# ZhehuiWu/MP-HSIR

Measured on AMD Instinct MI355X. Metric: hsi_patches_per_sec_fwd_bwd, higher is better.
Workload: dtype bf16; 1 GPU; natural-scene MP_HSIR_Net(31,31,64,T=6) training step fwd+bwd+allreduce+AdamW, 64x64x31 patches, batch 32/GPU, dp1; global_batch=32, patch=64x64x31, parallelism=dp1, launch=hipGraph replay

## Files before the change

include/mphsir.h:

```cpp
#ifndef MPHSIR_H
#define MPHSIR_H
#include <stddef.h>
#include <stdint.h>

#ifdef __cplusplus
extern "C" {
#endif

#define MPHSIR_OK 0
#define MPHSIR_EINVAL (-1)
#define MPHSIR_ELAUNCH (-2)

#define MPHSIR_F32 0
#define MPHSIR_BF16 1
#define MPHSIR_F16 2

const char* mphsir_version(void);
const char* mphsir_last_error(void);
int mphsir_device_arch(char* buf, int n);

typedef struct mphsir_gemm_args {
    uint32_t struct_size;
    const void* X; int64_t ldx;
    const void* W; int64_t w_batch_stride; int64_t rows_per_batch;
    const float* bias;
    const float* ln_w; const float* ln_b;
    void* Y; int64_t ldy;
    int64_t M, N, K;
    int epi;
    const void* R; int64_t ldr;
    const void* SA; int64_t ldsa;
    const float* gate;
    const float* keep;
    int32_t H, Wimg, shift;
    int32_t form;
} mphsir_gemm_args;
int mphsir_gemm_tok(const mphsir_gemm_args* a, int dtype, void* stream);

typedef struct mphsir_win_attn_args {
    uint32_t struct_size;
    const void* X;
    const float* ln_w; const float* ln_b;
    const void* Wqkv; const float* bqkv;
    const float* rpb;
    const void* Wproj; const float* bproj;
    void* SA;
    float* mu;
    void* Oattn;
    int32_t B, H, W, C, heads, shift;
} mphsir_win_attn_args;
typedef struct mphsir_pg_fwd_args {
    uint32_t struct_size;
    const float* mu;
    const float* Wprompt; const float* prompt_param; const float* Wq; const float* Wkv; const float* Wdown;
    const float* Wpproj; const float* bpproj; const float* Wup;
    float* gate;
    int32_t nW, C, r;
} mphsir_pg_fwd_args;
int mphsir_pg_gate_fwd(const mphsir_pg_fwd_args* a, void* stream);
int mphsir_win_attn_fwd(const mphsir_win_attn_args* a, int dtype, void* stream);
int mphsir_win_attn_hdp(int head_dim, int dtype);

typedef struct mphsir_gram_args {
    uint32_t struct_size;
    const void* Tq; int64_t ldq; const void* Tk; int64_t ldk; const void* Tv; int64_t ldv;
    const float* wq; const float* wk; const float* wv; int64_t ldw;
    void* V; int64_t ldvo;
    float* Gpart; float* Spart;
    int32_t B, H, W, C, heads, nsplit;
    void* QK; int64_t ldqk;
} mphsir_gram_args;
int mphsir_dwconv_gram(const mphsir_gram_args* a, int dtype, void* stream);
int mphsir_dwconv_gram_keeps_qk(int32_t C, int32_t W, int dtype);

typedef struct mphsir_fused_gram_args {
    uint32_t struct_size;
    const void* X; int64_t ldx;
    const float* ln_w; const float* ln_b;
    const void* Wqkv;
    const float* w9; int64_t ldw;
    void* V; int64_t ldvo;
    float* Gpart; float* Spart;
    int32_t B, H, W, C, heads, nsplit;
    int32_t head_groups;
    void* T; int64_t ldt;
    void* QK; int64_t ldqk;
    int32_t row_segments;
} mphsir_fused_gram_args;
int mphsir_qkv_dwconv_gram(const mphsir_fused_gram_args* a, int dtype, void* stream);
int mphsir_qkv_dwconv_gram_fits(int32_t C, int32_t heads, int32_t H, int32_t W, int dtype);
int mphsir_qkv_dwconv_gram_rows_fits(int32_t C, int32_t heads, int32_t H, int32_t W, int dtype, int32_t with_ln);
enum { MPHSIR_DEBUG_PG_GATE = 0, MPHSIR_DEBUG_WIN_ATTN = 1, MPHSIR_DEBUG_FUSED_PASS_A = 2 };
int mphsir_debug(int kind, void* stamps);
typedef struct mphsir_fold_args {
    uint32_t struct_size;
    const float* Gpart; const float* Spart;
    const float* temperature;
    const float* Wo;
    void* M;
    void* MT;
    int32_t B, C, heads, nsplit;
    float* Gsum; float* Ssum;
} mphsir_fold_args;
int mphsir_spectral_fold(const mphsir_fold_args* a, int dtype, void* stream);

typedef struct mphsir_gate_args {
    uint32_t struct_size;
    const void* T; int64_t ldt;
    const float* w9; int64_t ldw;
    void* U; int64_t ldu;
    int32_t B, H, W, HP;
} mphsir_gate_args;
int mphsir_dwconv_gate(const mphsir_gate_args* a, int dtype, void* stream);

typedef struct mphsir_gdfn_args {
    uint32_t struct_size;
    const void* X; int64_t ldx;
    const float* ln_w; const float* ln_b;
    const void* Win; const float* w9; int64_t ldw;
    const void* Wout;
    void* Y; int64_t ldy;
    int32_t B, H, W, D, HP, nsplit;
    void* T; int64_t ldt;
} mphsir_gdfn_args;
int mphsir_gdfn_fused(const mphsir_gdfn_args* a, int dtype, void* stream);
int mphsir_gdfn_fused_fits(int32_t D, int32_t HP, int32_t H, int32_t W, int dtype);
int mphsir_gdfn_fused_tile_width(int32_t D);

typedef struct mphsir_mlp_args {
    uint32_t struct_size;
    const void* X; int64_t ldx;
    const float* ln_w; const float* ln_b;
    const void* W1; const float* b1;
    const void* W2; const float* b2;
    const float* keep; int64_t rows_per_batch;
    void* Y; int64_t ldy;
    int64_t M; int32_t C, HP;
    int32_t tiles_per_wave;
    int32_t hsplit;
    float* ypart;
    const void* R; int64_t ldr;
    const void* PV; int64_t ldpv; const void* PM; int64_t pm_batch_stride;
    const void* PSA; int64_t ldpsa; const float* pgate; const float* pkeep;
    void* Yb; int64_t ldyb;
    int32_t H, Wimg, shift;
} mphsir_mlp_args;
int mphsir_gated_mlp_fwd(const mphsir_mlp_args* a, int dtype, void* stream);
int mphsir_gated_mlp_fwd_fuses(int32_t C, int64_t M, int dtype);

typedef struct mphsir_mlp_bwd_args {
    uint32_t struct_size;
    const void* X; const void* dY; const void* DM;
    const float* ln_w; const float* ln_b;
    const void* W1; const float* b1; const void* W1T; const void* W2T;
    void* dX; void* XN; void* H; void* DPRE; float* part;
    int64_t M; int32_t C, HP;
    int32_t variant;
    const float* keep;
    int64_t rows_per_batch;
    int32_t hsplit;
    float* dxn_part;
} mphsir_mlp_bwd_args;
int mphsir_gated_mlp_bwd(const mphsir_mlp_bwd_args* a, int dtype, void* stream);

typedef struct mphsir_mlp_wgrad_args {
    uint32_t struct_size;
    const void* XN; const void* DM;
    const void* W1; const float* b1; const void* W2T;
    float* dW1p; float* dW2p; float* db1p; float* db2p;
    int64_t M; int32_t C, HP;
    int32_t ranges;
    int32_t chunks_per_wg;
} mphsir_mlp_wgrad_args;
int mphsir_gated_mlp_wgrad(const mphsir_mlp_wgrad_args* a, int dtype, void* stream);
int mphsir_gated_mlp_wgrad_fits(int32_t C, int32_t chunks_per_wg, int dtype);

int mphsir_gdfn_dw_bwd(const void* T, const float* w9, int64_t ldw, const void* dU, void* U, void* dT, float* partial, int32_t nblk,
                       int32_t B, int32_t H, int32_t W, int32_t HP, int32_t round_mid, int dtype, void* stream);
int mphsir_gdfn_dw_bwd_fits(int32_t H, int32_t W, int32_t HP, int dtype);

int mphsir_combine_bwd(const void* dY, const void* SA, const float* gate, const float* keep, void* dOut, void* dSA,
                       float* dgate, int32_t B, int32_t H, int32_t W, int32_t C, int32_t shift, int dtype, void* stream);
typedef struct mphsir_win_attn_bwd_args {
    uint32_t struct_size;
    const void* X; const void* dSA; const float* dmu;
    const float* ln_w; const float* ln_b;
    const void* Wqkv; const float* bqkv; const float* rpb; const void* WprojT;
    void* dQKV; void* XNw; void* dSAt; float* drpb;
    int32_t B, H, W, C, heads, shift;
    int32_t head_split;
} mphsir_win_attn_bwd_args;
int mphsir_win_attn_bwd(const mphsir_win_attn_bwd_args* a, int dtype, void* stream);
int mphsir_win_attn_bwd_fits(int32_t C, int32_t heads, int dtype);
int mphsir_ln_bwd_win(const void* X, const void* dXNw, const void* dRes, const float* ln_w, void* dX, float* part,
                      int32_t B, int32_t H, int32_t W, int32_t C, int32_t shift, const float* ln_b, void* XN, int32_t linear,
                      int dtype, void* stream);

int mphsir_ln_bwd_win_dxn(const void* X, const void* dQKV, const void* WqkvT, const void* dRes, const void* dRes2, const float* ln_w, void* dX,
                          float* part, int32_t B, int32_t H, int32_t W, int32_t C, int32_t shift, int dtype, void* stream);
int mphsir_ln_bwd_win_dxn_fits(int32_t C, int dtype);
int mphsir_ln_bwd_tok_dxn(const void* X, const void* dY, const void* WT, const void* dRes, const float* ln_w, const float* ln_b, void* dX,
                          void* XN, float* part, int64_t M, int32_t C, int32_t K, int32_t x_f32, int dtype, void* stream);

int mphsir_layernorm_tok(const void* X, int x_dtype, const float* ln_w, const float* ln_b, void* Y, void* Xcopy, int y_dtype,
                         int64_t M, int32_t C, void* stream);

typedef struct mphsir_fold_bwd_args {
    uint32_t struct_size;
    const float* Gpart; const float* Spart; const float* temperature; const float* Wo; const float* dM;
    void* W2; float* dWo; float* dtemp;
    int32_t B, C, heads, nsplit;
    int32_t dM_nsplit;
    const void* DO; int64_t lddo; const void* V; int64_t ldv; int32_t N;
    const float* dm_scale;
    int32_t w2_blocks;
} mphsir_fold_bwd_args;
int mphsir_spectral_fold_bwd(const mphsir_fold_bwd_args* a, int dtype, void* stream);
typedef struct mphsir_pg_bwd_args {
    uint32_t struct_size;
    const float* mu; const float* dgate;
    const float* Wprompt; const float* prompt_param; const float* Wq; const float* Wkv; const float* Wdown;
    const float* Wpproj; const float* bpproj; const float* Wup;
    float* dmu; void* L; void* R;
    int32_t nW, C, r, KL, KR;
    int32_t lr_bf16;
} mphsir_pg_bwd_args;
int mphsir_pg_gate_bwd(const mphsir_pg_bwd_args* a, void* stream);

typedef struct mphsir_spectral_bwd_args {
    uint32_t struct_size;
    const void* QK; int64_t ldqk;
    const void* DO; int64_t lddo;
    const void* T; int64_t ldt;
    const void* W2; const void* MbT;
    const float* w9; int64_t ldw;
    void* dT; int64_t lddt;
    float* part;
    int32_t B, H, W, C, heads, nblk, round_dall;
    const float* vscale;
} mphsir_spectral_bwd_args;
int mphsir_spectral_dqkv_bwd(const mphsir_spectral_bwd_args* a, int dtype, void* stream);
int mphsir_spectral_dqkv_bwd_fits(int32_t C, int32_t heads, int32_t H, int32_t W, int dtype);
int mphsir_spectral_dqkv_bwd_slabs(int32_t C, int32_t heads);

int mphsir_conv3x3_tok(const void* X, int64_t ldx, const void* W, void* Y, int64_t ldy, int32_t B, int32_t H, int32_t Wd,
                       int32_t Cin, int32_t N, int dtype, void* stream);
int mphsir_im2col3x3(const void* X, int64_t ldx, void* Col, int32_t B, int32_t H, int32_t Wd, int32_t Cin, int dtype, void* stream);
int mphsir_conv3x3_wgrad(const void* dY, int64_t lddy, const void* X, int64_t ldx, float* Cpart, int32_t B, int32_t H, int32_t W,
                         int32_t Cout, int32_t Cin, int32_t nsplit, int32_t form ,
                         int dtype, void* stream);

int mphsir_gemm_tn(const void* A, int64_t lda, int64_t a_batch_stride, const void* B, int64_t ldb, int64_t b_batch_stride,
                   float* Cpart, float* colsum_part, int64_t M, int32_t N1, int32_t N2, int32_t nsplit, int32_t batch,
                   int32_t tile128, int dtype, void* stream);
#define MPHSIR_TN_GROUP_MAX 8
typedef struct mphsir_gemm_tn_problem {
    const void* A; int64_t lda; const void* B; int64_t ldb;
    float* Cpart; float* colsum_part;
    int64_t M; int32_t N1, N2, nsplit, pad_;
} mphsir_gemm_tn_problem;
int mphsir_gemm_tn_group(const mphsir_gemm_tn_problem* probs, int32_t n, int32_t form , int dtype, void* stream);

int mphsir_dwconv3x3(const void* X, int64_t ldx, const float* w9, int64_t ldw, void* Y, int64_t ldy,
                     int32_t B, int32_t H, int32_t W, int32_t C, int32_t flip, int dtype, void* stream);
int mphsir_dwconv3x3_wgrad(const void* X, int64_t ldx, const void* dY, int64_t lddy, float* partial, int32_t nblk,
                           int32_t B, int32_t H, int32_t W, int32_t C, int dtype, void* stream);
int mphsir_dwconv3x3_wgrad_tiled(int32_t H, int32_t W, int32_t C, int dtype);
int mphsir_dwconv3x3_bwd(const void* X, int64_t ldx, const void* dY, int64_t lddy, const float* w9, int64_t ldw, void* dX, int64_t lddx,
                         float* partial, int32_t nblk, int32_t B, int32_t H, int32_t W, int32_t C, int dtype, void* stream);

int mphsir_gdfn_gate_bwd(const void* T, const void* dU, void* U, void* dT, int64_t M, int32_t HP, int dtype, void* stream);
int mphsir_dwconv_gate_bwd(const void* T, const float* w9, int64_t ldw, const void* dU, void* U, void* dT, int32_t B, int32_t H, int32_t W,
                           int32_t HP, int dtype, void* stream);
int mphsir_dwconv_gate_bwd_fits(int32_t H, int32_t W, int32_t HP, int dtype);

int64_t mphsir_gemm_tn_workspace_bytes(int32_t N1, int32_t N2, int32_t nsplit, int32_t batch, int32_t with_colsum);
int64_t mphsir_dwconv_gram_workspace_bytes(int32_t B, int32_t nsplit, int32_t C, int32_t heads);
int64_t mphsir_pg_gate_bwd_workspace_bytes(int32_t nW, int32_t C, int32_t r, int dtype, int32_t* KL, int32_t* KR);
int64_t mphsir_win_attn_bwd_workspace_bytes(int32_t B, int32_t H, int32_t W, int32_t C, int32_t heads, int dtype);

int mphsir_tvsp_text_map(const float* L, const float* clip, float* text, int32_t B, int32_t ps, int32_t D, void* stream);
int mphsir_tvsp_text_map_bwd(const float* dtext, const float* clip, float* part, int32_t B, int32_t ps, int32_t D, void* stream);
int mphsir_resize_bilinear(const void* X, void* Y, int32_t B, int32_t h, int32_t w, int32_t H, int32_t W, int32_t C, int32_t backward,
                           int dtype, void* stream);

int mphsir_nchw_to_cl(const float* X, void* Y, int32_t B, int32_t C, int64_t HW, int32_t Cp, int dtype, void* stream);
int mphsir_cl_to_nchw_add(const void* Y, int64_t ldy, const float* R, float* O, int32_t B, int32_t C, int64_t HW, int dtype, void* stream);
int mphsir_task_weights(const int64_t* ids, float* w, int32_t B, int32_t n, int32_t T, void* stream);
int mphsir_mix_rows(const float* A, const float* Bm, float* O, int32_t I, int32_t J, int32_t D, float scale, int32_t transA, void* stream);

typedef struct mphsir_scene_gather_args {
    uint32_t struct_size;
    const float* scene;
    const int32_t* origins;
    float* tiles;
    int32_t n, C, H, W, th, tw;
} mphsir_scene_gather_args;
int mphsir_scene_gather(const mphsir_scene_gather_args* a, void* stream);
typedef struct mphsir_scene_blend_args {
    uint32_t struct_size;
    const float* tiles;
    const int32_t* oy;
    const int32_t* ox;
    float* scene;
    int32_t ny, nx, C, H, W, th, tw, ov, clamp01;
} mphsir_scene_blend_args;
int mphsir_scene_blend(const mphsir_scene_blend_args* a, void* stream);

typedef struct mphsir_scene_gather_d4_args {
    uint32_t struct_size;
    const float* scene;
    const int32_t* origins;
    float* tiles;
    int32_t j0, count, n_tiles, G, modes_packed, C, H, W, th, tw;
} mphsir_scene_gather_d4_args;
int mphsir_scene_gather_d4(const mphsir_scene_gather_d4_args* a, void* stream);
typedef struct mphsir_scene_fold_d4_args {
    uint32_t struct_size;
    const float* y;
    float* store;
    int32_t j0, count, n_tiles, G, modes_packed, C, th, tw;
} mphsir_scene_fold_d4_args;
int mphsir_scene_fold_d4(const mphsir_scene_fold_d4_args* a, void* stream);

typedef struct mphsir_quality_args {
    uint32_t struct_size;
    const float* restored;
    const float* clean;
    double* psnr;
    double* ssim;
    double* sam_deg;
    int64_t* sam_pixels;
    void* workspace;
    int64_t workspace_bytes;
    int32_t B, C, H, W;
} mphsir_quality_args;
int64_t mphsir_quality_workspace_bytes(int32_t B, int32_t C, int32_t H, int32_t W);
int mphsir_quality(const mphsir_quality_args* a, void* stream);

#define MPHSIR_DEG_NONE 0
#define MPHSIR_DEG_GAUSSIAN 1
#define MPHSIR_DEG_COMPLEX 2
#define MPHSIR_DEG_BLUR 3
#define MPHSIR_DEG_SR 4
#define MPHSIR_DEG_INPAINT 5
#define MPHSIR_DEG_BANDMISS 6
#define MPHSIR_DEG_HAZE 7
#define MPHSIR_DEG_MAX_TASKS 16
#define MPHSIR_DEG_MAX_STENCILS 16
#define MPHSIR_DEG_MAX_FACTORS 8
#define MPHSIR_DEG_STENCIL_SIDE 21
typedef struct mphsir_degrade_args {
    uint32_t struct_size;
    const float* clean;
    float* degraded;
    float* clean_aug;
    const int32_t* menu;
    const int32_t* ksize;
    const int32_t* sr_factor;
    const int32_t* task;
    const int32_t* aug;
    const float* param;
    const int32_t* sub;
    const float* band_sigma;
    const uint8_t* band_flag;
    const uint8_t* col_dead;
    const float* col_off;
    const float* stencils;
    const float* cirrus;
    const float* atm;
    const float* haze_ratio;
    const float* z;
    const float* u0;
    const float* u1;
    const int64_t* ordinal_dev;
    int64_t seed, ordinal;
    int32_t B, C, H, W, T, K, F;
} mphsir_degrade_args;
int mphsir_degrade_batch(const mphsir_degrade_args* a, void* stream);

int mphsir_flat_adamw(float* p, const float* g, float* m, float* v, int64_t n, float lr, float beta1, float beta2,
                      float eps, float weight_decay, int32_t step, float grad_scale, const float* hyper, void* stream);

int mphsir_grad_check(const float* g, int64_t n, float* scaler, void* stream);
int mphsir_flat_adamw_scaled(float* p, const float* g, float* m, float* v, int64_t n, float lr, float beta1, float beta2, float eps,
                             float weight_decay, float grad_scale, const float* hyper, const float* scaler, void* stream);
int mphsir_scaler_update(float* scaler, float growth_factor, float backoff_factor, int32_t growth_interval, void* stream);

#define MPHSIR_REDUCE_MAX_SEGS 32
typedef struct mphsir_reduce_seg {
    const float* src; float* dst;
    int64_t n, stride, src_batch_stride, dst_batch_stride;
    int32_t nsplit, nbatch;
    int32_t rows, dst_col_stride;
    int64_t src_ld, dst_ld;
} mphsir_reduce_seg;
int mphsir_reduce_parts(const mphsir_reduce_seg* segs, int32_t nseg, void* stream);

int mphsir_pack_gather(const float* arena, const int32_t* index, void* dst, int64_t n, int dtype, void* stream);

int mphsir_multi_copy(const int64_t* table_dev, int32_t nseg, int64_t total_blocks, void* stream);

int mphsir_l1_clamp_loss(const float* y, const float* clean, float* grad, float* part, int64_t n, int32_t nblocks, void* stream);

#define MPHSIR_K_GEMM_TOK 0
#define MPHSIR_K_WIN_ATTN 1
#define MPHSIR_K_DWCONV_GRAM 2
#define MPHSIR_K_SPECTRAL_FOLD 3
#define MPHSIR_K_GATED_MLP 4
#define MPHSIR_K_DWCONV_GATE 5
#define MPHSIR_K_FLAT_ADAMW 6
#define MPHSIR_K_DWCONV 7
#define MPHSIR_K_DWCONV_WGRAD 8
#define MPHSIR_K_GATED_MLP_BWD 9
#define MPHSIR_K_COMBINE_BWD 10
#define MPHSIR_K_WIN_ATTN_BWD 11
#define MPHSIR_K_LN_BWD_WIN 12
#define MPHSIR_K_GEMM_TN 13
#define MPHSIR_K_GDFN_GATE_BWD 14
#define MPHSIR_K_FOLD_BWD 15
#define MPHSIR_K_PG_GATE_BWD 16
#define MPHSIR_K_CONV3X3 17
#define MPHSIR_K_IM2COL 18
#define MPHSIR_K_REDUCE_PARTS 19
#define MPHSIR_K_PACK_GATHER 20
#define MPHSIR_K_LAYERNORM 21
#define MPHSIR_K_PG_GATE 22
#define MPHSIR_K_RESAMPLE 23
#define MPHSIR_K_QKV_DWCONV_GRAM 24
#define MPHSIR_K_GDFN_FUSED 25
#define MPHSIR_K_DWCONV_BWD 26
#define MPHSIR_K_MULTI_COPY 27
#define MPHSIR_K_L1_LOSS 28
#define MPHSIR_K_GATED_MLP_WGRAD 29
#define MPHSIR_K_SPECTRAL_DQKV_BWD 30
#define MPHSIR_K_LAYOUT 31
#define MPHSIR_K_SCENE 32
#define MPHSIR_K_QUALITY 33
#define MPHSIR_K_DEGRADE 34
#define MPHSIR_K_COUNT 35
int mphsir_prof_enable(int kid);
int mphsir_prof_read(int* launches, float* total_ms);
const char* mphsir_kernel_name(int kid);

#ifdef __cplusplus
}
#endif
#endif
```

mp-hsir_amd/_lib.py:

```python
import ctypes
import os

import torch

_HERE = os.path.dirname(os.path.abspath(__file__))
_PATH = os.path.join(_HERE, os.environ.get("MPHSIR_LIB_AB", "libmphsir.so"))
_lib = None
_is_emu = False

c_void_p, c_int64, c_int32, c_int, c_float_p = (ctypes.c_void_p, ctypes.c_int64, ctypes.c_int32, ctypes.c_int,
                                                ctypes.POINTER(ctypes.c_float))


class _Args(ctypes.Structure):

    def __init__(self, *args, **kw):
        super().__init__(*args, **kw)
        self.struct_size = ctypes.sizeof(self)


_SZ = [("struct_size", ctypes.c_uint32)]


class GemmArgs(_Args):
    _fields_ = _SZ + [("X", c_void_p), ("ldx", c_int64), ("W", c_void_p), ("w_batch_stride", c_int64),
                ("rows_per_batch", c_int64), ("bias", c_void_p), ("ln_w", c_void_p), ("ln_b", c_void_p),
                ("Y", c_void_p), ("ldy", c_int64), ("M", c_int64), ("N", c_int64), ("K", c_int64),
                ("epi", c_int), ("R", c_void_p), ("ldr", c_int64), ("SA", c_void_p), ("ldsa", c_int64),
                ("gate", c_void_p), ("keep", c_void_p), ("H", c_int32), ("Wimg", c_int32), ("shift", c_int32), ("form", c_int32)]


class MlpArgs(_Args):
    _fields_ = _SZ + [("X", c_void_p), ("ldx", c_int64), ("ln_w", c_void_p), ("ln_b", c_void_p), ("W1", c_void_p),
                ("b1", c_void_p), ("W2", c_void_p), ("b2", c_void_p), ("keep", c_void_p), ("rows_per_batch", c_int64),
                ("Y", c_void_p), ("ldy", c_int64), ("M", c_int64), ("C", c_int32), ("HP", c_int32), ("tiles_per_wave", c_int32),
                ("hsplit", c_int32), ("ypart", c_void_p), ("R", c_void_p), ("ldr", c_int64),
                ("PV", c_void_p), ("ldpv", c_int64), ("PM", c_void_p), ("pm_batch_stride", c_int64), ("PSA", c_void_p), ("ldpsa", c_int64),
                ("pgate", c_void_p), ("pkeep", c_void_p), ("Yb", c_void_p), ("ldyb", c_int64), ("H", c_int32), ("Wimg", c_int32), ("shift", c_int32)]


class WinAttnArgs(_Args):
    _fields_ = _SZ + [(n, c_void_p) for n in ("X", "ln_w", "ln_b", "Wqkv", "bqkv", "rpb", "Wproj", "bproj", "SA", "mu", "Oattn")] + \
               [(n, c_int32) for n in ("B", "H", "W", "C", "heads", "shift")]


class PgFwdArgs(_Args):
    _fields_ = _SZ + [(n, c_void_p) for n in ("mu", "Wprompt", "prompt_param", "Wq", "Wkv", "Wdown", "Wpproj", "bpproj", "Wup", "gate")] + \
               [(n, c_int32) for n in ("nW", "C", "r")]


class GramArgs(_Args):
    _fields_ = _SZ + [("Tq", c_void_p), ("ldq", c_int64), ("Tk", c_void_p), ("ldk", c_int64), ("Tv", c_void_p), ("ldv", c_int64),
                ("wq", c_void_p), ("wk", c_void_p), ("wv", c_void_p), ("ldw", c_int64), ("V", c_void_p), ("ldvo", c_int64),
                ("Gpart", c_void_p), ("Spart", c_void_p)] + [(n, c_int32) for n in ("B", "H", "W", "C", "heads", "nsplit")] + \
               [("QK", c_void_p), ("ldqk", c_int64)]


class FusedGramArgs(_Args):
    _fields_ = _SZ + [("X", c_void_p), ("ldx", c_int64), ("ln_w", c_void_p), ("ln_b", c_void_p), ("Wqkv", c_void_p), ("w9", c_void_p),
                ("ldw", c_int64), ("V", c_void_p), ("ldvo", c_int64), ("Gpart", c_void_p), ("Spart", c_void_p)] + \
               [(n, c_int32) for n in ("B", "H", "W", "C", "heads", "nsplit", "head_groups")] + \
               [("T", c_void_p), ("ldt", c_int64), ("QK", c_void_p), ("ldqk", c_int64), ("row_segments", c_int32)]


class FoldArgs(_Args):
    _fields_ = _SZ + [("Gpart", c_void_p), ("Spart", c_void_p), ("temperature", c_void_p), ("Wo", c_void_p), ("M", c_void_p),
                ("MT", c_void_p)] + \
               [(n, c_int32) for n in ("B", "C", "heads", "nsplit")] + [("Gsum", c_void_p), ("Ssum", c_void_p)]


class GateArgs(_Args):
    _fields_ = _SZ + [("T", c_void_p), ("ldt", c_int64), ("w9", c_void_p), ("ldw", c_int64), ("U", c_void_p), ("ldu", c_int64)] + \
               [(n, c_int32) for n in ("B", "H", "W", "HP")]


class GdfnArgs(_Args):
    _fields_ = _SZ + [("X", c_void_p), ("ldx", c_int64), ("ln_w", c_void_p), ("ln_b", c_void_p), ("Win", c_void_p), ("w9", c_void_p),
                ("ldw", c_int64), ("Wout", c_void_p), ("Y", c_void_p), ("ldy", c_int64)] + \
               [(n, c_int32) for n in ("B", "H", "W", "D", "HP", "nsplit")] + [("T", c_void_p), ("ldt", c_int64)]


class MlpBwdArgs(_Args):
    _fields_ = _SZ + [(n, c_void_p) for n in ("X", "dY", "DM", "ln_w", "ln_b", "W1", "b1", "W1T", "W2T", "dX", "XN", "H", "DPRE", "part")] + \
               [("M", c_int64), ("C", c_int32), ("HP", c_int32), ("variant", c_int32), ("keep", c_void_p), ("rows_per_batch", c_int64),
                ("hsplit", c_int32), ("dxn_part", c_void_p)]


class MlpWgradArgs(_Args):
    _fields_ = _SZ + [(n, c_void_p) for n in ("XN", "DM", "W1", "b1", "W2T", "dW1p", "dW2p", "db1p", "db2p")] + \
               [("M", c_int64), ("C", c_int32), ("HP", c_int32), ("ranges", c_int32), ("chunks_per_wg", c_int32)]


class WinAttnBwdArgs(_Args):
    _fields_ = _SZ + [(n, c_void_p) for n in ("X", "dSA", "dmu", "ln_w", "ln_b", "Wqkv", "bqkv", "rpb", "WprojT", "dQKV", "XNw",
                                         "dSAt", "drpb")] + [(n, c_int32) for n in ("B", "H", "W", "C", "heads", "shift", "head_split")]


class FoldBwdArgs(_Args):
    _fields_ = _SZ + [(n, c_void_p) for n in ("Gpart", "Spart", "temperature", "Wo", "dM", "W2", "dWo", "dtemp")] + \
               [(n, c_int32) for n in ("B", "C", "heads", "nsplit", "dM_nsplit")] + \
               [("DO", c_void_p), ("lddo", c_int64), ("V", c_void_p), ("ldv", c_int64), ("N", c_int32), ("dm_scale", c_void_p),
                ("w2_blocks", c_int32)]


class PgBwdArgs(_Args):
    _fields_ = _SZ + [(n, c_void_p) for n in ("mu", "dgate", "Wprompt", "prompt_param", "Wq", "Wkv", "Wdown", "Wpproj", "bpproj", "Wup",
                                         "dmu", "L", "R")] + [(n, c_int32) for n in ("nW", "C", "r", "KL", "KR", "lr_bf16")]


class SpectralBwdArgs(_Args):
    _fields_ = _SZ + [("QK", c_void_p), ("ldqk", c_int64), ("DO", c_void_p), ("lddo", c_int64), ("T", c_void_p), ("ldt", c_int64),
                      ("W2", c_void_p), ("MbT", c_void_p), ("w9", c_void_p), ("ldw", c_int64), ("dT", c_void_p), ("lddt", c_int64),
                      ("part", c_void_p)] + [(n, c_int32) for n in ("B", "H", "W", "C", "heads", "nblk", "round_dall")] + [("vscale", c_void_p)]


class SceneGatherArgs(_Args):
    _fields_ = _SZ + [("scene", c_void_p), ("origins", c_void_p), ("tiles", c_void_p)] + [(n, c_int32) for n in ("n", "C", "H", "W", "th", "tw")]


class SceneBlendArgs(_Args):
    _fields_ = _SZ + [("tiles", c_void_p), ("oy", c_void_p), ("ox", c_void_p), ("scene", c_void_p)] + \
               [(n, c_int32) for n in ("ny", "nx", "C", "H", "W", "th", "tw", "ov", "clamp01")]


class SceneGatherD4Args(_Args):
    _fields_ = _SZ + [("scene", c_void_p), ("origins", c_void_p), ("tiles", c_void_p)] + \
               [(n, c_int32) for n in ("j0", "count", "n_tiles", "G", "modes_packed", "C", "H", "W", "th", "tw")]


class SceneFoldD4Args(_Args):
    _fields_ = _SZ + [("y", c_void_p), ("store", c_void_p)] + [(n, c_int32) for n in ("j0", "count", "n_tiles", "G", "modes_packed", "C", "th", "tw")]


class QualityArgs(_Args):
    _fields_ = _SZ + [(n, c_void_p) for n in ("restored", "clean", "psnr", "ssim", "sam_deg", "sam_pixels", "workspace")] + \
               [("workspace_bytes", c_int64)] + [(n, c_int32) for n in ("B", "C", "H", "W")]


class DegradeArgs(_Args):
    _fields_ = _SZ + [(n, c_void_p) for n in ("clean", "degraded", "clean_aug", "menu", "ksize", "sr_factor", "task", "aug", "param", "sub", "band_sigma",
                                         "band_flag", "col_dead", "col_off", "stencils", "cirrus", "atm", "haze_ratio", "z", "u0", "u1",
                                         "ordinal_dev")] + [("seed", c_int64), ("ordinal", c_int64)] + \
               [(n, c_int32) for n in ("B", "C", "H", "W", "T", "K", "F")]


class TnProblem(ctypes.Structure):
    _fields_ = [("A", c_void_p), ("lda", c_int64), ("B", c_void_p), ("ldb", c_int64), ("Cpart", c_void_p), ("colsum_part", c_void_p),
                ("M", c_int64), ("N1", c_int32), ("N2", c_int32), ("nsplit", c_int32), ("pad_", c_int32)]


TN_GROUP_MAX = 8


class ReduceSeg(ctypes.Structure):
    _fields_ = [("src", c_void_p), ("dst", c_void_p), ("n", c_int64), ("stride", c_int64), ("src_batch_stride", c_int64),
                ("dst_batch_stride", c_int64), ("nsplit", c_int32), ("nbatch", c_int32), ("rows", c_int32),
                ("dst_col_stride", c_int32), ("src_ld", c_int64), ("dst_ld", c_int64)]


REDUCE_MAX_SEGS = 32


_SYMBOLS = {
    "mphsir_version": (ctypes.c_char_p, []),
    "mphsir_last_error": (ctypes.c_char_p, []),
    "mphsir_device_arch": (c_int, [ctypes.c_char_p, c_int]),
    "mphsir_kernel_name": (ctypes.c_char_p, [c_int]),
    "mphsir_gemm_tn_workspace_bytes": (c_int64, [c_int32, c_int32, c_int32, c_int32, c_int32]),
    "mphsir_dwconv_gram_workspace_bytes": (c_int64, [c_int32, c_int32, c_int32, c_int32]),
    "mphsir_pg_gate_bwd_workspace_bytes": (c_int64, [c_int32, c_int32, c_int32, c_int, ctypes.POINTER(c_int32), ctypes.POINTER(c_int32)]),
    "mphsir_win_attn_bwd_workspace_bytes": (c_int64, [c_int32, c_int32, c_int32, c_int32, c_int32, c_int]),
    "mphsir_prof_enable": (c_int, [c_int]),
    "mphsir_prof_read": (c_int, [ctypes.POINTER(c_int), c_float_p]),
    "mphsir_gemm_tok": (c_int, [ctypes.POINTER(GemmArgs), c_int, c_void_p]),
    "mphsir_tvsp_text_map": (c_int, [c_void_p, c_void_p, c_void_p, c_int32, c_int32, c_int32, c_void_p]),
    "mphsir_tvsp_text_map_bwd": (c_int, [c_void_p, c_void_p, c_void_p, c_int32, c_int32, c_int32, c_void_p]),
    "mphsir_resize_bilinear": (c_int, [c_void_p, c_void_p, c_int32, c_int32, c_int32, c_int32, c_int32, c_int32, c_int32, c_int, c_void_p]),
    "mphsir_layernorm_tok": (c_int, [c_void_p, c_int, c_void_p, c_void_p, c_void_p, c_void_p, c_int, c_int64, c_int32, c_void_p]),
    "mphsir_win_attn_fwd": (c_int, [ctypes.POINTER(WinAttnArgs), c_int, c_void_p]),
    "mphsir_win_attn_hdp": (c_int, [c_int, c_int]),
    "mphsir_pg_gate_fwd": (c_int, [ctypes.POINTER(PgFwdArgs), c_void_p]),
    "mphsir_dwconv_gram": (c_int, [ctypes.POINTER(GramArgs), c_int, c_void_p]),
    "mphsir_dwconv_gram_keeps_qk": (c_int, [c_int32, c_int32, c_int]),
    "mphsir_qkv_dwconv_gram": (c_int, [ctypes.POINTER(FusedGramArgs), c_int, c_void_p]),
    "mphsir_qkv_dwconv_gram_fits": (c_int, [c_int32, c_int32, c_int32, c_int32, c_int]),
    "mphsir_qkv_dwconv_gram_rows_fits": (c_int, [c_int32, c_int32, c_int32, c_int32, c_int, c_int32]),
    "mphsir_debug": (c_int, [c_int, c_void_p]),
    "mphsir_dwconv3x3_wgrad_tiled": (c_int, [c_int32, c_int32, c_int32, c_int]),
    "mphsir_spectral_fold": (c_int, [ctypes.POINTER(FoldArgs), c_int, c_void_p]),
    "mphsir_dwconv_gate": (c_int, [ctypes.POINTER(GateArgs), c_int, c_void_p]),
    "mphsir_dwconv_gate_bwd": (c_int, [c_void_p, c_void_p, c_int64, c_void_p, c_void_p, c_void_p, c_int32, c_int32, c_int32, c_int32, c_int, c_void_p]),
    "mphsir_dwconv_gate_bwd_fits": (c_int, [c_int32, c_int32, c_int32, c_int]),
    "mphsir_gdfn_dw_bwd": (c_int, [c_void_p, c_void_p, c_int64, c_void_p, c_void_p, c_void_p, c_void_p, c_int32, c_int32, c_int32, c_int32, c_int32, c_int32, c_int, c_void_p]),
    "mphsir_gdfn_dw_bwd_fits": (c_int, [c_int32, c_int32, c_int32, c_int]),
    "mphsir_gdfn_fused": (c_int, [ctypes.POINTER(GdfnArgs), c_int, c_void_p]),
    "mphsir_gdfn_fused_fits": (c_int, [c_int32, c_int32, c_int32, c_int32, c_int]),
    "mphsir_gdfn_fused_tile_width": (c_int, [c_int32]),
    "mphsir_dwconv3x3": (c_int, [c_void_p, c_int64, c_void_p, c_int64, c_void_p, c_int64, c_int32, c_int32, c_int32, c_int32,
                                 c_int32, c_int, c_void_p]),
    "mphsir_dwconv3x3_bwd": (c_int, [c_void_p, c_int64, c_void_p, c_int64, c_void_p, c_int64, c_void_p, c_int64, c_void_p, c_int32, c_int32, c_int32,
                                     c_int32, c_int32, c_int, c_void_p]),
    "mphsir_dwconv3x3_wgrad": (c_int, [c_void_p, c_int64, c_void_p, c_int64, c_void_p, c_int32, c_int32, c_int32, c_int32,
                                       c_int32, c_int, c_void_p]),
    "mphsir_flat_adamw": (c_int, [c_void_p, c_void_p, c_void_p, c_void_p, c_int64, ctypes.c_float, ctypes.c_float,
                                  ctypes.c_float, ctypes.c_float, ctypes.c_float, c_int32, ctypes.c_float, c_void_p, c_void_p]),
    "mphsir_grad_check": (c_int, [c_void_p, c_int64, c_void_p, c_void_p]),
    "mphsir_flat_adamw_scaled": (c_int, [c_void_p, c_void_p, c_void_p, c_void_p, c_int64, ctypes.c_float, ctypes.c_float, ctypes.c_float,
                                         ctypes.c_float, ctypes.c_float, ctypes.c_float, c_void_p, c_void_p, c_void_p]),
    "mphsir_scaler_update": (c_int, [c_void_p, ctypes.c_float, ctypes.c_float, c_int32, c_void_p]),
    "mphsir_combine_bwd": (c_int, [c_void_p] * 7 + [c_int32] * 5 + [c_int, c_void_p]),
    "mphsir_win_attn_bwd": (c_int, [ctypes.POINTER(WinAttnBwdArgs), c_int, c_void_p]),
    "mphsir_win_attn_bwd_fits": (c_int, [c_int32, c_int32, c_int]),
    "mphsir_ln_bwd_win": (c_int, [c_void_p] * 6 + [c_int32] * 5 + [c_void_p, c_void_p, c_int32, c_int, c_void_p]),
    "mphsir_ln_bwd_win_dxn": (c_int, [c_void_p] * 8 + [c_int32] * 5 + [c_int, c_void_p]),
    "mphsir_ln_bwd_win_dxn_fits": (c_int, [c_int32, c_int]),
    "mphsir_ln_bwd_tok_dxn": (c_int, [c_void_p] * 9 + [c_int64, c_int32, c_int32, c_int32, c_int, c_void_p]),
    "mphsir_gemm_tn": (c_int, [c_void_p, c_int64, c_int64, c_void_p, c_int64, c_int64, c_void_p, c_void_p, c_int64, c_int32, c_int32,
                               c_int32, c_int32, c_int32, c_int, c_void_p]),
    "mphsir_spectral_fold_bwd": (c_int, [ctypes.POINTER(FoldBwdArgs), c_int, c_void_p]),
    "mphsir_pg_gate_bwd": (c_int, [ctypes.POINTER(PgBwdArgs), c_void_p]),
    "mphsir_spectral_dqkv_bwd": (c_int, [ctypes.POINTER(SpectralBwdArgs), c_int, c_void_p]),
    "mphsir_spectral_dqkv_bwd_fits": (c_int, [c_int32, c_int32, c_int32, c_int32, c_int]),
    "mphsir_spectral_dqkv_bwd_slabs": (c_int, [c_int32, c_int32]),
    "mphsir_conv3x3_tok": (c_int, [c_void_p, c_int64, c_void_p, c_void_p, c_int64, c_int32, c_int32, c_int32, c_int32, c_int32,
                                   c_int, c_void_p]),
    "mphsir_conv3x3_wgrad": (c_int, [c_void_p, c_int64, c_void_p, c_int64, c_void_p, c_int32, c_int32, c_int32, c_int32, c_int32, c_int32, c_int32, c_int, c_void_p]),
    "mphsir_im2col3x3": (c_int, [c_void_p, c_int64, c_void_p, c_int32, c_int32, c_int32, c_int32, c_int, c_void_p]),
    "mphsir_gdfn_gate_bwd": (c_int, [c_void_p, c_void_p, c_void_p, c_void_p, c_int64, c_int32, c_int, c_void_p]),
    "mphsir_gated_mlp_bwd": (c_int, [ctypes.POINTER(MlpBwdArgs), c_int, c_void_p]),
    "mphsir_gated_mlp_wgrad": (c_int, [ctypes.POINTER(MlpWgradArgs), c_int, c_void_p]),
    "mphsir_gated_mlp_wgrad_fits": (c_int, [c_int32, c_int32, c_int]),
    "mphsir_gated_mlp_fwd": (c_int, [ctypes.POINTER(MlpArgs), c_int, c_void_p]),
    "mphsir_gated_mlp_fwd_fuses": (c_int, [c_int32, c_int64, c_int]),
    "mphsir_reduce_parts": (c_int, [ctypes.POINTER(ReduceSeg), c_int32, c_void_p]),
    "mphsir_gemm_tn_group": (c_int, [ctypes.POINTER(TnProblem), c_int32, c_int32, c_int, c_void_p]),
    "mphsir_pack_gather": (c_int, [c_void_p, c_void_p, c_void_p, c_int64, c_int, c_void_p]),
    "mphsir_multi_copy": (c_int, [c_void_p, c_int32, c_int64, c_void_p]),
    "mphsir_nchw_to_cl": (c_int, [c_void_p, c_void_p, c_int32, c_int32, c_int64, c_int32, c_int, c_void_p]),
    "mphsir_cl_to_nchw_add": (c_int, [c_void_p, c_int64, c_void_p, c_void_p, c_int32, c_int32, c_int64, c_int, c_void_p]),
    "mphsir_task_weights": (c_int, [c_void_p, c_void_p, c_int32, c_int32, c_int32, c_void_p]),
    "mphsir_mix_rows": (c_int, [c_void_p, c_void_p, c_void_p, c_int32, c_int32, c_int32, ctypes.c_float, c_int32, c_void_p]),
    "mphsir_scene_gather": (c_int, [ctypes.POINTER(SceneGatherArgs), c_void_p]),
    "mphsir_scene_blend": (c_int, [ctypes.POINTER(SceneBlendArgs), c_void_p]),
    "mphsir_scene_gather_d4": (c_int, [ctypes.POINTER(SceneGatherD4Args), c_void_p]),
    "mphsir_scene_fold_d4": (c_int, [ctypes.POINTER(SceneFoldD4Args), c_void_p]),
    "mphsir_quality_workspace_bytes": (c_int64, [c_int32, c_int32, c_int32, c_int32]),
    "mphsir_quality": (c_int, [ctypes.POINTER(QualityArgs), c_void_p]),
    "mphsir_degrade_batch": (c_int, [ctypes.POINTER(DegradeArgs), c_void_p]),
    "mphsir_l1_clamp_loss": (c_int, [c_void_p, c_void_p, c_void_p, c_void_p, c_int64, c_int32, c_void_p]),
}


def symbols():
    return sorted(_SYMBOLS)


def _bind(lib):
    for name, (res, args) in _SYMBOLS.items():
        fn = getattr(lib, name)
        fn.restype = res
        fn.argtypes = args
    return lib


def load(path=None):
    global _lib, _is_emu
    if _lib is not None and path is None:
        return _lib
    p = path or _PATH
    if not os.path.exists(p):
        raise RuntimeError("mp-hsir_amd: HIP library %s not found -- run `python mp-hsir_amd/build.py` "
                           "(there is no CPU fallback)" % p)
    try:
        lib = _bind(ctypes.CDLL(p))
    except (OSError, AttributeError) as e:
        raise RuntimeError("mp-hsir_amd: cannot load %s: %s" % (p, e))
    _lib = lib
    _is_emu = path is not None and "hipemu" in os.path.abspath(path)
    return _lib


def use_library_for_tests(path):
    return load(path)


def is_emulated():
    return _is_emu


def check(rc, what):
    if rc != 0:
        raise RuntimeError("mp-hsir_amd: %s failed (%d): %s" % (what, rc, load().mphsir_last_error().decode()))
```

mp-hsir_amd/autograd_ops.py:

```python
import torch
import torch.nn.functional as F

from . import ops


class SkipGrad:

    def __init__(self):
        self.dz = None

    def take(self):
        dz, self.dz = self.dz, None
        return dz


def _skip_put(skip, dz, needed):
    if not needed:
        return None
    if skip is not None and skip[2]:
        skip[0].dz = dz
        return None
    return dz


def _skip_take(skip):
    return skip[0].take() if (skip is not None and skip[1]) else None


class _GatedMlp(torch.autograd.Function):

    @staticmethod
    def forward(ctx, blk, k2, y, ln_w, ln_b, fc1_w, fc1_b, fc2_w, fc2_b, res=None, skip=None):
        B, H, W, Cc = y.shape
        pk = blk.packed(y.dtype)
        ctx.blk, ctx.k2, ctx.skip = blk, k2, skip
        ctx.save_for_backward(y)
        z = ops.gated_mlp_fwd(y.reshape(-1, Cc), pk["ln2"][0], pk["ln2"][1], pk["W1"], pk["b1"], pk["W2"], pk["b2"],
                              keep=k2, rows_per_batch=H * W, res=None if res is None else res.reshape(-1, Cc))
        return z.reshape(B, H, W, Cc)

    @staticmethod
    def backward(ctx, dz):
        (y,) = ctx.saved_tensors
        return (None, None) + _gated_mlp_backward(ctx.blk, ctx.k2, y, dz) + (_skip_put(ctx.skip, dz, ctx.needs_input_grad[9]), None)


def _gated_mlp_backward(blk, k2, y, dz):
    B, H, W, Cc = y.shape
    dt = y.dtype
    pk = blk.packed(dt)
    dz2 = dz.reshape(-1, Cc).contiguous()
    hid = blk.mlp.fc2.weight.shape[1]
    HP = pk["W2T"].shape[0]
    fused = ops.gated_mlp_wgrad_fits(dz2.shape[0], Cc, HP, dt)
    if k2 is None:
        dm = dz2
        dx, xn, h, dpre, part = ops.gated_mlp_bwd(y.reshape(-1, Cc), dz2, dm, pk["ln2"][0], pk["ln2"][1], pk["W1"], pk["b1"],
                                                  pk["W1T"], pk["W2T"], operands=not fused)
    else:
        dx, xn, h, dpre, part, dm = ops.gated_mlp_bwd(y.reshape(-1, Cc), dz2, None, pk["ln2"][0], pk["ln2"][1], pk["W1"], pk["b1"],
                                                      pk["W1T"], pk["W2T"], keep=k2, rows_per_batch=H * W, operands=not fused)
    with ops.reduce_scope(leaf=True):
        if fused:
            dW1, db1, dW2, db2 = ops.gated_mlp_wgrad(xn, dm, pk["W1"], pk["b1"], pk["W2T"], hid)
        else:
            dW2, db2 = ops.gemm_tn_blocks(dm, h, [(0, Cc)], ncols=hid, colsum=True)
            dW1, db1 = ops.gemm_tn_blocks(dpre, xn, [(0, hid), (HP, hid)], colsum=True)
        dln = ops.reduce_parts(part)
    return (dx.reshape(B, H, W, Cc), dln[0], dln[1], dW1, db1, dW2, db2)


def channel_attention_bwd(d_out, t_q, t_k, t_v, w9q, w9k, w9v, v, gp, sp, Mb, MbT, temperature, wo, heads, B, H, W, qk=None, keep=None):
    C = v.shape[1]
    N = H * W
    M = B * N
    dt = v.dtype
    temp32, wo32 = temperature.detach().reshape(heads).float().contiguous(), wo.detach().reshape(C, C).float().contiguous()
    joint = (t_q.data_ptr() + C * t_q.element_size() == t_k.data_ptr() and t_k.data_ptr() + C * t_k.element_size() == t_v.data_ptr()
             and t_q.stride() == t_k.stride() == t_v.stride() and w9q.data_ptr() + 4 * C == w9k.data_ptr()
             and w9k.data_ptr() + 4 * C == w9v.data_ptr())
    fused = joint and t_q.stride(2) == 3 * C and w9q.stride(0) == 3 * C and ops.spectral_dqkv_bwd_fits(C, heads, H, W, dt)
    if ops.fold_bwd_forms_dm(N, C, heads, dt):
        W2, dwo_p, dtemp_p = ops.spectral_fold_bwd(gp, sp, temp32, wo32, None, dt, reduce=False, d_out=d_out.reshape(M, C), v=v.reshape(M, C), dm_scale=keep,
                                                   w2_blocks=fused)
    else:
        dM = ops.gemm_tn(d_out.reshape(B, N, C), v.reshape(B, N, C), reduce=False)
        W2, dwo_p, dtemp_p = ops.spectral_fold_bwd(gp, sp, temp32, wo32, dM, dt, reduce=False, dm_scale=keep, w2_blocks=fused)
    if qk is not None:
        pass
    elif joint:
        qk = ops.dwconv3x3(torch.as_strided(t_q, (B, H, W, 2 * C), t_q.stride()), torch.as_strided(w9q, (9, 2 * C), w9q.stride()))
    else:
        qk = torch.empty((B, H, W, 2 * C), dtype=dt, device=v.device)
        ops.dwconv3x3(t_q, w9q, out=qk[..., :C])
        ops.dwconv3x3(t_k, w9k, out=qk[..., C:])
    if fused:
        dwo, dtemp = ops.reduce_parts(dwo_p), ops.reduce_parts(dtemp_p)
        t_all = torch.as_strided(t_q, (M, 3 * C), (3 * C, 1))
        w9_all = torch.as_strided(w9q, (9, 3 * C), w9q.stride())
        dt_all, dw_all = ops.spectral_dqkv_bwd(qk.reshape(M, 2 * C), d_out, t_all, W2, MbT, w9_all, B, H, W, C, heads, vscale=keep)
        dt_all = dt_all.reshape(B, H, W, 3 * C)
        return (dt_all[..., :C], dt_all[..., C:2 * C], dt_all[..., 2 * C:], dw_all[:C], dw_all[C:2 * C], dw_all[2 * C:], dtemp, dwo)
    assert keep is None, "the unscaled d_out form needs the fused launch (ops.spectral_dqkv_bwd_fits)"
    dall = torch.empty((M, 3 * C), dtype=dt, device=v.device)
    ops.gemm_tok(d_out, MbT, out=dall[:, 2 * C:])
    dwo, dtemp = ops.reduce_parts(dwo_p), ops.reduce_parts(dtemp_p)
    ops.gemm_tok(qk.reshape(M, 2 * C), W2, out=dall[:, :2 * C])
    dall4 = dall.reshape(B, H, W, 3 * C)
    if joint:
        t_all = torch.as_strided(t_q, (B, H, W, 3 * C), t_q.stride())
        w9_all = torch.as_strided(w9q, (9, 3 * C), w9q.stride())
        dt_all, dw_all = ops.dwconv3x3_bwd(t_all, dall4, w9_all, col_ranges=[(0, 3 * C)])
        return (dt_all[..., :C], dt_all[..., C:2 * C], dt_all[..., 2 * C:], dw_all[:C], dw_all[C:2 * C], dw_all[2 * C:],
                dtemp, dwo)
    dq4, dk4, dv4 = dall4[..., :C], dall4[..., C:2 * C], dall4[..., 2 * C:]
    dw3 = torch.empty((3 * C, 9), dtype=torch.float32, device=v.device)
    dkv = torch.empty((B, H, W, 2 * C), dtype=dt, device=v.device)
    return (ops.dwconv3x3(dq4, w9q, flip=True), ops.dwconv3x3(dk4, w9k, flip=True, out=dkv[..., :C]), ops.dwconv3x3(dv4, w9v, flip=True, out=dkv[..., C:]),
            ops.dwconv3x3_wgrad(t_q, dq4, col_ranges=[(0, C)], out=dw3[:C]), ops.dwconv3x3_wgrad(t_k, dk4, col_ranges=[(0, C)], out=dw3[C:2 * C]),
            ops.dwconv3x3_wgrad(t_v, dv4, col_ranges=[(0, C)], out=dw3[2 * C:]), dtemp, dwo)


import os
COMBINE_SIDE = os.environ.get("MPHSIR_COMBINE_SIDE", "0") == "1"


_PG_KEYS = ("linear_down.weight", "linear_up.weight", "linear_prompt.weight", "prompt_param", "q.weight", "kv.weight",
            "proj.weight", "proj.bias")


def _pass_a_infer(x2, wqkv, w9, B, H, W, C, heads, ln=None):
    if ops.qkv_dwconv_gram_fits(C, heads, H, W, x2.dtype):
        v, gp, sp, _ = ops.qkv_dwconv_gram(x2, wqkv, w9, B, H, W, C, heads, ln=ln)
    else:
        t = ops.gemm_tok(x2, wqkv, ln=ln)
        v, gp, sp, _ = ops.dwconv_gram(t[:, :C], t[:, C:2 * C], t[:, 2 * C:], w9[:, :C], w9[:, C:2 * C], w9[:, 2 * C:], 3 * C, B, H, W, C, heads)
    return v, gp, sp


def _pgsstb_attn_infer(blk, k1, x, fuse=False):
    B, H, W, Cc = x.shape
    dt = x.dtype
    pk = blk.packed(dt)
    sp = blk.gobal_spectral_attn.packed(dt)
    heads, shift = blk.num_heads, blk.shift_size
    sa, mu, _ = ops.win_attn_fwd(x, pk["ln1"][0], pk["ln1"][1], pk["wqkv"], pk["bqkv"], pk["rpb"], pk["wproj"], pk["bproj"],
                                 pk["pg"], heads, shift, gate=False)
    sa2 = sa.reshape(-1, Cc)
    v, gp, spart = _pass_a_infer(sa2, sp["wqkv"], sp["w9"], B, H, W, Cc, heads)
    with ops.side_stream(sa, ops.SIDE_BRANCH) as br:
        gate = ops.pg_gate_fwd(mu, pk["pg"])
    Mb = ops.spectral_fold(gp, spart, sp["temp"], sp["wo"], dt)
    br.join()
    if fuse:
        return dict(v=v, Mb=Mb, sa=sa2, gate=gate, keep=k1, geom=(H, W, shift))
    y = ops.gemm_tok(v, Mb, epi=2, res=x.reshape(-1, Cc), sa=sa2, gate=gate, keep=k1, geom=(H, W, shift))
    return y.reshape(B, H, W, Cc)


def _self_channel_attn_infer(attn, ln, geom, t2):
    B, H, W = geom
    pa = attn.packed(t2.dtype)
    v, gp, sp = _pass_a_infer(t2, pa["wqkv"], pa["w9"], B, H, W, t2.shape[1], attn.num_heads, ln=ln.pair())
    return ops.gemm_tok(v, ops.spectral_fold(gp, sp, pa["temp"], pa["wo"], t2.dtype), epi=1, res=t2)


def _pgsstb_attn_forward(blk, k1, x, fuse=False):
    B, H, W, Cc = x.shape
    dt = x.dtype
    pk = blk.packed(dt)
    sp = blk.gobal_spectral_attn.packed(dt)
    heads, shift = blk.num_heads, blk.shift_size
    w9 = sp["w9"]
    sa, mu, oattn = ops.win_attn_fwd(x, pk["ln1"][0], pk["ln1"][1], pk["wqkv"], pk["bqkv"], pk["rpb"], pk["wproj"],
                                     pk["bproj"], pk["pg"], heads, shift, save=True, gate=False)
    with ops.side_stream(sa, ops.SIDE_BRANCH) as br:
        gate = ops.pg_gate_fwd(mu, pk["pg"])
    sa2 = sa.reshape(-1, Cc)
    if ops.FUSED_TRAIN and ops.qkv_dwconv_gram_fits(Cc, heads, H, W, dt):
        v, gp, spart, _, t, qk = ops.qkv_dwconv_gram(sa2, sp["wqkv"], w9, B, H, W, Cc, heads, keep=True)
    else:
        t = ops.gemm_tok(sa2, sp["wqkv"])
        v, gp, spart, _, qk = ops.dwconv_gram(t[:, :Cc], t[:, Cc:2 * Cc], t[:, 2 * Cc:], w9[:, :Cc], w9[:, Cc:2 * Cc], w9[:, 2 * Cc:],
                                              3 * Cc, B, H, W, Cc, heads, keep_qk=True)
    Mb, MbT, gp, spart = ops.spectral_fold(gp, spart, sp["temp"], sp["wo"], dt, transposed=True)
    br.join()
    saved = (x, sa, gate, mu, oattn, t, v, gp, spart, Mb, MbT) + ((qk,) if qk is not None else ())
    if fuse:
        return None, saved
    y = ops.gemm_tok(v, Mb, epi=2, res=x.reshape(-1, Cc), sa=sa2, gate=gate, keep=k1, geom=(H, W, shift))
    return y.reshape(B, H, W, Cc), saved


def _pgsstb_attn_backward(blk, k1, saved, dy, extra=None):
    x, sa, gate, mu, oattn, t, v, gp, spart, Mb, MbT = saved[:11]
    qk = saved[11] if len(saved) > 11 else None
    B, H, W, Cc = x.shape
    dt = x.dtype
    M = B * H * W
    heads, shift = blk.num_heads, blk.shift_size
    pk = blk.packed(dt)
    sp = blk.gobal_spectral_attn.packed(dt)
    dy = dy.contiguous()
    with ops.reduce_scope(leaf=True):
        f32_factors = dt == torch.float16 or mu.shape[0] <= 512
        lean = COMBINE_SIDE and ops.spectral_dqkv_bwd_fits(Cc, heads, H, W, dt) and sp["w9"].stride(0) == 3 * Cc and t.is_contiguous()
        if lean:
            with ops.side_stream(dy, ops.SIDE_BRANCH) as br:
                _, d_sa, dgate = ops.combine_bwd(dy, sa, gate, k1, shift, want_dout=False)
                dmu, gpg = ops.pg_gate_bwd(mu, dgate, pk["pg"], factor_dtype=torch.float32 if f32_factors else dt)
            d_out, keep_s = dy, k1
        else:
            d_out, d_sa, dgate = ops.combine_bwd(dy, sa, gate, k1, shift)
            keep_s = None
            with ops.side_stream(dy, ops.SIDE_BRANCH) as br:
                dmu, gpg = ops.pg_gate_bwd(mu, dgate, pk["pg"], factor_dtype=torch.float32 if f32_factors else dt)
        t4 = t.reshape(B, H, W, 3 * Cc)
        w9 = sp["w9"]
        tq, tk, tv = t4[..., :Cc], t4[..., Cc:2 * Cc], t4[..., 2 * Cc:]
        dtq, dtk, dtv, dwq, dwk, dwv, dtemp, dwo = channel_attention_bwd(
            d_out.reshape(M, Cc), tq, tk, tv, w9[:, :Cc], w9[:, Cc:2 * Cc], w9[:, 2 * Cc:], v, gp, spart, Mb, MbT,
            blk.gobal_spectral_attn.temperature, blk.gobal_spectral_attn.project_out.weight, heads, B, H, W, qk=qk, keep=keep_s)
        if dtq.data_ptr() + Cc * dtq.element_size() == dtk.data_ptr() and dtq.stride(2) == 3 * Cc:
            dt3 = torch.as_strided(dtq, (M, 3 * Cc), (3 * Cc, 1))
        else:
            dt3 = torch.cat([dtq, dtk, dtv], dim=-1).reshape(M, 3 * Cc)
        if lean:
            br.join()
        d_sa = ops.gemm_tok(dt3, sp["wqkvT"], epi=1, res=d_sa.reshape(M, Cc))
        d_sqkv = ops.gemm_tn(dt3, sa.reshape(M, Cc)).reshape(3 * Cc, Cc, 1, 1)
        dpg = tuple(gpg[k].reshape(getattr_path(blk.local_spectral_attn, k).shape) for k in _PG_KEYS)
        if not lean:
            br.join()
        dqkv, xnw, dsat, drpb = ops.win_attn_bwd(x, d_sa.reshape(B, H, W, Cc), dmu, pk["ln1"][0], pk["ln1"][1], pk["wqkv"], pk["bqkv"],
                                                 pk["rpb"], pk["wprojT"], heads, shift)
        d_qkv_w, d_qkv_b = ops.gemm_tn(dqkv, xnw, colsum=True)
        dsat2 = dsat.reshape(M, Cc)
        d_proj_w, d_proj_b = ops.gemm_tn(dsat2, oattn.reshape(M, Cc), colsum=True)
        if ops.ln_bwd_win_dxn_fits(M, Cc, dt):
            dx, part = ops.ln_bwd_win_dxn(x, dqkv, pk["wqkvT"], dy, pk["ln1"][0], shift, dres2=None if extra is None else extra.contiguous())
        else:
            dx, part = ops.ln_bwd_win(x, ops.gemm_tok(dqkv, pk["wqkvT"]), dy, pk["ln1"][0], shift)
            if extra is not None:
                dx = dx + extra
        dln = ops.reduce_parts(part)
        drpb = ops.reduce_parts(drpb)
    d_sdw = _join_taps(dwq, dwk, dwv).reshape(3 * Cc, 1, 3, 3)
    return (dx, dln[0], dln[1], d_qkv_w, d_qkv_b, d_proj_w, d_proj_b, drpb,
            dtemp.reshape(heads, 1, 1), d_sqkv, d_sdw, dwo.reshape(Cc, Cc, 1, 1)) + tuple(dpg)




class _PgsstbAttn(torch.autograd.Function):

    @staticmethod
    def forward(ctx, blk, k1, skip, x, n1w, n1b, qkv_w, qkv_b, proj_w, proj_b, rpb, s_temp, s_qkv, s_dw, s_out, *pg):
        y, saved = _pgsstb_attn_forward(blk, k1, x)
        ctx.blk, ctx.k1, ctx.skip = blk, k1, skip
        ctx.save_for_backward(*saved)
        return y

    @staticmethod
    def backward(ctx, dy):
        return (None, None, None) + _pgsstb_attn_backward(ctx.blk, ctx.k1, ctx.saved_tensors, dy, extra=_skip_take(ctx.skip))


_N_ATTN_PARAMS = 11 + len(_PG_KEYS)


class _Pgsstb(torch.autograd.Function):

    @staticmethod
    def forward(ctx, blk, k1, k2, res, skip, x, *params):
        B, H, W, Cc = x.shape
        _, saved = _pgsstb_attn_forward(blk, k1, x, fuse=True)
        pk = blk.packed(x.dtype)
        z, y = ops.gated_mlp_fwd(x.reshape(-1, Cc), pk["ln2"][0], pk["ln2"][1], pk["W1"], pk["b1"], pk["W2"], pk["b2"], keep=k2, rows_per_batch=H * W,
                                 res=None if res is None else res.reshape(-1, Cc),
                                 branch=dict(v=saved[6], Mb=saved[9], sa=saved[1].reshape(-1, Cc), gate=saved[2], keep=k1,
                                             geom=(H, W, blk.shift_size), want_y=True))
        ctx.blk, ctx.k1, ctx.k2, ctx.skip = blk, k1, k2, skip
        ctx.save_for_backward(y.reshape(B, H, W, Cc), *saved)
        return z.reshape(B, H, W, Cc)

    @staticmethod
    def backward(ctx, dz):
        y, saved = ctx.saved_tensors[0], ctx.saved_tensors[1:]
        d_res = _skip_put(ctx.skip, dz, ctx.needs_input_grad[3])
        gm = _gated_mlp_backward(ctx.blk, ctx.k2, y, dz)
        ga = _pgsstb_attn_backward(ctx.blk, ctx.k1, saved, gm[0], extra=_skip_take(ctx.skip))
        return (None, None, None, d_res, None) + ga + gm[1:]


def _join_taps(*dw):
    w0 = dw[0]
    ok, off = True, w0.data_ptr()
    for w in dw:
        ok = (ok and w.data_ptr() == off and w.is_contiguous()
              and w.untyped_storage().data_ptr() == w0.untyped_storage().data_ptr())
        off += w.numel() * w.element_size()
    if ok:
        return torch.as_strided(w0, (sum(w.shape[0] for w in dw), 9), (9, 1))
    ops.flush_deferred()
    return torch.cat(dw, dim=0)


def getattr_path(mod, dotted):
    for part in dotted.split("."):
        mod = getattr(mod, part)
    return mod


def pgsstb(blk, x, k1, k2, res=None, skip=None):
    a, sp, pgm = blk.attn, blk.gobal_spectral_attn, blk.local_spectral_attn
    m = blk.mlp
    B, H, W, Cc = x.shape
    fuse = ops.gated_mlp_fuses(B * H * W, Cc, H * W, x.dtype)
    if not torch.is_grad_enabled():
        if fuse:
            pk = blk.packed(x.dtype)
            z, _ = ops.gated_mlp_fwd(x.reshape(-1, Cc), pk["ln2"][0], pk["ln2"][1], pk["W1"], pk["b1"], pk["W2"], pk["b2"], keep=k2, rows_per_batch=H * W,
                                     res=None if res is None else res.reshape(-1, Cc), branch=_pgsstb_attn_infer(blk, k1, x, fuse=True))
            return z.reshape(B, H, W, Cc)
        y = _pgsstb_attn_infer(blk, k1, x)
    else:
        attn_params = (blk.norm1.weight, blk.norm1.bias, a.qkv.weight, a.qkv.bias, a.proj.weight, a.proj.bias,
                       a.relative_position_bias_table, sp.temperature, sp.qkv.weight, sp.qkv_dwconv.weight,
                       sp.project_out.weight, *[getattr_path(pgm, k) for k in _PG_KEYS])
        if fuse:
            return _Pgsstb.apply(blk, k1, k2, res, skip, x, *attn_params, blk.norm2.weight, blk.norm2.bias, m.fc1.weight, m.fc1.bias, m.fc2.weight, m.fc2.bias)
        y = _PgsstbAttn.apply(blk, k1, skip, x, *attn_params)
    return _GatedMlp.apply(blk, k2, y, blk.norm2.weight, blk.norm2.bias, m.fc1.weight, m.fc1.bias, m.fc2.weight, m.fc2.bias, res, skip)


class _GdfnRes(torch.autograd.Function):

    @staticmethod
    def forward(ctx, ffn, ln, geom, a2, ln_w, ln_b, w_in, w_dw, w_out):
        B, H, W = geom
        pf = ffn.packed(a2.dtype)
        D, HP = a2.shape[1], pf["w_out"].shape[1]
        if B * H * W >= ops.GDFN_FUSED_MIN_PIXELS and ops.gdfn_fused_fits(D, HP, H, W, a2.dtype):
            y, t = ops.gdfn_fused(a2, ln.pair(), pf["w_in"], pf["w9"], pf["w_out"], B, H, W, keep=True)
        else:
            t = ops.gemm_tok(a2, pf["w_in"], ln=ln.pair())
            u = ops.dwconv_gate(t, pf["w9"], B, H, W)
            y = ops.gemm_tok(u, pf["w_out"], epi=1, res=a2)
        ctx.ffn, ctx.ln, ctx.geom = ffn, ln, geom
        ctx.save_for_backward(a2, t)
        return y

    @staticmethod
    def backward(ctx, dy):
        a2, t = ctx.saved_tensors
        ffn, ln, (B, H, W) = ctx.ffn, ctx.ln, ctx.geom
        pf = ffn.packed(a2.dtype)
        HP = pf["w_out"].shape[1]
        hid = ffn.project_out.weight.shape[1]
        D = a2.shape[1]
        dy = dy.contiguous()
        t4 = t.reshape(B, H, W, 2 * HP)
        with ops.reduce_scope(leaf=True):
            du = ops.gemm_tok(dy, pf["w_outT"])
            if ops.gdfn_dw_bwd_fits(H, W, HP, a2.dtype):
                u, dt_, dwp = ops.gdfn_dw_bwd(t, pf["w9"], du, B, H, W)
                d_out_w = ops.gemm_tn_blocks(dy, u, [(0, D)], ncols=hid).reshape(D, hid, 1, 1)
                d_dw = torch.empty((2 * hid, 9), dtype=torch.float32, device=t.device)
                ops.reduce_block(dwp, 0, 9, 0, hid, d_dw[:hid], transpose=True)
# ... 405 lines not shown
```

mp-hsir_amd/csrc/arena.hip:

```cpp
#include <stdlib.h>

#include "mphsir_dev.h"
#include "mphsir_host.h"

namespace mphsir {

struct RedSegDev {
    const float* src; float* dst;
    long n, stride, sbs, dbs, t0, nitems;
    long src_ld, dst_ld;
    int nsplit, vec, lg, rows, dcs;
};
struct RedDev {
    RedSegDev s[MPHSIR_REDUCE_MAX_SEGS];
    int nseg; long threads;
};

__global__ __launch_bounds__(256) void reduce_parts_kernel(RedDev a) {
    const long t = (long)blockIdx.x * 256 + threadIdx.x;
    if (t >= a.threads) return;
    RedSegDev s = a.s[0];
#pragma unroll
    for (int k = 1; k < MPHSIR_REDUCE_MAX_SEGS; ++k)
        if (k < a.nseg && t >= a.s[k].t0) s = a.s[k];
    const int G = 1 << s.lg;
    const long local = t - s.t0, item = local >> s.lg, ipr = (s.n + 3) / 4, ipb = ipr * s.rows;
    const int g = (int)(local & (G - 1));
    const bool live = item < s.nitems;
    const long b = live ? item / ipb : 0, rem = live ? item % ipb : 0, r = rem / ipr, i4 = (rem % ipr) * 4;
    const float* src = s.src + b * s.sbs + r * s.src_ld + i4;
    const int ne = (s.n - i4) < 4 ? (int)(s.n - i4) : 4;
    f32x4 acc = f32x4{0.f, 0.f, 0.f, 0.f};
    if (live) {
        int sp = g;
        if (s.vec & 1) {
            for (; sp + 7 * G < s.nsplit; sp += 8 * G) {
                f32x4 v[8];
#pragma unroll
                for (int u = 0; u < 8; ++u) v[u] = *reinterpret_cast<const f32x4*>(src + (long)(sp + u * G) * s.stride);
#pragma unroll
                for (int u = 0; u < 8; ++u) acc += v[u];
            }
            for (; sp < s.nsplit; sp += G) acc += *reinterpret_cast<const f32x4*>(src + (long)sp * s.stride);
        } else {
            for (; sp + 7 * G < s.nsplit; sp += 8 * G) {
                f32x4 v[8];
#pragma unroll
                for (int u = 0; u < 8; ++u)
                    for (int e = 0; e < 4; ++e) v[u][e] = e < ne ? src[(long)(sp + u * G) * s.stride + e] : 0.f;
#pragma unroll
                for (int u = 0; u < 8; ++u) acc += v[u];
            }
            for (; sp < s.nsplit; sp += G)
                for (int e = 0; e < ne; ++e) acc[e] += src[(long)sp * s.stride + e];
        }
    }
    for (int m = 1; m < G; m <<= 1)
        for (int e = 0; e < 4; ++e) acc[e] += __shfl_xor(acc[e], m);
    if (live && g == 0) {
        float* dst = s.dst + b * s.dbs + r * s.dst_ld + i4 * s.dcs;
        if (s.vec & 2) *reinterpret_cast<f32x4*>(dst) = acc;
        else
            for (int e = 0; e < ne; ++e) dst[(long)e * s.dcs] = acc[e];
    }
}

template <class T>
__global__ __launch_bounds__(256) void pack_gather_kernel(const float* arena, const int* idx, T* dst, long n) {
    const long i = (long)blockIdx.x * 256 + threadIdx.x;
    if (i >= n / 4) return;
    const int* ip = idx + i * 4;
    const int i0 = ip[0], i1 = ip[1], i2 = ip[2], i3 = ip[3];
    f32x4 v;
    v[0] = i0 >= 0 ? arena[i0] : 0.f;
    v[1] = i1 >= 0 ? arena[i1] : 0.f;
    v[2] = i2 >= 0 ? arena[i2] : 0.f;
    v[3] = i3 >= 0 ? arena[i3] : 0.f;
    store4<T>(dst + i * 4, v);
}

constexpr int MC_BLOCK = 4096;
__global__ __launch_bounds__(256) void multi_copy_kernel(const long* __restrict__ table, int nseg) {
    const long b = blockIdx.x;
    int lo = 0, hi = nseg - 1;
    while (lo < hi) {
        const int mid = (lo + hi + 1) >> 1;
        if (table[4 * mid + 3] <= b) lo = mid; else hi = mid - 1;
    }
    const float* src = reinterpret_cast<const float*>(table[4 * lo]);
    float* dst = reinterpret_cast<float*>(table[4 * lo + 1]);
    const long n = table[4 * lo + 2], e0 = (b - table[4 * lo + 3]) * MC_BLOCK;
    const long e1 = e0 + MC_BLOCK < n ? e0 + MC_BLOCK : n;
    if ((((unsigned long)src | (unsigned long)dst) & 15) == 0) {
        for (long e = e0 + 4 * threadIdx.x; e + 4 <= e1; e += 1024) *reinterpret_cast<f32x4*>(dst + e) = *reinterpret_cast<const f32x4*>(src + e);
        for (long e = e0 + ((e1 - e0) & ~3L) + threadIdx.x; e < e1; e += 256) dst[e] = src[e];
    } else {
        for (long e = e0 + threadIdx.x; e < e1; e += 256) dst[e] = src[e];
    }
}

__device__ __forceinline__ float clamp01_nan(float y) { return y < 0.f ? 0.f : (y > 1.f ? 1.f : y); }
__global__ __launch_bounds__(256) void l1_clamp_loss_kernel(const float* __restrict__ y, const float* __restrict__ c, float* __restrict__ g,
                                                            float* __restrict__ part, long n, float inv_n) {
    __shared__ float red[4];
    float acc = 0.f;
    const long stride = (long)gridDim.x * 1024;
    for (long e = (long)blockIdx.x * 1024 + 4 * threadIdx.x; e < n; e += stride) {
        if (e + 4 <= n) {
            const f32x4 yv = *reinterpret_cast<const f32x4*>(y + e), cv = *reinterpret_cast<const f32x4*>(c + e);
            f32x4 gv;
            for (int i = 0; i < 4; ++i) {
                const float d = clamp01_nan(yv[i]) - cv[i];
                acc += fabsf(d);
                gv[i] = (yv[i] >= 0.f && yv[i] <= 1.f) ? (d > 0.f ? inv_n : (d < 0.f ? -inv_n : 0.f)) : 0.f;
            }
            if (g) *reinterpret_cast<f32x4*>(g + e) = gv;
        } else {
            for (long k = e; k < n; ++k) {
                const float d = clamp01_nan(y[k]) - c[k];
                acc += fabsf(d);
                if (g) g[k] = (y[k] >= 0.f && y[k] <= 1.f) ? (d > 0.f ? inv_n : (d < 0.f ? -inv_n : 0.f)) : 0.f;
            }
        }
    }
    acc = wave_sum(acc);
    if (lane_id() == 0) red[wave_id()] = acc;
    __syncthreads();
    if (threadIdx.x == 0) part[blockIdx.x] = ((red[0] + red[1]) + (red[2] + red[3])) * inv_n;
}

}

extern "C" int mphsir_multi_copy(const int64_t* table_dev, int32_t nseg, int64_t total_blocks, void* stream) {
    using namespace mphsir;
    clear_error();
    MPHSIR_REQUIRE(table_dev && nseg > 0 && total_blocks > 0 && total_blocks < (1LL << 31), "multi_copy: bad arguments");
    static_assert(sizeof(long) == sizeof(int64_t), "table rows are 64-bit");
    MPHSIR_LAUNCH(MPHSIR_K_MULTI_COPY, multi_copy_kernel, dim3((unsigned)total_blocks), dim3(256), 0, reinterpret_cast<hipStream_t>(stream),
                  reinterpret_cast<const long*>(table_dev), (int)nseg);
    return MPHSIR_OK;
}

extern "C" int mphsir_l1_clamp_loss(const float* y, const float* clean, float* grad, float* part, int64_t n, int32_t nblocks, void* stream) {
    using namespace mphsir;
    clear_error();
    MPHSIR_REQUIRE(y && clean && part && n > 0 && nblocks > 0 && nblocks <= 65535, "l1_clamp_loss: bad arguments");
    MPHSIR_REQUIRE(aligned16(y) && aligned16(clean) && (grad == nullptr || aligned16(grad)), "l1_clamp_loss: 16-byte alignment required");
    MPHSIR_LAUNCH(MPHSIR_K_L1_LOSS, l1_clamp_loss_kernel, dim3((unsigned)nblocks), dim3(256), 0, reinterpret_cast<hipStream_t>(stream),
                  y, clean, grad, part, (long)n, 1.0f / (float)n);
    return MPHSIR_OK;
}

extern "C" int mphsir_reduce_parts(const mphsir_reduce_seg* segs, int32_t nseg, void* stream) {
    using namespace mphsir;
    clear_error();
    MPHSIR_REQUIRE(segs && nseg > 0 && nseg <= MPHSIR_REDUCE_MAX_SEGS, "reduce_parts: 1..%d segments per call", MPHSIR_REDUCE_MAX_SEGS);
    RedDev d;
    d.nseg = nseg;
    long threads = 0;
    for (int k = 0; k < nseg; ++k) {
        const mphsir_reduce_seg& g = segs[k];
        MPHSIR_REQUIRE(g.src && g.dst && g.n > 0 && g.nsplit > 0 && g.nbatch > 0, "reduce_parts: bad segment %d", k);
        const int rows = g.rows > 1 ? g.rows : 1, dcs = g.dst_col_stride > 0 ? g.dst_col_stride : 1;
        const long src_ld = rows > 1 ? (long)g.src_ld : 0, dst_ld = rows > 1 ? (long)g.dst_ld : 0;
        const bool vload = aligned16(g.src) && g.n % 4 == 0 && g.stride % 4 == 0 && g.src_batch_stride % 4 == 0 && src_ld % 4 == 0;
        const bool vstore = vload && aligned16(g.dst) && dcs == 1 && g.dst_batch_stride % 4 == 0 && dst_ld % 4 == 0;
        const long nitems = (long)g.nbatch * rows * ((g.n + 3) / 4);
        int lg = 0;
        while (lg < 6 && (g.nsplit >> lg) > 32) ++lg;
        while (lg < 6 && (nitems << lg) < 8192 && (g.nsplit >> lg) > 4) ++lg;
        d.s[k] = RedSegDev{g.src, g.dst, (long)g.n, (long)g.stride, (long)g.src_batch_stride, (long)g.dst_batch_stride, threads, nitems,
                           src_ld, dst_ld, g.nsplit, (vload ? 1 : 0) | (vstore ? 2 : 0), lg, rows, dcs};
        threads += ((nitems << lg) + 63) / 64 * 64;
    }
    d.threads = threads;
    MPHSIR_LAUNCH(MPHSIR_K_REDUCE_PARTS, reduce_parts_kernel, dim3((unsigned)((threads + 255) / 256)), dim3(256), 0,
                  reinterpret_cast<hipStream_t>(stream), d);
    return MPHSIR_OK;
}

extern "C" int mphsir_pack_gather(const float* arena, const int32_t* index, void* dst, int64_t n, int dtype, void* stream) {
    using namespace mphsir;
    clear_error();
    MPHSIR_REQUIRE(arena && index && dst, "pack_gather: null pointer");
    MPHSIR_REQUIRE(MPHSIR_DTYPE_OK(dtype), "pack_gather: dtype %d unsupported", dtype);
    const int vec = dtype == MPHSIR_F32 ? 4 : 8;
    MPHSIR_REQUIRE(n > 0 && n % vec == 0 && aligned16(index) && aligned16(dst), "pack_gather: n must be a multiple of %d, 16-byte alignment", vec);
    const dim3 grid((unsigned)((n / 4 + 255) / 256));
    hipStream_t s = reinterpret_cast<hipStream_t>(stream);
    if (dtype == MPHSIR_F32) {
        MPHSIR_LAUNCH(MPHSIR_K_PACK_GATHER, pack_gather_kernel<float>, grid, dim3(256), 0, s, arena, index, reinterpret_cast<float*>(dst), (long)n);
    } else if (dtype == MPHSIR_BF16) {
        MPHSIR_LAUNCH(MPHSIR_K_PACK_GATHER, pack_gather_kernel<bf16_t>, grid, dim3(256), 0, s, arena, index, reinterpret_cast<bf16_t*>(dst), (long)n);
    } else {
        MPHSIR_LAUNCH(MPHSIR_K_PACK_GATHER, pack_gather_kernel<f16_t>, grid, dim3(256), 0, s, arena, index, reinterpret_cast<f16_t*>(dst), (long)n);
    }
    return MPHSIR_OK;
}
```

mp-hsir_amd/csrc/pg_gate.hip:

```cpp
#include "mphsir_dev.h"
#include "mphsir_host.h"

namespace mphsir {

constexpr int PG_NWIN = 16;
constexpr int PG_RMAX = 32;

struct PgDev {
    const float* mu; const float* dgate;
    const float* Wprompt; const float* Pp; const float* Wq; const float* Wkv; const float* Wdown;
    const float* Wpproj; const float* bpproj; const float* Wup;
    float* gate;
    float* dmu;
    void* L; void* R;
    int nW, C, r, KL, KR, lr_bf16;
    int stage_wdn;
    int wpg;
    unsigned long long* dbg;
};
static unsigned long long* g_pg_dbg = nullptr;
#define PG_MARK(k) do { if (a.dbg && blockIdx.x == 0 && threadIdx.x == 0) a.dbg[k] = __builtin_amdgcn_s_memtime(); } while (0)

__device__ __forceinline__ f32x4 pg_frag_rows(const float* W, int ld, int nrows, int row0, int k0) {
    const int l = lane_id();
    int row = row0 + (l & 15);
    row = row < nrows ? row : nrows - 1;
    return *reinterpret_cast<const f32x4*>(W + (long)row * ld + k0 + 4 * (l >> 4));
}
__device__ __forceinline__ f32x4 pg_frag_cols(const float* W, int ld, int ncols, int nk, int col0, int k0) {
    const int l = lane_id();
    int col = col0 + (l & 15);
    col = col < ncols ? col : ncols - 1;
    const int kb = k0 + 4 * (l >> 4);
    f32x4 v;
#pragma unroll
    for (int j = 0; j < 4; ++j) {
        const int k = kb + j < nk ? kb + j : nk - 1;
        v[j] = kb + j < nk ? W[(long)k * ld + col] : 0.f;
        (void)k;
    }
    return v;
}

struct FastDiv {
    unsigned d, m;
    __device__ __forceinline__ explicit FastDiv(int dd) : d((unsigned)dd), m(0xFFFFFFFFu / (unsigned)dd + 1u) {}
    __device__ __forceinline__ int div(int i) const { return (int)(((unsigned long long)(unsigned)i * m) >> 32); }
};

struct PgLds {
    float* mu;
    float* dg;
    float* w;
    float* dl;
    float* P;
    float* Wq;
    float* Wkv;
    float* Wpp;
    float* bpp;
    float* Wup;
    float* Wdn;
    float* sm;
    float* At;
    int LDC, LDW, LDA, RP;
};
#define PG_S (0 * pgw)
#define PG_D (1 * pgw)
#define PG_KV (2 * pgw)
#define PG_Q (4 * pgw)
#define PG_O (5 * pgw)
#define PG_O2 (6 * pgw)
#define PG_DO2 (7 * pgw)
#define PG_DO (8 * pgw)
#define PG_DQ (9 * pgw)
#define PG_DKV (10 * pgw)
#define PG_DD (12 * pgw)
#define PG_DS (13 * pgw)
#define PG_RS (14 * pgw)
#define PG_SMW (15 * pgw + 4)

__device__ __forceinline__ PgLds pg_lds(float* base, int C, int r, bool bwd, bool wdn = false) {
    PgLds s;
    const int pgw = r;
    s.LDC = C + 8;
    s.LDW = 128 + 8;
    s.RP = r + 1;
    s.LDA = r * (r + 1) + 4;
    s.mu = base;
    s.dg = s.mu + PG_NWIN * s.LDC;
    s.w = s.dg + (bwd ? PG_NWIN * s.LDC : 0);
    s.dl = s.w + PG_NWIN * s.LDW;
    s.P = s.dl + (bwd ? PG_NWIN * s.LDW : 0);
    s.Wq = s.P + 128 * (r + 1);
    s.Wkv = s.Wq + r * (r + 1);
    s.Wpp = s.Wkv + 2 * r * (r + 1);
    s.bpp = s.Wpp + r * (r + 1) + (4 - (132 * (r + 1)) % 4) % 4;
    s.Wup = s.bpp + ((r + 3) & ~3);
    s.Wdn = s.Wup + C * (r + 1) + 32 + (4 - (C * (r + 1)) % 4) % 4;
    s.sm = s.Wdn + (bwd && wdn ? r * C : 0);
    s.At = s.sm + PG_NWIN * PG_SMW;
    return s;
}
static size_t pg_lds_bytes(int C, int r, bool bwd, bool wdn = false) {
    const size_t rp = r + 1;
    const int pgw = r;
    size_t n = (size_t)PG_NWIN * (C + 8) * (bwd ? 2 : 1) + (size_t)PG_NWIN * 136 * (bwd ? 2 : 1) + 132 * rp + 3 + 4 * (size_t)r * rp +
               ((r + 3) & ~3) + (size_t)C * rp + 32 + 3 + (size_t)PG_NWIN * PG_SMW;
    if (bwd) n += (size_t)PG_NWIN * (r * rp + 4) + (wdn ? (size_t)r * C : 0);
    return n * sizeof(float);
}

template <int NT, bool COLS>
__device__ __forceinline__ void pg_load_chunk(f32x4 (&wf)[8][NT], const float* W, int ld, int nrows, int nk, const int (&row0)[NT], int k0, int K) {
#pragma unroll
    for (int i = 0; i < 8; ++i)
#pragma unroll
        for (int t = 0; t < NT; ++t)
            if (k0 + 16 * i < K)
                wf[i][t] = COLS ? pg_frag_cols(W, ld, nrows, nk, row0[t], k0 + 16 * i) : pg_frag_rows(W, ld, nrows, row0[t], k0 + 16 * i);
}
template <int NT>
__device__ __forceinline__ void pg_mma_chunk(f32x4 (&acc)[NT], const f32x4 (&wf)[8][NT], const float* B, int ldb, int k0, int K) {
#pragma unroll
    for (int i = 0; i < 8; ++i)
        if (k0 + 16 * i < K) {
            const f32x4 b = load_frag<float>(B, ldb, 0, k0 + 16 * i);
#pragma unroll
            for (int t = 0; t < NT; ++t) mma(acc[t], wf[i][t], b);
        }
}
template <int NT, bool COLS>
__device__ __forceinline__ void pg_mfma_rows(f32x4 (&acc)[NT], f32x4 (&wf)[8][NT], const float* W, int ld, int nrows, int nk,
                                             const int (&row0)[NT], const float* B, int ldb, int K) {
    pg_mma_chunk<NT>(acc, wf, B, ldb, 0, K);
    for (int k0 = 128; k0 < K; k0 += 128) {
        pg_load_chunk<NT, COLS>(wf, W, ld, nrows, nk, row0, k0, K);
        pg_mma_chunk<NT>(acc, wf, B, ldb, k0, K);
    }
}

template <bool KEEP_AT, int R>
__device__ __forceinline__ void pg_forward_chain(const PgDev& a, const PgLds& s, int win0) {
    const int C = a.C, r = R > 0 ? R : a.r, pgw = r, tid = threadIdx.x, lane = tid & 63, wv = wave_id_uniform(), nwl = a.wpg;
    const int rows[2] = {wv * 32, wv * 32 + 16}, rowd[1] = {wv * 16};
    const bool has_d = wv * 16 < r;
    PG_MARK(0);
    f32x4 wfp[8][2], wfd[8][1];
    pg_load_chunk<2, false>(wfp, a.Wprompt, C, 128, 0, rows, 0, C);
    if (has_d) pg_load_chunk<1, false>(wfd, a.Wdown, C, r, 0, rowd, 0, C);
    const FastDiv byC(C), byR(r);
#pragma unroll 4
    for (int i = tid; i < nwl * C; i += 256) {
        const int w = byC.div(i), c = i - w * C;
        s.mu[w * s.LDC + c] = win0 + w < a.nW ? a.mu[(long)(win0 + w) * C + c] : 0.f;
    }
    const int RP = s.RP;
#pragma unroll 4
    for (int i = tid; i < 128 * r; i += 256) { const int q = byR.div(i); s.P[q * RP + i - q * r] = a.Pp[i]; }
    for (int i = tid; i < r * r; i += 256) {
        const int q = byR.div(i), o = q * RP + i - q * r;
        s.Wq[o] = a.Wq[i]; s.Wpp[o] = a.Wpproj[i]; s.Wkv[o] = a.Wkv[i]; s.Wkv[r * RP + o] = a.Wkv[r * r + i];
    }
    if (tid < r) s.bpp[tid] = a.bpproj[tid];
#pragma unroll 4
    for (int i = tid; i < C * r; i += 256) { const int q = byR.div(i); s.Wup[q * RP + i - q * r] = a.Wup[i]; }
    if (tid < 32) s.Wup[C * RP + tid] = 0.f;
    if (KEEP_AT && a.stage_wdn)
        for (int i = tid; i < r * C; i += 256) s.Wdn[i] = a.Wdown[i];
    __syncthreads();
    PG_MARK(1);
    {
        f32x4 acc[2] = {{0, 0, 0, 0}, {0, 0, 0, 0}};
        pg_mfma_rows<2, false>(acc, wfp, a.Wprompt, C, 128, 0, rows, s.mu, s.LDC, C);
        const int w = lane & 15, rr = (lane >> 4) * 4;
        for (int j = 0; j < 4; ++j) {
            s.w[w * s.LDW + wv * 32 + rr + j] = acc[0][j];
            s.w[w * s.LDW + wv * 32 + 16 + rr + j] = acc[1][j];
        }
        if (has_d) {
            f32x4 accd[1] = {{0, 0, 0, 0}};
            pg_mfma_rows<1, false>(accd, wfd, a.Wdown, C, r, 0, rowd, s.mu, s.LDC, C);
            for (int j = 0; j < 4; ++j)
                if (wv * 16 + rr + j < r) s.sm[w * PG_SMW + PG_D + wv * 16 + rr + j] = accd[0][j];
        }
    }
    __syncthreads();
    PG_MARK(2);
    for (int ww = 0; ww < 4; ++ww) {
        if (wv * 4 + ww >= nwl) break;
        float* lw = s.w + (wv * 4 + ww) * s.LDW;
        const float l0 = lw[lane], l1 = lw[lane + 64];
        float m = fmaxf(l0, l1);
        for (int k = 32; k >= 1; k >>= 1) m = fmaxf(m, __shfl_xor(m, k));
        const float e0 = expf(l0 - m), e1 = expf(l1 - m);
        const float tot = wave_sum(e0 + e1);
        lw[lane] = e0 / tot;
        lw[lane + 64] = e1 / tot;
    }
    const FastDiv by2R(2 * r);
    for (int i = tid; i < nwl * 2 * r; i += 256) {
        const int w = by2R.div(i), m = i - w * 2 * r;
        const float* d = s.sm + w * PG_SMW + PG_D;
        float acc = 0.f;
        for (int j = 0; j < r; ++j) acc += s.Wkv[m * RP + j] * d[j];
        s.sm[w * PG_SMW + PG_KV + m] = acc;
    }
    __syncthreads();
    PG_MARK(3);
    for (int i = tid; i < nwl * r; i += 256) {
        const int w = byR.div(i), j = i - w * r;
        const float* lw = s.w + w * s.LDW;
        float acc = 0.f;
        for (int p = 0; p < 128; ++p) acc += lw[p] * s.P[p * RP + j];
        s.sm[w * PG_SMW + PG_S + j] = acc;
    }
    __syncthreads();
    PG_MARK(4);
    for (int i = tid; i < nwl * r; i += 256) {
        const int w = byR.div(i), m = i - w * r;
        const float* sv = s.sm + w * PG_SMW + PG_S;
        float acc = 0.f;
        for (int j = 0; j < r; ++j) acc += s.Wq[m * RP + j] * sv[j];
        s.sm[w * PG_SMW + PG_Q + m] = acc;
    }
    __syncthreads();
    PG_MARK(5);
    const float sc = rsqrtf((float)r);
    for (int i = tid; i < nwl * r; i += 256) {
        const int w = byR.div(i), m = i - w * r;
        const float* kv = s.sm + w * PG_SMW + PG_KV;
        const float qs = s.sm[w * PG_SMW + PG_Q + m] * sc;
        float mx = -3.0e38f;
        for (int j = 0; j < r; ++j) mx = fmaxf(mx, qs * kv[j]);
        float den = 0.f, num = 0.f;
        for (int j = 0; j < r; ++j) {
            const float e = expf(qs * kv[j] - mx);
            if (KEEP_AT) s.At[w * s.LDA + m * RP + j] = e;
            den += e;
            num += e * kv[r + j];
        }
        if (KEEP_AT)
            for (int j = 0; j < r; ++j) s.At[w * s.LDA + m * RP + j] /= den;
        s.sm[w * PG_SMW + PG_O + m] = num / den;
    }
    __syncthreads();
    PG_MARK(6);
    for (int i = tid; i < nwl * r; i += 256) {
        const int w = byR.div(i), m = i - w * r;
        const float* o = s.sm + w * PG_SMW + PG_O;
        float acc = s.bpp[m];
        for (int j = 0; j < r; ++j) acc += s.Wpp[m * RP + j] * o[j];
        s.sm[w * PG_SMW + PG_O2 + m] = acc;
    }
    __syncthreads();
}

template <int R>
__global__ __launch_bounds__(256) void pg_gate_fwd_kernel(PgDev a) {
    HIP_DYNAMIC_SHARED(f32x4, smem_v)
    const int C = a.C, r = R > 0 ? R : a.r, pgw = r, tid = threadIdx.x, nwl = a.wpg, win0 = blockIdx.x * nwl;
    const PgLds s = pg_lds(reinterpret_cast<float*>(smem_v), C, r, false);
    pg_forward_chain<false, R>(a, s, win0);
    PG_MARK(7);
    const FastDiv byC(C);
    if (R > 0 && R % 4 == 0 && 256 % C == 0) {
        constexpr int RR = R > 0 ? R : 4;
        const int c = tid % C;
        float wrow[RR];
#pragma unroll
        for (int j = 0; j < RR; ++j) wrow[j] = s.Wup[c * s.RP + j];
        for (int i = tid; i < nwl * C; i += 256) {
            const int w = byC.div(i);
            if (win0 + w >= a.nW) continue;
            const float* o2 = s.sm + w * PG_SMW + PG_O2;
            float acc = 0.f;
#pragma unroll
            for (int j4 = 0; j4 < RR / 4; ++j4) {
                const f32x4 ov = *reinterpret_cast<const f32x4*>(o2 + 4 * j4);
                for (int e = 0; e < 4; ++e) acc += wrow[4 * j4 + e] * ov[e];
            }
            a.gate[(long)(win0 + w) * C + c] = acc;
        }
    } else {
        for (int i = tid; i < nwl * C; i += 256) {
            const int w = byC.div(i), c = i - w * C;
            if (win0 + w >= a.nW) continue;
            const float* o2 = s.sm + w * PG_SMW + PG_O2;
            float acc = 0.f;
            for (int j = 0; j < r; ++j) acc += s.Wup[c * s.RP + j] * o2[j];
            a.gate[(long)(win0 + w) * C + c] = acc;
        }
    }
    PG_MARK(8);
}

template <int R>
__global__ __launch_bounds__(256) void pg_gate_bwd_kernel(PgDev a) {
    HIP_DYNAMIC_SHARED(f32x4, smem_v)
    const int C = a.C, r = R > 0 ? R : a.r, pgw = r, tid = threadIdx.x, lane = tid & 63, wv = wave_id_uniform(), nwl = a.wpg, win0 = blockIdx.x * nwl;
    const PgLds s = pg_lds(reinterpret_cast<float*>(smem_v), C, r, true, a.stage_wdn != 0);
    const int nct = C / 16;
    const int colA[1] = {wv * 16}, colB[1] = {(wv + 4) * 16};
    f32x4 wfa[8][1], wfb[8][1];
    if (wv < nct) pg_load_chunk<1, true>(wfa, a.Wprompt, C, C, 128, colA, 0, 128);
    if (wv + 4 < nct) pg_load_chunk<1, true>(wfb, a.Wprompt, C, C, 128, colB, 0, 128);
    const FastDiv byC(C), byR(r);
#pragma unroll 4
    for (int i = tid; i < nwl * C; i += 256) {
        const int w = byC.div(i), c = i - w * C;
        s.dg[w * s.LDC + c] = win0 + w < a.nW ? a.dgate[(long)(win0 + w) * C + c] : 0.f;
    }
    pg_forward_chain<true, R>(a, s, win0);
    PG_MARK(7);
    const float sc = rsqrtf((float)r);
    if (wv * 16 < r) {
        f32x4 acc = {0, 0, 0, 0};
        for (int kc = 0; kc < C; kc += 16)
            mma(acc, load_frag_tr<float>(s.Wup, s.RP, wv * 16, kc), load_frag<float>(s.dg, s.LDC, 0, kc));
        const int w = lane & 15, rr = wv * 16 + (lane >> 4) * 4;
        for (int j = 0; j < 4; ++j)
            if (rr + j < r) s.sm[w * PG_SMW + PG_DO2 + rr + j] = acc[j];
    }
    __syncthreads();
    PG_MARK(8);
    for (int i = tid; i < nwl * r; i += 256) {
        const int w = byR.div(i), m = i - w * r;
        const float* do2 = s.sm + w * PG_SMW + PG_DO2;
        float acc = 0.f;
        for (int j = 0; j < r; ++j) acc += s.Wpp[j * s.RP + m] * do2[j];
        s.sm[w * PG_SMW + PG_DO + m] = acc;
    }
    __syncthreads();
    PG_MARK(9);
    for (int i = tid; i < nwl * r; i += 256) {
        const int w = byR.div(i), m = i - w * r;
        const float* A = s.At + w * s.LDA + m * s.RP;
        const float* kv = s.sm + w * PG_SMW + PG_KV;
        const float dov = s.sm[w * PG_SMW + PG_DO + m];
        float rs = 0.f;
        for (int j = 0; j < r; ++j) rs += A[j] * dov * kv[r + j];
        float acc = 0.f;
        for (int j = 0; j < r; ++j) acc += A[j] * (dov * kv[r + j] - rs) * kv[j];
        s.sm[w * PG_SMW + PG_DQ + m] = acc * sc;
        s.sm[w * PG_SMW + PG_RS + m] = rs;
    }
    __syncthreads();
    PG_MARK(10);
    for (int i = tid; i < nwl * r; i += 256) {
        const int w = byR.div(i), j = i - w * r;
        const float* sm = s.sm + w * PG_SMW;
        const float vj = sm[PG_KV + r + j];
        float dk = 0.f, dv = 0.f;
        for (int m = 0; m < r; ++m) {
            const float A = s.At[w * s.LDA + m * s.RP + j], dov = sm[PG_DO + m];
            dk += A * (dov * vj - sm[PG_RS + m]) * sm[PG_Q + m];
            dv += A * dov;
        }
        s.sm[w * PG_SMW + PG_DKV + j] = dk * sc;
        s.sm[w * PG_SMW + PG_DKV + r + j] = dv;
    }
    __syncthreads();
    PG_MARK(11);
    for (int i = tid; i < nwl * r; i += 256) {
        const int w = byR.div(i), j = i - w * r;
        const float* dkv = s.sm + w * PG_SMW + PG_DKV;
        const float* dq = s.sm + w * PG_SMW + PG_DQ;
        float acc = 0.f, acc2 = 0.f;
        for (int m = 0; m < 2 * r; ++m) acc += s.Wkv[m * s.RP + j] * dkv[m];
        for (int m = 0; m < r; ++m) acc2 += s.Wq[m * s.RP + j] * dq[m];
        s.sm[w * PG_SMW + PG_DD + j] = acc;
        s.sm[w * PG_SMW + PG_DS + j] = acc2;
    }
    __syncthreads();
    PG_MARK(12);
    for (int i = tid; i < nwl * 128; i += 256) {
        const int w = i >> 7, p = i & 127;
        const float* ds = s.sm + w * PG_SMW + PG_DS;
        float acc = 0.f;
        for (int j = 0; j < r; ++j) acc += s.P[p * s.RP + j] * ds[j];
        s.dl[w * s.LDW + p] = acc;
    }
    __syncthreads();
    PG_MARK(13);
    for (int ww = 0; ww < 4; ++ww) {
        const int w = wv * 4 + ww;
        if (w >= nwl) break;
        const float w0 = s.w[w * s.LDW + lane], w1 = s.w[w * s.LDW + lane + 64];
        const float d0 = s.dl[w * s.LDW + lane], d1 = s.dl[w * s.LDW + lane + 64];
        const float tot = wave_sum(w0 * d0 + w1 * d1);
        s.dl[w * s.LDW + lane] = w0 * (d0 - tot);
        s.dl[w * s.LDW + lane + 64] = w1 * (d1 - tot);
    }
    __syncthreads();
    PG_MARK(14);
    for (int ct = wv; ct < nct; ct += 4) {
        f32x4 acc[1] = {{0, 0, 0, 0}};
        const int col0[1] = {ct * 16};
        if (ct == wv) pg_mma_chunk<1>(acc, wfa, s.dl, s.LDW, 0, 128);
        else if (ct == wv + 4) pg_mma_chunk<1>(acc, wfb, s.dl, s.LDW, 0, 128);
        else {
            f32x4 wf[8][1];
            pg_load_chunk<1, true>(wf, a.Wprompt, C, C, 128, col0, 0, 128);
            pg_mma_chunk<1>(acc, wf, s.dl, s.LDW, 0, 128);
        }
        const int w = lane & 15, c0 = ct * 16 + (lane >> 4) * 4;
        const float* dd = s.sm + w * PG_SMW + PG_DD;
        const float* wdn = a.stage_wdn ? s.Wdn : a.Wdown;
        for (int m = 0; m < r; ++m) {
            const f32x4 wd = *reinterpret_cast<const f32x4*>(wdn + (long)m * C + c0);
            for (int j = 0; j < 4; ++j) acc[0][j] += wd[j] * dd[m];
        }
        if (w < nwl && win0 + w < a.nW) *reinterpret_cast<f32x4*>(a.dmu + (long)(win0 + w) * C + c0) = acc[0];
    }
    PG_MARK(15);
    auto put = [&](void* base, long idx, float v) __attribute__((always_inline)) {
        if (a.lr_bf16 == MPHSIR_BF16) reinterpret_cast<bf16_t*>(base)[idx] = (bf16_t)v;
        else if (a.lr_bf16 == MPHSIR_F16) reinterpret_cast<f16_t*>(base)[idx] = (f16_t)v;
        else reinterpret_cast<float*>(base)[idx] = v;
    };
    for (int w = wv; w < nwl && win0 + w < a.nW; w += 4) {
        const float* sm = s.sm + w * PG_SMW;
        const long L0 = (long)(win0 + w) * a.KL, R0 = (long)(win0 + w) * a.KR;
        for (int c = lane; c < C; c += 64) { put(a.L, L0 + c, s.dg[w * s.LDC + c]); put(a.R, R0 + 5 * r + 1 + c, s.mu[w * s.LDC + c]); }
        for (int c = lane; c < 128; c += 64) { put(a.L, L0 + C + 4 * r + c, s.w[w * s.LDW + c]); put(a.L, L0 + C + 4 * r + 128 + c, s.dl[w * s.LDW + c]); }
        if (lane < r) {
            put(a.L, L0 + C + lane, sm[PG_DO2 + lane]);
            put(a.L, L0 + C + 3 * r + lane, sm[PG_DQ + lane]);
            put(a.L, L0 + C + 4 * r + 256 + lane, sm[PG_DD + lane]);
            put(a.R, R0 + lane, sm[PG_O2 + lane]);
            put(a.R, R0 + r + lane, sm[PG_O + lane]);
            put(a.R, R0 + 2 * r + 1 + lane, sm[PG_D + lane]);
            put(a.R, R0 + 3 * r + 1 + lane, sm[PG_S + lane]);
            put(a.R, R0 + 4 * r + 1 + lane, sm[PG_DS + lane]);
        }
        if (lane < 2 * r) put(a.L, L0 + C + r + lane, sm[PG_DKV + lane]);
        if (lane == 0) put(a.R, R0 + 2 * r, 1.f);
        for (int c = C + 5 * r + 256 + lane; c < a.KL; c += 64) put(a.L, L0 + c, 0.f);
        for (int c = 5 * r + 1 + C + lane; c < a.KR; c += 64) put(a.R, R0 + c, 0.f);
    }
    PG_MARK(16);
}

}

namespace mphsir {
static int pg_windows_per_wg(int nW) {
    int w = PG_NWIN;
    while (w > 2 && (nW + w / 2 - 1) / (w / 2) <= 256) w /= 2;
    return w;
}
void pg_debug_buffer(unsigned long long* p) { g_pg_dbg = p; }
}

extern "C" int mphsir_pg_gate_fwd(const mphsir_pg_fwd_args* a, void* stream) {
    using namespace mphsir;
    clear_error();
    MPHSIR_CHECK_ARGS(a, "pg_gate_fwd");
    MPHSIR_REQUIRE(a && a->mu && a->Wprompt && a->prompt_param && a->Wq && a->Wkv && a->Wdown && a->Wpproj && a->bpproj && a->Wup && a->gate,
                   "pg_gate_fwd: null pointer");
    MPHSIR_REQUIRE(a->nW > 0 && a->C > 0 && a->C % 16 == 0 && a->r > 0 && a->r <= PG_RMAX, "pg_gate_fwd: need C %% 16 == 0 and 0 < r <= 32");
    PgDev d{a->mu, nullptr, a->Wprompt, a->prompt_param, a->Wq, a->Wkv, a->Wdown, a->Wpproj, a->bpproj, a->Wup, a->gate, nullptr, nullptr,
            nullptr, a->nW, a->C, a->r, 0, 0, 0, 0, pg_windows_per_wg(a->nW), g_pg_dbg};
    const size_t shmem = pg_lds_bytes(a->C, a->r, false);
    MPHSIR_REQUIRE(shmem <= 160 * 1024, "pg_gate_fwd: (C=%d, r=%d) needs %d bytes of LDS", a->C, a->r, (int)shmem);
    const dim3 grid((a->nW + d.wpg - 1) / d.wpg);
    hipStream_t s = reinterpret_cast<hipStream_t>(stream);
#define MPHSIR_PG_FWD(R_)                                                                        \
    do {                                                                                         \
        allow_big_lds(pg_gate_fwd_kernel<R_>, shmem);                                            \
        MPHSIR_LAUNCH(MPHSIR_K_PG_GATE, pg_gate_fwd_kernel<R_>, grid, dim3(256), shmem, s, d);    \
        return MPHSIR_OK;                                                                        \
    } while (0)
    if (a->r == 8) MPHSIR_PG_FWD(8);
    if (a->r == 12) MPHSIR_PG_FWD(12);
    if (a->r == 16) MPHSIR_PG_FWD(16);
    if (a->r == 24) MPHSIR_PG_FWD(24);
    MPHSIR_PG_FWD(0);
#undef MPHSIR_PG_FWD
}

extern "C" int mphsir_pg_gate_bwd(const mphsir_pg_bwd_args* a, void* stream) {
    using namespace mphsir;
    clear_error();
    MPHSIR_CHECK_ARGS(a, "pg_gate_bwd");
    MPHSIR_REQUIRE(a && a->mu && a->dgate && a->Wprompt && a->prompt_param && a->Wq && a->Wkv && a->Wdown && a->Wpproj && a->bpproj &&
                       a->Wup && a->dmu && a->L && a->R, "pg_gate_bwd: null pointer");
    MPHSIR_REQUIRE(a->nW > 0 && a->C > 0 && a->C % 16 == 0 && a->r > 0 && a->r <= PG_RMAX, "pg_gate_bwd: need C %% 16 == 0 and 0 < r <= 32");
    MPHSIR_REQUIRE(a->KL >= a->C + 5 * a->r + 256 && a->KR >= 5 * a->r + 1 + a->C, "pg_gate_bwd: factor widths too small");
    MPHSIR_REQUIRE(!a->lr_bf16 || (a->KL % 8 == 0 && a->KR % 8 == 0), "pg_gate_bwd: bf16 factor rows need KL, KR multiples of 8");
    PgDev d{a->mu, a->dgate, a->Wprompt, a->prompt_param, a->Wq, a->Wkv, a->Wdown, a->Wpproj, a->bpproj, a->Wup, nullptr, a->dmu, a->L, a->R,
            a->nW, a->C, a->r, a->KL, a->KR, a->lr_bf16, 0, pg_windows_per_wg(a->nW), g_pg_dbg};
    d.stage_wdn = pg_lds_bytes(a->C, a->r, true, true) <= 160 * 1024 ? 1 : 0;
    const size_t shmem = pg_lds_bytes(a->C, a->r, true, d.stage_wdn != 0);
    MPHSIR_REQUIRE(shmem <= 160 * 1024, "pg_gate_bwd: (C=%d, r=%d) needs %d bytes of LDS", a->C, a->r, (int)shmem);
    const dim3 grid((a->nW + d.wpg - 1) / d.wpg);
    hipStream_t s = reinterpret_cast<hipStream_t>(stream);
#define MPHSIR_PG_BWD(R_)                                                                            \
    do {                                                                                             \
        allow_big_lds(pg_gate_bwd_kernel<R_>, shmem);                                                \
        MPHSIR_LAUNCH(MPHSIR_K_PG_GATE_BWD, pg_gate_bwd_kernel<R_>, grid, dim3(256), shmem, s, d);    \
        return MPHSIR_OK;                                                                            \
    } while (0)
    if (a->r == 8) MPHSIR_PG_BWD(8);
    if (a->r == 12) MPHSIR_PG_BWD(12);
    if (a->r == 16) MPHSIR_PG_BWD(16);
    if (a->r == 24) MPHSIR_PG_BWD(24);
    MPHSIR_PG_BWD(0);
#undef MPHSIR_PG_BWD
}
```

mp-hsir_amd/ops.py:

```python
import ctypes
import os
import weakref

import torch

from . import _lib

_DT = {torch.float32: 0, torch.bfloat16: 1, torch.float16: 2}
_HALF = (torch.bfloat16, torch.float16)

ACCOUNT = None


def _acct(name, flops, nbytes):
    if ACCOUNT is not None:
        a = ACCOUNT.setdefault(name, [0, 0.0, 0.0])
        a[0] += 1
        a[1] += flops
        a[2] += nbytes


def _p(t):
    return None if t is None else ctypes.c_void_p(t.data_ptr())


def _stream(t):
    if t.is_cuda:
        return ctypes.c_void_p(torch.cuda.current_stream(t.device).cuda_stream)
    return None


def _check(*tensors):
    emu = _lib.is_emulated()
    for t in tensors:
        if t is None:
            continue
        if emu and t.is_cuda:
            raise RuntimeError("mp-hsir_amd: emulated test library bound but got a GPU tensor")
        if not emu and not t.is_cuda:
            raise RuntimeError("mp-hsir_amd: ops run on the GPU only (got a CPU tensor; there is no CPU fallback)")


_SIDE = {}
SIDE_BRANCH = os.environ.get("MPHSIR_SIDE_BRANCH", "1") == "1"
PROMPT_SIDE = os.environ.get("MPHSIR_PROMPT_SIDE", "1") == "1"
_SIDE_USED = set()


class side_stream:

    def __init__(self, like, enabled=True, name="gate", track=True):
        self.on = enabled and like.is_cuda
        self.ctx = None
        self.track = track
        if self.on:
            dev = like.device
            self.main = torch.cuda.current_stream(dev)
            self.side = _SIDE.get((dev, name))
            if self.side is None:
                self.side = _SIDE[(dev, name)] = torch.cuda.Stream(dev)

    def __enter__(self):
        if self.on:
            self.side.wait_stream(self.main)
            if self.track:
                _SIDE_USED.add((self.main.device, self.side))
            self.ctx = torch.cuda.stream(self.side)
            self.ctx.__enter__()
        return self

    def __exit__(self, *exc):
        if self.on:
            self.ctx.__exit__(*exc)
        return False

    def join(self, *tensors):
        if self.on:
            self.main.wait_stream(self.side)
            for t in tensors:
                if t is not None:
                    t.record_stream(self.main)


_SCOPE = None


_DEFERRED = None


class reduce_scope:

    def __init__(self, leaf=False):
        self.leaf = leaf

    def __enter__(self):
        global _SCOPE
        self.prev, self.segs, self.gemms, self.calls = _SCOPE, [], [], []
        _SCOPE = self
        return self

    def __exit__(self, *exc):
        global _SCOPE
        _SCOPE = self.prev
        if exc[0] is None:
            if self.leaf and _DEFERRED is not None and DW_SIDE and _dw_side(self):
                pass
            elif self.leaf and _DEFERRED is not None:
                _flush_calls(self.calls)
                _flush_gemms(self.gemms)
                for g in self.segs:
                    g["keep"] = (g["keep"][0], g["keep"][1].detach())
                _poison(self.segs)
                _DEFERRED.extend(self.segs)
            else:
                _flush_calls(self.calls)
                _flush_gemms(self.gemms)
                _flush(self.segs)
        self.segs, self.gemms, self.calls = [], [], []
        return False


DW_SIDE = int(os.environ.get("MPHSIR_DW_SIDE", "2"))
_DW_STREAM = {}
_DW_KEEP = []


DEBUG_DEFERRED = os.environ.get("MPHSIR_DEBUG_DEFERRED", "0") == "1"


def _poison(segs):
    if DEBUG_DEFERRED:
        for g in segs:
            g["keep"][1].fill_(float("nan"))


def _dw_side(scope):
    like = None
    for g in scope.gemms + scope.segs:
        like = g["keep"][0]
        break
    if like is None or not like.is_cuda:
        return False
    dev = like.device
    st = _DW_STREAM.get(dev)
    if st is None:
        st = _DW_STREAM[dev] = torch.cuda.Stream(dev)
    main = torch.cuda.current_stream(dev)
    for g in scope.segs:
        g["keep"] = (g["keep"][0], g["keep"][1].detach())
    _poison(scope.segs)
    if DW_SIDE >= 2:
        nbytes = sum(g["M"] * (g["N1"] + g["N2"]) * 2 for g in scope.gemms)
        rows = max([g["M"] for g in scope.gemms] + [c["keep"][0].shape[0] for c in scope.calls if c["keep"][0].dim() == 2] + [0])
        if DW_DEFER and rows >= DW_DEFER_ROWS:
            _DW_HELD.setdefault(dev, []).append((scope.gemms, scope.calls, scope.segs))
            return True
        if DW_DEFER and rows > 0:
            _dw_release_held(dev)
        pend = _DW_PENDING.setdefault(dev, [[], [], [], 0])
        pend[0] += scope.gemms
        pend[1] += scope.calls
        pend[2] += scope.segs
        pend[3] += nbytes
        if scope.calls or pend[3] >= DW_BATCH_BYTES or len(pend[0]) + 3 > _lib.TN_GROUP_MAX or len(pend[2]) + 17 > _lib.REDUCE_MAX_SEGS:
            _dw_flush_pending(dev)
        return True
    else:
        _flush_calls(scope.calls)
        _flush_gemms(scope.gemms)
        st.wait_stream(main)
        for d2, s2 in list(_SIDE_USED):
            if d2 == dev and s2 != st:
                st.wait_stream(s2)
        with torch.cuda.stream(st):
            _flush(scope.segs)
    _DW_KEEP.append((dev, [g["keep"] for g in scope.gemms] + [c["keep"] for c in scope.calls], [g["keep"] for g in scope.segs]))
    return True


DW_BATCH_BYTES = int(float(os.environ.get("MPHSIR_DW_BATCH_MB", "256")) * (1 << 20))
_DW_PENDING = {}
DW_DEFER = os.environ.get("MPHSIR_DW_DEFER", "0") == "1"
DW_DEFER_ROWS = int(os.environ.get("MPHSIR_DW_DEFER_ROWS", "65536"))
_DW_HELD = {}
DW_SUMS_LATE = os.environ.get("MPHSIR_DW_SUMS_LATE", "0") == "1"
_DW_SUMS = {}


def _dw_release_held(dev):
    held = _DW_HELD.get(dev)
    if not held:
        return
    _dw_flush_pending(dev)
    _DW_HELD[dev] = []
    for gemms, calls, segs in held:
        _DW_PENDING[dev] = [list(gemms), list(calls), list(segs), 0]
        _dw_flush_pending(dev)


def _dw_flush_pending(dev):
    pend = _DW_PENDING.get(dev)
    if not pend or not (pend[0] or pend[1] or pend[2]):
        return
    gemms, calls, segs = pend[0], pend[1], pend[2]
    _DW_PENDING[dev] = [[], [], [], 0]
    st = _DW_STREAM[dev]
    st.wait_stream(torch.cuda.current_stream(dev))
    for d2, s2 in list(_SIDE_USED):
        if d2 == dev and s2 != st:
            st.wait_stream(s2)
    with torch.cuda.stream(st):
        _flush_calls(calls)
        _flush_gemms(gemms)
        if DW_SUMS_LATE:
            _DW_SUMS.setdefault(dev, []).extend(segs)
        else:
            _flush(segs)
    _DW_KEEP.append((dev, [g["keep"] for g in gemms] + [c["keep"] for c in calls], [g["keep"] for g in segs]))


def _dw_join(final=True):
    for dev in list(_DW_HELD):
        _dw_release_held(dev)
    for dev in list(_DW_PENDING):
        _dw_flush_pending(dev)
    for dev, segs in list(_DW_SUMS.items()):
        if segs:
            _DW_SUMS[dev] = []
            with torch.cuda.stream(_DW_STREAM[dev]):
                _flush(segs)
    if _DW_KEEP:
        for dev in {k[0] for k in _DW_KEEP}:
            torch.cuda.current_stream(dev).wait_stream(_DW_STREAM[dev])
        if final:
            del _DW_KEEP[:]
    for dev, st in list(_SIDE_USED):
        torch.cuda.current_stream(dev).wait_stream(st)
    if final:
        _SIDE_USED.clear()


class deferred_reductions:

    def __enter__(self):
        global _DEFERRED
        self.prev = _DEFERRED
        _DEFERRED = []
        if self.prev is None:
            _SIDE_USED.clear()
        return self

    def __exit__(self, *exc):
        global _DEFERRED
        segs, _DEFERRED = _DEFERRED, self.prev
        if exc[0] is None:
            _flush(segs)
        _dw_join()
        return False


def flush_deferred():
    if _DEFERRED:
        segs = _DEFERRED[:]
        del _DEFERRED[:]
        _flush(segs)
    _dw_join(final=False)


LOG_SEGS = os.environ.get("MPHSIR_LOG_SEGS", "0") == "1"


def _flush_calls(calls):
    for c in calls:
        c["run"]()


def _flush_gemms(gemms):
    lib = _lib.load()
    for i in range(0, len(gemms), _lib.TN_GROUP_MAX):
        chunk = gemms[i:i + _lib.TN_GROUP_MAX]
        k0 = chunk[0]["keep"][0]
        assert all(g["keep"][0].dtype == k0.dtype and g["keep"][0].device == k0.device for g in chunk), "grouped token-reduction GEMMs of mixed dtype / device"
        arr = (_lib.TnProblem * len(chunk))()
        for k, g in enumerate(chunk):
            q = arr[k]
            q.A, q.lda, q.B, q.ldb, q.Cpart, q.colsum_part = g["A"], g["lda"], g["B"], g["ldb"], g["Cpart"], g["cs"]
            q.M, q.N1, q.N2, q.nsplit = g["M"], g["N1"], g["N2"], g["nsplit"]
        form = TN_FORM or (2 if all(g["form"] == 2 for g in chunk) else 1)
        if LOG_SEGS:
            print("gemm_tn_group form %d:" % form, [(g["M"], g["N1"], g["N2"], g["nsplit"], g["cs"] is not None) for g in chunk], flush=True)
        _lib.check(lib.mphsir_gemm_tn_group(arr, len(chunk), form, _DT[chunk[0]["keep"][0].dtype], _stream(chunk[0]["keep"][0])), "gemm_tn_group")


def _flush(segs):
    lib = _lib.load()
    for i in range(0, len(segs), _lib.REDUCE_MAX_SEGS):
        chunk = segs[i:i + _lib.REDUCE_MAX_SEGS]
        arr = (_lib.ReduceSeg * len(chunk))()
        nbytes = 0.0
        for k, g in enumerate(chunk):
            a = arr[k]
            a.src, a.dst = g["src"], g["dst"]
            a.n, a.stride, a.src_batch_stride, a.dst_batch_stride = g["n"], g["stride"], g["sbs"], g["dbs"]
            a.nsplit, a.nbatch, a.rows, a.dst_col_stride = g["nsplit"], g["nbatch"], g["rows"], g["dcs"]
            a.src_ld, a.dst_ld = g["src_ld"], g["dst_ld"]
            nbytes += 4.0 * g["nbatch"] * max(1, g["rows"]) * g["n"] * (g["nsplit"] + 1)
        _lib.check(lib.mphsir_reduce_parts(arr, len(chunk), _stream(chunk[0]["keep"][0])), "reduce_parts")
        _acct("reduce_parts", nbytes / 4.0, nbytes)
        if LOG_SEGS:
            print("reduce_parts %.1f MB:" % (nbytes / 1e6), [(g["n"], g["rows"], g["nsplit"], g["nbatch"], g["dcs"], g["src"] % 16 == 0 and g["stride"] % 4 == 0) for g in chunk], flush=True)


def _submit(seg, immediate):
    if _SCOPE is None or immediate:
        _flush([seg])
    else:
        _SCOPE.segs.append(seg)


def reduce_parts(part, batched=False, immediate=False):
    _check(part)
    assert part.dtype == torch.float32
    if batched:
        Bt, nsplit, shape = part.shape[0], part.shape[1], tuple(part.shape[2:])
        sbs, sst = part.stride(0), part.stride(1)
    else:
        Bt, nsplit, shape = 1, part.shape[0], tuple(part.shape[1:])
        sbs, sst = 0, part.stride(0)
    n = 1
    for d in shape:
        n *= d
    assert part[0, 0].is_contiguous() if batched else part[0].is_contiguous()
    if nsplit == 1 and (not batched or Bt == 1 or sbs == n):
        return part[:, 0] if batched else part[0]
    out = torch.empty(((Bt,) + shape) if batched else shape, dtype=torch.float32, device=part.device)
    _submit(dict(src=part.data_ptr(), dst=out.data_ptr(), n=n, stride=sst, sbs=sbs, dbs=n, nsplit=nsplit, nbatch=Bt,
                 rows=1, dcs=1, src_ld=0, dst_ld=0, keep=(part, out)), immediate)
    return out


def reduce_block(part, r0, nr, c0, nc, out, transpose=False, immediate=False):
    _check(part, out)
    assert part.dtype == torch.float32 and part.dim() == 3 and part[0].is_contiguous() and out.dtype == torch.float32
    nsplit, R, Cc = part.shape
    assert 0 <= r0 and r0 + nr <= R and 0 <= c0 and c0 + nc <= Cc and out.dim() == 2
    if transpose:
        assert tuple(out.shape) == (nc, nr) and out.stride(1) == 1
        dst_ld, dcs = 1, out.stride(0)
    else:
        assert tuple(out.shape) == (nr, nc) and out.stride(1) == 1
        dst_ld, dcs = out.stride(0), 1
    _submit(dict(src=part.data_ptr() + 4 * (r0 * Cc + c0), dst=out.data_ptr(), n=nc, stride=part.stride(0), sbs=0, dbs=0, nsplit=nsplit,
                 nbatch=1, rows=max(nr, 1), dcs=dcs, src_ld=Cc, dst_ld=dst_ld, keep=(part, out)), immediate)
    if nr == 1:
        pass
    return out


def pack_gather(arena, index, dtype, out=None):
    lib = _lib.load()
    _check(arena, index, out)
    assert arena.dtype == torch.float32 and index.dtype == torch.int32 and arena.is_contiguous() and index.is_contiguous()
    n = index.numel()
    if out is None:
        out = torch.empty((n,), dtype=dtype, device=arena.device)
    assert out.numel() == n and out.dtype == dtype and out.is_contiguous()
    _lib.check(lib.mphsir_pack_gather(_p(arena), _p(index), _p(out), n, _DT[dtype], _stream(arena)), "pack_gather")
    _acct("pack_gather", 0.0, n * (8.0 + out.element_size()))
    return out


class MultiCopy:
    BLOCK = 4096

    def __init__(self, device, capacity, ring=4):
        self.device, self.capacity, self.ring = device, capacity, ring
        self.host = [torch.empty((capacity, 4), dtype=torch.int64).pin_memory() if device.type == "cuda" else torch.empty((capacity, 4), dtype=torch.int64)
                     for _ in range(ring)]
        self.dev = [torch.empty((capacity, 4), dtype=torch.int64, device=device) for _ in range(ring)]
        self.events = [None] * ring
        self.turn = 0
        pin = device.type == "cuda"
        self.for_capture = [(torch.empty((capacity, 4), dtype=torch.int64).pin_memory() if pin else torch.empty((capacity, 4), dtype=torch.int64),
                             torch.empty((capacity, 4), dtype=torch.int64, device=device)) for _ in range(24)]
        self.captured = []

    def __call__(self, dsts, srcs):
        n = len(dsts)
        if n == 0:
            return
        assert n <= self.capacity
        capturing = self.device.type == "cuda" and torch.cuda.is_current_stream_capturing()
        if capturing:
            if not self.for_capture:
                torch._foreach_copy_(list(dsts), list(srcs))
                return
            h, dv = self.for_capture.pop()
            self.captured.append((h, dv))
        else:
            k = self.turn
            self.turn = (k + 1) % self.ring
            if self.events[k] is not None:
                self.events[k].synchronize()
            h, dv = self.host[k], self.dev[k]
        rows, blk = [], 0
        for d, s_ in zip(dsts, srcs):
            ne = d.numel()
            rows.append((s_.data_ptr(), d.data_ptr(), ne, blk))
            blk += (ne + self.BLOCK - 1) // self.BLOCK
        h[:n] = torch.tensor(rows, dtype=torch.int64)
        dv[:n].copy_(h[:n], non_blocking=True)
        _lib.check(_lib.load().mphsir_multi_copy(_p(dv), n, blk, _stream(dv)), "multi_copy")
        if self.device.type == "cuda" and not capturing:
            self.events[k] = torch.cuda.Event()
            self.events[k].record()
        _acct("multi_copy", 0.0, 8.0 * sum(d.numel() for d in dsts))


class _L1ClampLoss(torch.autograd.Function):

    @staticmethod
    def forward(ctx, y, clean):
        lib = _lib.load()
        _check(y, clean)
        y, clean = y.contiguous(), clean.contiguous()
        assert y.dtype == torch.float32 and clean.dtype == torch.float32 and y.shape == clean.shape
        n = y.numel()
        nblk = max(1, min(1024, (n + 1023) // 1024))
        need = ctx.needs_input_grad[0]
        g = torch.empty_like(y) if need else None
        part = torch.empty((nblk, 1), dtype=torch.float32, device=y.device)
        _lib.check(lib.mphsir_l1_clamp_loss(_p(y), _p(clean), _p(g), _p(part), n, nblk, _stream(y)), "l1_clamp_loss")
        _acct("l1_clamp_loss", 4.0 * n, 4.0 * n * (3 if need else 2))
        ctx.g = g
        return reduce_parts(part, immediate=True).reshape(())

    @staticmethod
    def backward(ctx, dloss):
        g, ctx.g = ctx.g, None
        assert g is not None, "l1_clamp_loss: its gradient buffer is scaled in place and handed over: backward() runs once"
        return g.mul_(dloss), None


def l1_clamp_loss(y, clean):
    return _L1ClampLoss.apply(y, clean)


def l1_clamp_loss_grad(y, clean):
    lib = _lib.load()
    _check(y, clean)
    y, clean = y.contiguous(), clean.contiguous()
    assert y.dtype == torch.float32 and clean.dtype == torch.float32 and y.shape == clean.shape
    n = y.numel()
    nblk = max(1, min(1024, (n + 1023) // 1024))
    g = torch.empty_like(y)
    part = torch.empty((nblk, 1), dtype=torch.float32, device=y.device)
    _lib.check(lib.mphsir_l1_clamp_loss(_p(y), _p(clean), _p(g), _p(part), n, nblk, _stream(y)), "l1_clamp_loss")
    _acct("l1_clamp_loss", 4.0 * n, 12.0 * n)
    return reduce_parts(part, immediate=True).reshape(()), g


def _rows(t):
    assert t.dim() == 2 and t.stride(1) == 1, "expected a row-major 2-D view"
    return t.shape[0], t.stride(0)


TOK_FORM = int(os.environ.get("MPHSIR_TOK_FORM", "0"))


def gemm_tok(x, w, bias=None, ln=None, epi=0, res=None, sa=None, gate=None, keep=None, geom=None, out=None):
    lib = _lib.load()
    _check(x, w, bias, res, sa, gate, keep)
    M, ldx = _rows(x)
    K = x.shape[1]
    per_sample = w.dim() == 3
    N = w.shape[-2]
    assert w.shape[-1] == K and w.is_contiguous() and w.dtype == x.dtype, (w.shape, K, w.dtype, x.dtype)
    y = out if out is not None else torch.empty((M, N), dtype=x.dtype, device=x.device)
    a = _lib.GemmArgs()
    a.X, a.ldx = _p(x), ldx
    a.W = _p(w)
    a.w_batch_stride = N * K if per_sample else 0
    a.rows_per_batch = M // w.shape[0] if per_sample else 0
    a.bias = _p(bias)
    if ln is not None:
        a.ln_w, a.ln_b = _p(ln[0]), _p(ln[1])
    a.Y, a.ldy = _p(y), _rows(y)[1]
    a.M, a.N, a.K, a.epi = M, N, K, epi
    if res is not None:
        a.R, a.ldr = _p(res), _rows(res)[1]
    if sa is not None:
        a.SA, a.ldsa = _p(sa), _rows(sa)[1]
    a.gate, a.keep = _p(gate), _p(keep)
    if geom is not None:
        a.H, a.Wimg, a.shift = geom
    a.form = TOK_FORM
    _lib.check(lib.mphsir_gemm_tok(ctypes.byref(a), _DT[x.dtype], _stream(x)), "gemm_tok")
    es = x.element_size()
    _acct("gemm_tok", 2.0 * M * N * K, (M * K + M * N * (1 + (res is not None) + (sa is not None))) * es + w.numel() * es)
    return y





def layernorm_tok(x, ln_w, ln_b, out_dtype, want_cast=False):
    lib = _lib.load()
    _check(x, ln_w, ln_b)
# ... 210 lines not shown
    B, C, H, W = clean.shape
    want = {"b": (B,), "bc": (B, C), "bcn": (B, C, W), "k": (len(plan.ksize), 21, 21), "bnn": (B, H, W), "c": (C,)}
    for (name, dt, shp), t in zip(_DEG_TABLES, tabs):
        assert t is None or (t.dtype == dt and tuple(t.shape) == want[shp] and t.is_contiguous() and t.device == clean.device), \
            "degrade_batch: plan.%s must be a contiguous %s tensor of shape %s on %s" % (name, dt, want[shp], clean.device)
    for t in dr:
        assert t is None or (t.dtype == torch.float32 and t.shape == clean.shape and t.is_contiguous() and t.device == clean.device), \
            "degrade_batch: explicit draws are contiguous fp32 cubes of the batch's shape"
    if od is not None:
        assert od.dtype == torch.int64 and od.numel() == 1 and od.device == clean.device, "degrade_batch: a device ordinal is one int64"
    if out is None:
        out = (torch.empty_like(clean), torch.empty_like(clean))
    for t in out:
        assert t.shape == clean.shape and t.dtype == torch.float32 and t.is_contiguous() and t.device == clean.device
    assert out[0].data_ptr() != out[1].data_ptr() and clean.data_ptr() not in (out[0].data_ptr(), out[1].data_ptr()), "degrade_batch: distinct cubes"
    host = [(ctypes.c_int32 * max(len(v), 1))(*v) for v in (plan.menu, plan.ksize, plan.sr_factor)]
    a = _lib.DegradeArgs(clean=_p(clean), degraded=_p(out[0]), clean_aug=_p(out[1]), menu=ctypes.addressof(host[0]),
                         ksize=ctypes.addressof(host[1]) if plan.ksize else None, sr_factor=ctypes.addressof(host[2]) if plan.sr_factor else None,
                         z=_p(dr[0]), u0=_p(dr[1]), u1=_p(dr[2]), ordinal_dev=_p(od), seed=ctypes.c_int64(int(seed) & 0xFFFFFFFFFFFFFFFF).value,
                         ordinal=0 if od is not None else int(ordinal), B=B, C=C, H=H, W=W, T=len(plan.menu), K=len(plan.ksize),
                         F=len(plan.sr_factor), **{n: _p(t) for (n, _, _), t in zip(_DEG_TABLES, tabs)})
    _lib.check(lib.mphsir_degrade_batch(ctypes.byref(a), _stream(clean)), "degrade_batch")
    _acct("degrade", 0.0, 12.0 * clean.numel())
    return out


def round_up(n, m):
    return (n + m - 1) // m * m


def pack_gated_mlp(fc1_w, fc1_b, fc2_w, dtype):
    two_hid, C = fc1_w.shape
    hid = two_hid // 2
    HP = round_up(hid, 32)
    W1 = torch.zeros((2 * HP, C), dtype=cdt(dtype), device=fc1_w.device)
    W1[:hid] = fc1_w[:hid].to(cdt(dtype))
    W1[HP:HP + hid] = fc1_w[hid:].to(cdt(dtype))
    b1 = torch.zeros((2 * HP,), dtype=torch.float32, device=fc1_w.device)
    b1[:hid] = fc1_b[:hid]
    b1[HP:HP + hid] = fc1_b[hid:]
    W2 = torch.zeros((C, HP), dtype=cdt(dtype), device=fc1_w.device)
    W2[:, :hid] = fc2_w.to(cdt(dtype))
    return W1, b1, W2




BASE_SKIP_FUSED = os.environ.get("MPHSIR_BASE_SKIP_FUSED", "1") == "1"
BASE_SKIP_TRAIN = os.environ.get("MPHSIR_BASE_SKIP_TRAIN", "1") == "1"
BASE_SKIP_BWD = os.environ.get("MPHSIR_BASE_SKIP_BWD", "1") == "1"
MLP_HSPLIT = os.environ.get("MPHSIR_MLP_HSPLIT", "1") == "1"


def mlp_hsplit(M, C, HP):
    if not MLP_HSPLIT or C < 192 or M // 64 >= 256:
        return 1
    s, chunks = 1, HP // 32
    while (M // 64) * s * 2 <= 256 and chunks % (s * 2) == 0:
        s *= 2
    return s


MLP_FUSE_SUM = os.environ.get("MPHSIR_MLP_FUSE_SUM", "1") == "1"
MLP_FUSE_MIN_TILES = int(os.environ.get("MPHSIR_MLP_FUSE_MIN_TILES", "256"))


def gated_mlp_fuses(M, C, HW, dtype):
    return (MLP_FUSE_SUM and dtype in _HALF and HW % 128 == 0 and M // 128 >= MLP_FUSE_MIN_TILES
            and bool(_lib.load().mphsir_gated_mlp_fwd_fuses(C, M, _DT[dtype])))


def gated_mlp_fwd(x, ln_w, ln_b, W1, b1, W2, b2, keep=None, rows_per_batch=0, out=None, tiles_per_wave=0, hsplit=None, res=None, branch=None):
    lib = _lib.load()
    _check(x, W1, W2, b1, b2, ln_w, ln_b, keep, res)
    M, ldx = _rows(x)
    C = x.shape[1]
    HP = W2.shape[1]
    assert W1.shape == (2 * HP, C) and W1.dtype == x.dtype and W2.dtype == x.dtype
    y = out if out is not None else torch.empty((M, C), dtype=x.dtype, device=x.device)
    a = _lib.MlpArgs()
    a.X, a.ldx, a.ln_w, a.ln_b = _p(x), ldx, _p(ln_w), _p(ln_b)
    a.W1, a.b1, a.W2, a.b2 = _p(W1), _p(b1), _p(W2), _p(b2)
    a.keep, a.rows_per_batch = _p(keep), rows_per_batch
    if res is not None:
        assert res.shape == x.shape and res.dtype == x.dtype
        a.R, a.ldr = _p(res), _rows(res)[1]
    a.Y, a.ldy, a.M, a.C, a.HP, a.tiles_per_wave = _p(y), _rows(y)[1], M, C, HP, tiles_per_wave
    yb = None
    if branch is not None:
        v, Mb, sa, gate = branch["v"], branch["Mb"], branch["sa"], branch["gate"]
        H, W, shift = branch["geom"]
        _check(v, Mb, sa, gate, branch.get("keep"))
        assert x.dtype in _HALF and (H * W) % 128 == 0 and lib.mphsir_gated_mlp_fwd_fuses(C, M, _DT[x.dtype]) and Mb.dim() == 3 and Mb.shape[1:] == (C, C) and Mb.is_contiguous() and M == Mb.shape[0] * H * W
        assert v.dtype == x.dtype and sa.dtype == x.dtype and gate.dtype == torch.float32 and gate.is_contiguous() and hsplit in (None, 1)
        a.PV, a.ldpv, a.PM, a.pm_batch_stride = _p(v), _rows(v)[1], _p(Mb), C * C
        a.PSA, a.ldpsa, a.pgate, a.pkeep = _p(sa), _rows(sa)[1], _p(gate), _p(branch.get("keep"))
        a.H, a.Wimg, a.shift = H, W, shift
        if branch.get("want_y"):
            yb = torch.empty((M, C), dtype=x.dtype, device=x.device)
            a.Yb, a.ldyb = _p(yb), C
        hsplit = 1
    if hsplit is None:
        hsplit = mlp_hsplit(M, C, HP) if tiles_per_wave == 0 and (x.dtype in _HALF or C < 256) else 1
    if hsplit > 1:
        ypart = torch.empty((hsplit, M, C), dtype=torch.float32, device=x.device)
        a.hsplit, a.ypart, a.tiles_per_wave = hsplit, _p(ypart), 1
    _lib.check(lib.mphsir_gated_mlp_fwd(ctypes.byref(a), _DT[x.dtype], _stream(x)), "gated_mlp_fwd")
    es = x.element_size()
    if branch is not None:
        _acct("gated_mlp", 6.0 * M * C * HP + 2.0 * M * C * C, (4.0 + (1.0 if yb is not None else 0.0)) * M * C * es + 3.0 * C * HP * es)
        return y, yb
    _acct("gated_mlp", 6.0 * M * C * HP, 2.0 * M * C * es + 3.0 * C * HP * es)
    return y


def pack_win_proj(proj_w, heads, dtype):
    C = proj_w.shape[0]
    hd = C // heads
    hdp = _lib.load().mphsir_win_attn_hdp(hd, _DT[dtype])
    if hdp == hd:
        return proj_w.to(cdt(dtype)).contiguous()
    out = torch.zeros((C, heads, hdp), dtype=cdt(dtype), device=proj_w.device)
    out[:, :, :hd] = proj_w.reshape(C, heads, hd).to(cdt(dtype))
    return out.reshape(C, heads * hdp)


def win_attn_fwd(x, ln_w, ln_b, Wqkv, bqkv, rpb, Wproj, bproj, pg, heads, shift, save=False, gate=True):
    lib = _lib.load()
    _check(x, Wqkv, Wproj, *pg.values())
    B, H, W, C = x.shape
    assert x.is_contiguous() and Wqkv.shape == (3 * C, C) and Wqkv.dtype == x.dtype and Wproj.dtype == x.dtype
    sa = torch.empty_like(x)
    mu = torch.empty((B * (H // 8) * (W // 8), C), dtype=torch.float32, device=x.device)
    a = _lib.WinAttnArgs()
    a.X, a.ln_w, a.ln_b = _p(x), _p(ln_w), _p(ln_b)
    a.Wqkv, a.bqkv, a.rpb, a.Wproj, a.bproj = _p(Wqkv), _p(bqkv), _p(rpb), _p(Wproj), _p(bproj)
    a.SA, a.mu = _p(sa), _p(mu)
    oattn = None
    if save:
        oattn = torch.empty_like(x)
        a.Oattn = _p(oattn)
    a.B, a.H, a.W, a.C, a.heads, a.shift = B, H, W, C, heads, shift
    _lib.check(lib.mphsir_win_attn_fwd(ctypes.byref(a), _DT[x.dtype], _stream(x)), "win_attn_fwd")
    M = B * H * W
    _acct("win_attn", M * (8.0 * C * C + 4.0 * 64 * C), 2.0 * M * C * x.element_size() + mu.numel() * 4 + 4.0 * C * C * x.element_size())
    if not gate:
        return sa, mu, oattn
    gate = pg_gate_fwd(mu, pg)
    if save:
        return sa, gate, mu, oattn
    return sa, gate


def pg_gate_fwd(mu, pg):
    lib = _lib.load()
    _check(mu, *pg.values())
    nW, C = mu.shape
    r = pg["linear_down.weight"].shape[0]
    gate = torch.empty_like(mu)
    a = _lib.PgFwdArgs()
    a.mu, a.gate = _p(mu), _p(gate)
    a.Wprompt, a.prompt_param = _p(pg["linear_prompt.weight"]), _p(pg["prompt_param"])
    a.Wq, a.Wkv, a.Wdown = _p(pg["q.weight"]), _p(pg["kv.weight"]), _p(pg["linear_down.weight"])
    a.Wpproj, a.bpproj, a.Wup = _p(pg["proj.weight"]), _p(pg["proj.bias"]), _p(pg["linear_up.weight"])
    a.nW, a.C, a.r = nW, C, r
    _lib.check(lib.mphsir_pg_gate_fwd(ctypes.byref(a), _stream(mu)), "pg_gate_fwd")
    _acct("pg_gate", 2.0 * nW * C * (128 + 2 * r), 4.0 * nW * 2 * C)
    return gate


def pack_dw(w):
    return w.reshape(w.shape[0], 9).t().contiguous().float()


def choose_nsplit(B, H, W):
    tiles = H * W // 64
    n = tiles
    while n > 1 and B * n > 1024 and n % 2 == 0:
        n //= 2
    return n


def dwconv_gram(tq, tk, tv, wq, wk, wv, ldw, B, H, W, C, heads, nsplit=None, keep_qk=False):
    lib = _lib.load()
    _check(tq, tk, tv, wq, wk, wv)
    M = B * H * W
    nsplit = nsplit or choose_nsplit(B, H, W)
    hd = C // heads
    v = torch.empty((M, C), dtype=tq.dtype, device=tq.device)
    gp = torch.empty((B, nsplit, heads, hd, hd), dtype=torch.float32, device=tq.device)
    sp = torch.empty((B, nsplit, 2, C), dtype=torch.float32, device=tq.device)
    a = _lib.GramArgs()
    a.Tq, a.ldq, a.Tk, a.ldk, a.Tv, a.ldv = _p(tq), tq.stride(0), _p(tk), tk.stride(0), _p(tv), tv.stride(0)
    a.wq, a.wk, a.wv, a.ldw = _p(wq), _p(wk), _p(wv), ldw
    a.V, a.ldvo, a.Gpart, a.Spart = _p(v), C, _p(gp), _p(sp)
    a.B, a.H, a.W, a.C, a.heads, a.nsplit = B, H, W, C, heads, nsplit
    qk = None
    if keep_qk and lib.mphsir_dwconv_gram_keeps_qk(C, W, _DT[tq.dtype]):
        qk = torch.empty((M, 2 * C), dtype=tq.dtype, device=tq.device)
        a.QK, a.ldqk = _p(qk), 2 * C
    _lib.check(lib.mphsir_dwconv_gram(ctypes.byref(a), _DT[tq.dtype], _stream(tq)), "dwconv_gram")
    _acct("dwconv_gram", M * (54.0 * C + 2.0 * C * hd), (4.0 + (2.0 if qk is not None else 0.0)) * M * C * tq.element_size() + gp.numel() * 4 + sp.numel() * 4)
    _acct("dwconv_gram:qk", 2.0 * M * C * hd, 0.0)
    if keep_qk:
        return v, gp, sp, nsplit, qk
    return v, gp, sp, nsplit


FUSED_TRAIN = os.environ.get("MPHSIR_FUSED_TRAIN", "1") == "1"


def qkv_dwconv_gram_fits(C, heads, H, W, dtype):
    return bool(_lib.load().mphsir_qkv_dwconv_gram_fits(C, heads, H, W, _DT[dtype]))


FUSED_WGS = 512


def fused_wgs(C):
    return 256 if C >= 256 else FUSED_WGS


def choose_nsplit_fused(B, H, W, C=0):
    n = (H // 8) * (W // 16)
    while n > 1 and B * n > fused_wgs(C) and n % 2 == 0:
        n //= 2
    return n


def choose_head_groups(B, nsplit, heads, C=0):
    g = 1
    while g < heads and heads % (2 * g) == 0 and B * nsplit * 2 * g <= fused_wgs(C):
        g *= 2
    return g


def qkv_dwconv_gram_rows_fits(C, heads, H, W, dtype, ln=False):
    return bool(_lib.load().mphsir_qkv_dwconv_gram_rows_fits(C, heads, H, W, _DT[dtype], int(bool(ln))))


ROWS_FORM = os.environ.get("MPHSIR_ROWS_FORM", "1") == "1"


def choose_row_segments(B, H, W, C, heads):
    hgroups = max(1, heads // (2 if C // heads == 32 else 1))
    s = 1
    while B * (W // 32) * s * hgroups < 256 and H % (2 * s) == 0 and H // (2 * s) >= 4:
        s *= 2
    return s


def qkv_dwconv_gram(x, wqkv, w9, B, H, W, C, heads, ln=None, nsplit=None, head_groups=None, keep=False, row_segments=None):
    lib = _lib.load()
    _check(x, wqkv, w9)
    M, ldx = _rows(x)
    assert M == B * H * W and wqkv.shape == (3 * C, C) and wqkv.is_contiguous() and wqkv.dtype == x.dtype
    if row_segments is None:
        row_segments = 0
        if ROWS_FORM and nsplit is None and head_groups is None and qkv_dwconv_gram_rows_fits(C, heads, H, W, x.dtype, ln is not None):
            row_segments = choose_row_segments(B, H, W, C, heads)
    if row_segments:
        nsplit = (W // 32) * row_segments
    nsplit = nsplit or choose_nsplit_fused(B, H, W, C)
    hd = C // heads
    v = torch.empty((M, C), dtype=x.dtype, device=x.device)
    gp = torch.empty((B, nsplit, heads, hd, hd), dtype=torch.float32, device=x.device)
    sp = torch.empty((B, nsplit, 2, C), dtype=torch.float32, device=x.device)
    a = _lib.FusedGramArgs()
    a.X, a.ldx, a.Wqkv, a.w9, a.ldw = _p(x), ldx, _p(wqkv), _p(w9), w9.stride(0)
    if ln is not None:
        a.ln_w, a.ln_b = _p(ln[0]), _p(ln[1])
    a.V, a.ldvo, a.Gpart, a.Spart = _p(v), C, _p(gp), _p(sp)
    a.B, a.H, a.W, a.C, a.heads, a.nsplit = B, H, W, C, heads, nsplit
    a.head_groups = 1 if row_segments else (head_groups or choose_head_groups(B, nsplit, heads, C))
    a.row_segments = row_segments
    t = qk = None
    if keep:
        t = torch.empty((M, 3 * C), dtype=x.dtype, device=x.device)
        qk = torch.empty((M, 2 * C), dtype=x.dtype, device=x.device)
        a.T, a.ldt, a.QK, a.ldqk = _p(t), 3 * C, _p(qk), 2 * C
    _lib.check(lib.mphsir_qkv_dwconv_gram(ctypes.byref(a), _DT[x.dtype], _stream(x)), "qkv_dwconv_gram")
    _acct("qkv_dwconv_gram", M * (6.0 * C * C + 54.0 * C + 2.0 * C * hd), (7.0 if keep else 2.0) * M * C * x.element_size()
          + wqkv.numel() * x.element_size() + gp.numel() * 4 + sp.numel() * 4)
    _acct("qkv_dwconv_gram:qk", 2.0 * M * C * hd, 0.0)
    _acct("qkv_dwconv_gram:rows" if row_segments else "qkv_dwconv_gram:tile", 0.0, 0.0)
    if keep:
        return v, gp, sp, nsplit, t, qk
    return v, gp, sp, nsplit


def spectral_fold(gp, sp, temperature, Wo, dtype, transposed=False):
    lib = _lib.load()
    _check(gp, sp, temperature, Wo)
    B, nsplit, heads, hd, _ = gp.shape
    C = heads * hd
    assert Wo.dtype == torch.float32 and Wo.is_contiguous() and temperature.is_contiguous()
    if nsplit > 64:
        with reduce_scope():
            gp = reduce_parts(gp, batched=True)
            sp = reduce_parts(sp, batched=True)
        gp, sp = gp.unsqueeze(1), sp.unsqueeze(1)
        nsplit = 1
    Mo = torch.empty((B, C, C), dtype=dtype, device=gp.device)
    a = _lib.FoldArgs()
    a.Gpart, a.Spart, a.temperature, a.Wo, a.M = _p(gp), _p(sp), _p(temperature), _p(Wo), _p(Mo)
    MT = torch.empty_like(Mo) if transposed else None
    a.MT = _p(MT)
    gsum = ssum = None
    if transposed:
        gsum = torch.empty((B, 1, heads, hd, hd), dtype=torch.float32, device=gp.device)
        ssum = torch.empty((B, 1, 2, C), dtype=torch.float32, device=gp.device)
        a.Gsum, a.Ssum = _p(gsum), _p(ssum)
    a.B, a.C, a.heads, a.nsplit = B, C, heads, nsplit
    _lib.check(lib.mphsir_spectral_fold(ctypes.byref(a), _DT[dtype], _stream(gp)), "spectral_fold")
    _acct("spectral_fold", 2.0 * B * C * C * hd, gp.numel() * 4 + sp.numel() * 4 + C * C * 4 + Mo.numel() * Mo.element_size())
    return (Mo, MT, gsum, ssum) if transposed else Mo


def dwconv_gate(t, w9, B, H, W):
    lib = _lib.load()
    _check(t, w9)
# ... 451 lines not shown
                resident = 2 if (N1 > 64 and N2 > 64) else (4 if (N1 <= 64 and N2 <= 64) else 3)
                nsplit = max(1, min(M // 256, 128, max(1, int(256 * resident * TN_BIG_ROUNDS) // tiles)))
        else:
            ts = 128 if tile128 else 64
            tiles = ((N1 + ts - 1) // ts) * ((N2 + ts - 1) // ts) * Bt
            nsplit = max(1, min(M // 512, 64, max(1, 768 // tiles)))
        if TN_PART_CAP > 0:
            cap = int(TN_PART_CAP * M * (N1 + N2) * a.element_size() / (N1 * N2 * 4.0))
            nsplit = max(1, (M + 4095) // 4096, min(nsplit, cap))
    part = torch.empty((Bt, nsplit, N1, N2), dtype=torch.float32, device=a.device)
    cs = torch.empty((Bt, nsplit, N1), dtype=torch.float32, device=a.device) if colsum else None
    if _SCOPE is not None and TN_GROUPED and not immediate and not batched and tile128 and a.dtype in _HALF:
        _SCOPE.gemms.append(dict(A=a.data_ptr(), lda=a.stride(-2), B=b.data_ptr(), ldb=b.stride(-2), Cpart=part.data_ptr(),
                                 cs=cs.data_ptr() if colsum else None, M=M, N1=N1, N2=N2, nsplit=nsplit, form=form,
                                 keep=(a, b, part, cs)))
    else:
        _lib.check(lib.mphsir_gemm_tn(_p(a), a.stride(-2), a.stride(0) if batched else 0, _p(b), b.stride(-2),
                                      b.stride(0) if batched else 0, _p(part), _p(cs), M, N1, N2, nsplit, Bt,
                                      (form if a.dtype in _HALF else 1) if tile128 else 0,
                                      _DT[a.dtype], _stream(a)),
                   "gemm_tn")
    _acct("gemm_tn", 2.0 * Bt * M * N1 * N2, Bt * M * (N1 + N2) * a.element_size())
    _acct("gemm_tn:partials", 0.0, part.numel() * 4.0)
    if not reduce:
        return (part, cs) if colsum else part
    out = reduce_parts(part, batched=True, immediate=immediate)
    out = out if batched else out[0]
    if colsum:
        c = reduce_parts(cs, batched=True, immediate=immediate)
        return out, (c if batched else c[0])
    return out


def gemm_tn_blocks(a, b, row_ranges, ncols=None, colsum=False):
    N2 = b.shape[-1]
    ncols = N2 if ncols is None else ncols
    res = gemm_tn(a, b, colsum=colsum, reduce=False)
    part, cs = (res if colsum else (res, None))
    rows = sum(nr for _, nr in row_ranges)
    out = torch.empty((rows, ncols), dtype=torch.float32, device=a.device)
    outc = torch.empty((1, rows), dtype=torch.float32, device=a.device) if colsum else None
    o = 0
    for r0, nr in row_ranges:
        reduce_block(part[0], r0, nr, 0, ncols, out[o:o + nr])
        if colsum:
            reduce_block(cs[0].unsqueeze(1), 0, 1, r0, nr, outc[:, o:o + nr])
        o += nr
    return (out, outc[0]) if colsum else out


def gdfn_gate_bwd(t, du):
    lib = _lib.load()
    _check(t, du)
    M, HP = du.shape
    assert t.shape == (M, 2 * HP) and t.is_contiguous() and du.is_contiguous()
    u, dt_ = torch.empty_like(du), torch.empty_like(t)
    _lib.check(lib.mphsir_gdfn_gate_bwd(_p(t), _p(du), _p(u), _p(dt_), M, HP, _DT[t.dtype], _stream(t)), "gdfn_gate_bwd")
    _acct("gdfn_gate_bwd", 30.0 * M * HP, 7.0 * M * HP * t.element_size())
    return u, dt_


def dwconv_gate_bwd(t, w9, du, B, H, W):
    lib = _lib.load()
    _check(t, w9, du)
    M, HP = du.shape
    assert t.shape == (M, 2 * HP) and t.is_contiguous() and du.is_contiguous() and M == B * H * W
    if not lib.mphsir_dwconv_gate_bwd_fits(H, W, HP, _DT[t.dtype]):
        return gdfn_gate_bwd(dwconv3x3(t.reshape(B, H, W, 2 * HP), w9).reshape(M, 2 * HP), du)
    u, dt_ = torch.empty_like(du), torch.empty_like(t)
    _lib.check(lib.mphsir_dwconv_gate_bwd(_p(t), _p(w9), w9.stride(0), _p(du), _p(u), _p(dt_), B, H, W, HP, _DT[t.dtype], _stream(t)), "dwconv_gate_bwd")
    _acct("gdfn_gate_bwd", 66.0 * M * HP, 6.0 * M * HP * t.element_size())
    return u, dt_


FOLD_BWD_DM_MAX_TOKENS = int(os.environ.get("MPHSIR_FOLD_BWD_DM_TOKENS", "1024"))


def fold_bwd_forms_dm(N, C, heads, dtype):
    return dtype in _HALF and 0 < N <= FOLD_BWD_DM_MAX_TOKENS and N % 64 == 0 and (C // heads) in (32, 48, 64)


GDFN_DW_BWD = os.environ.get("MPHSIR_GDFN_DW_BWD", "0") == "1"
GDFN_DW_BWD_WGS = int(os.environ.get("MPHSIR_GDFN_DW_BWD_WGS", "2048"))


def gdfn_dw_bwd_fits(H, W, HP, dtype):
    return GDFN_DW_BWD and dtype in _HALF and bool(_lib.load().mphsir_gdfn_dw_bwd_fits(H, W, HP, _DT[dtype]))


def gdfn_dw_bwd(t, w9, du, B, H, W, nblk=None, round_mid=False):
    lib = _lib.load()
    _check(t, w9, du)
    M, HP = du.shape
    assert t.shape == (M, 2 * HP) and t.is_contiguous() and du.is_contiguous() and M == B * H * W and w9.shape == (9, 2 * HP) and w9.stride(1) == 1
    nslab = HP // 16
    tiles = B * (H // 8) * (W // 16)
    if nblk is None:
        nblk = max(1, min(tiles, GDFN_DW_BWD_WGS // nslab))
        if nblk >= 8:
            nblk = nblk // 8 * 8
    u = torch.empty((M, HP), dtype=t.dtype, device=t.device)
    dt = torch.empty((M, 2 * HP), dtype=t.dtype, device=t.device)
    part = torch.empty((nblk, 9, 2 * HP), dtype=torch.float32, device=t.device)
    _lib.check(lib.mphsir_gdfn_dw_bwd(_p(t), _p(w9), w9.stride(0), _p(du), _p(u), _p(dt), _p(part), nblk, B, H, W, HP, int(round_mid),
                                      _DT[t.dtype], _stream(t)), "gdfn_dw_bwd")
    _acct("gdfn_gate_bwd", M * HP * (40.0 + 72.0), (2.0 * 1.9 + 1.4 + 1.0 + 2.0) * M * HP * t.element_size())
    return u, dt, part


def spectral_fold_bwd(gp, sp, temperature, Wo, dM, dtype, reduce=True, d_out=None, v=None, dm_scale=None, w2_blocks=False):
    lib = _lib.load()
    B, nsplit, heads, hd, _ = gp.shape
    C = heads * hd
    if dM is None:
        _check(gp, sp, temperature, Wo, d_out, v)
        N = d_out.shape[0] // B
        assert d_out.shape == (B * N, C) and v.shape == (B * N, C) and d_out.dtype == dtype and v.dtype == dtype and d_out.stride(1) == 1 and v.stride(1) == 1
        assert fold_bwd_forms_dm(N, C, heads, dtype)
        W2 = torch.empty((B, 2 * C, 2 * C), dtype=dtype, device=gp.device)
        dWo = torch.empty((B, C, C), dtype=torch.float32, device=gp.device)
        dtemp = torch.empty((B, heads), dtype=torch.float32, device=gp.device)
        a = _lib.FoldBwdArgs()
        a.Gpart, a.Spart, a.temperature, a.Wo = _p(gp), _p(sp), _p(temperature), _p(Wo)
        a.W2, a.dWo, a.dtemp = _p(W2), _p(dWo), _p(dtemp)
        a.B, a.C, a.heads, a.nsplit, a.dM_nsplit = B, C, heads, nsplit, 0
        a.DO, a.lddo, a.V, a.ldv, a.N = _p(d_out), d_out.stride(0), _p(v), v.stride(0), N
        a.dm_scale = _p(dm_scale)
        a.w2_blocks = 1 if w2_blocks else 0
        _lib.check(lib.mphsir_spectral_fold_bwd(ctypes.byref(a), _DT[dtype], _stream(gp)), "spectral_fold_bwd")
        _acct("spectral_fold_bwd", 4.0 * B * C * C * hd + 2.0 * B * N * C * C, 3.0 * B * C * C * 4 + 2.0 * B * N * C * d_out.element_size())
        _acct("spectral_fold_bwd:dm", 0.0, 0.0)
        if not reduce:
            return W2, dWo, dtemp
        return W2, reduce_parts(dWo), reduce_parts(dtemp)
    _check(gp, sp, temperature, Wo, dM)
    dm_nsplit = dM.shape[1] if dM.dim() == 4 else 1
    assert dM.shape[0] == B and dM.shape[-2:] == (C, C) and dM.dtype == torch.float32 and dM.is_contiguous()
    W2 = torch.empty((B, 2 * C, 2 * C), dtype=dtype, device=gp.device)
    dWo = torch.empty((B, C, C), dtype=torch.float32, device=gp.device)
    dtemp = torch.empty((B, heads), dtype=torch.float32, device=gp.device)
    a = _lib.FoldBwdArgs()
    a.Gpart, a.Spart, a.temperature, a.Wo, a.dM = _p(gp), _p(sp), _p(temperature), _p(Wo), _p(dM)
    a.W2, a.dWo, a.dtemp = _p(W2), _p(dWo), _p(dtemp)
    a.B, a.C, a.heads, a.nsplit, a.dM_nsplit = B, C, heads, nsplit, dm_nsplit
    a.dm_scale = _p(dm_scale)
    a.w2_blocks = 1 if w2_blocks else 0
    _lib.check(lib.mphsir_spectral_fold_bwd(ctypes.byref(a), _DT[dtype], _stream(gp)), "spectral_fold_bwd")
    _acct("spectral_fold_bwd", 4.0 * B * C * C * hd, 3.0 * B * C * C * 4)
    if not reduce:
        return W2, dWo, dtemp
    return W2, reduce_parts(dWo), reduce_parts(dtemp)


def pg_gate_bwd(mu, dgate, pg, factor_dtype=torch.float32):
    lib = _lib.load()
    _check(mu, dgate, *pg.values())
    nW, C = mu.shape
    r = pg["linear_down.weight"].shape[0]
    KL, KR = round_up(C + 5 * r + 256, 8), round_up(5 * r + 1 + C, 8)
    dmu = torch.empty_like(mu)
    L = torch.empty((nW, KL), dtype=factor_dtype, device=mu.device)
    R = torch.empty((nW, KR), dtype=factor_dtype, device=mu.device)
    a = _lib.PgBwdArgs()
    a.mu, a.dgate = _p(mu), _p(dgate)
    a.Wprompt, a.prompt_param = _p(pg["linear_prompt.weight"]), _p(pg["prompt_param"])
    a.Wq, a.Wkv, a.Wdown = _p(pg["q.weight"]), _p(pg["kv.weight"]), _p(pg["linear_down.weight"])
    a.Wpproj, a.bpproj, a.Wup = _p(pg["proj.weight"]), _p(pg["proj.bias"]), _p(pg["linear_up.weight"])
    a.dmu, a.L, a.R = _p(dmu), _p(L), _p(R)
    a.nW, a.C, a.r, a.KL, a.KR, a.lr_bf16 = nW, C, r, KL, KR, _DT[factor_dtype]
    _lib.check(lib.mphsir_pg_gate_bwd(ctypes.byref(a), _stream(mu)), "pg_gate_bwd")
    _acct("pg_gate_bwd", 4.0 * nW * C * (128 + 2 * r), 4.0 * nW * (2 * C + KL + KR))
    part = gemm_tn(L, R, reduce=False)[0]
    blocks = {
        "linear_up.weight": (0, C, 0, r),
        "proj.weight": (C, r, r, r),
        "proj.bias": (C, r, 2 * r, 1),
        "kv.weight": (C + r, 2 * r, 2 * r + 1, r),
        "q.weight": (C + 3 * r, r, 3 * r + 1, r),
        "prompt_param": (C + 4 * r, 128, 4 * r + 1, r),
        "linear_prompt.weight": (C + 4 * r + 128, 128, 5 * r + 1, C),
        "linear_down.weight": (C + 4 * r + 256, r, 5 * r + 1, C),
    }
    g = {k: reduce_block(part, r0, nr, c0, nc, torch.empty((nr, nc), dtype=torch.float32, device=mu.device))
         for k, (r0, nr, c0, nc) in blocks.items()}
    g["proj.bias"] = g["proj.bias"].reshape(r)
    return dmu, g


def pack_conv3x3(w, dtype, flip_transpose=False):
    if flip_transpose:
        w = w.flip(2, 3).transpose(0, 1)
    Co, Ci = w.shape[0], w.shape[1]
    Np, Cp = round_up(Co, 16), round_up(Ci, 32)
    out = torch.zeros((Np, 9, Cp), dtype=cdt(dtype), device=w.device)
    out[:Co, :, :Ci] = w.permute(0, 2, 3, 1).reshape(Co, 9, Ci).to(cdt(dtype))
    return out.reshape(Np, 9 * Cp)


def pixel_pitch(t):
    B, H, W, C = t.shape
    ld = t.stride(2)
    ok = t.stride(3) == 1 and ld >= C and t.stride(1) == W * ld and t.stride(0) == H * W * ld and (ld * t.element_size()) % 16 == 0 and t.data_ptr() % 16 == 0
    return ld if ok else None


def conv3x3_tok(x, wp, out=None):
    lib = _lib.load()
    _check(x, wp, out)
    B, H, W, Cp = x.shape
    Np = wp.shape[0]
    ldx = pixel_pitch(x)
    assert ldx is not None and wp.shape[1] == 9 * Cp and wp.dtype == x.dtype
    y = out if out is not None else torch.empty((B, H, W, Np), dtype=x.dtype, device=x.device)
    ldy = pixel_pitch(y)
    assert ldy is not None and y.shape == (B, H, W, Np) and y.dtype == x.dtype
    _lib.check(lib.mphsir_conv3x3_tok(_p(x), ldx, _p(wp), _p(y), ldy, B, H, W, Cp, Np, _DT[x.dtype], _stream(x)), "conv3x3_tok")
    _acct("conv3x3_tok", 18.0 * B * H * W * Cp * Np, (B * H * W * (Cp + Np) + wp.numel()) * x.element_size())
    return y


def conv3x3_wgrad(dy2, x, nsplit=None, cout=None, cin=None):
    lib = _lib.load()
    _check(dy2, x)
    B, H, W, Cp = x.shape
    M, Np = dy2.shape
    assert x.is_contiguous() and dy2.stride(1) == 1 and M == B * H * W and x.dtype == dy2.dtype and x.dtype in _HALF
    if nsplit is None:
        tiles = ((Np + 127) // 128 if Np > 64 else 1) * ((9 * Cp + 127) // 128)
        nsplit = max(1, min(M // 256, 128, max(1, (TN_RING_WGS if TN_FORM == 2 else int(256 * 2 * TN_BIG_ROUNDS)) // tiles)))
    part = torch.empty((1, nsplit, Np, 9 * Cp), dtype=torch.float32, device=x.device)
    _lib.check(lib.mphsir_conv3x3_wgrad(_p(dy2), dy2.stride(0), _p(x), Cp, _p(part), B, H, W, Np, Cp, nsplit, TN_FORM or 1, _DT[x.dtype],
                                        _stream(x)), "conv3x3_wgrad")
    _acct("gemm_tn", 2.0 * M * Np * 9 * Cp, M * (Np + Cp) * x.element_size())
    _acct("gemm_tn:partials", 0.0, part.numel() * 4.0)
    if cout is None:
        return reduce_parts(part, batched=True, immediate=True)[0]
    assert cout <= Np and cin <= Cp
    out = torch.empty((cout, cin, 3, 3), dtype=torch.float32, device=x.device)
    _submit(dict(src=part.data_ptr(), dst=out.data_ptr(), n=cin, stride=part.stride(1), sbs=9 * Cp, dbs=cin * 9, nsplit=part.shape[1], nbatch=cout,
                 rows=9, dcs=9, src_ld=Cp, dst_ld=1, keep=(part, out)), False)
    return out


def im2col3x3(x):
    lib = _lib.load()
    _check(x)
    B, H, W, Cp = x.shape
    assert x.is_contiguous()
    col = torch.empty((B * H * W, 9 * Cp), dtype=x.dtype, device=x.device)
    _lib.check(lib.mphsir_im2col3x3(_p(x), Cp, _p(col), B, H, W, Cp, _DT[x.dtype], _stream(x)), "im2col3x3")
    _acct("im2col3x3", 0.0, 10.0 * x.numel() * x.element_size())
    return col
```

Before: 1725 patches/s.

## Save prompt-gate forward state for backward and reduce weight grads via direct products

```diff
diff --git a/include/mphsir.h b/include/mphsir.h
--- a/include/mphsir.h
+++ b/include/mphsir.h
@@ -56,8 +56,10 @@
     const float* Wpproj; const float* bpproj; const float* Wup;
     float* gate;
     int32_t nW, C, r;
+    float* state;
 } mphsir_pg_fwd_args;
 int mphsir_pg_gate_fwd(const mphsir_pg_fwd_args* a, void* stream);
+int32_t mphsir_pg_state_width(int32_t r);
 int mphsir_win_attn_fwd(const mphsir_win_attn_args* a, int dtype, void* stream);
 int mphsir_win_attn_hdp(int head_dim, int dtype);
 
@@ -224,6 +226,7 @@
     float* dmu; void* L; void* R;
     int32_t nW, C, r, KL, KR;
     int32_t lr_bf16;
+    const float* state;
 } mphsir_pg_bwd_args;
 int mphsir_pg_gate_bwd(const mphsir_pg_bwd_args* a, void* stream);
 
@@ -394,6 +397,8 @@
     int32_t nsplit, nbatch;
     int32_t rows, dst_col_stride;
     int64_t src_ld, dst_ld;
+    const float* mul;
+    int64_t mul_stride;
 } mphsir_reduce_seg;
 int mphsir_reduce_parts(const mphsir_reduce_seg* segs, int32_t nseg, void* stream);
 
diff --git a/mp-hsir_amd/_lib.py b/mp-hsir_amd/_lib.py
--- a/mp-hsir_amd/_lib.py
+++ b/mp-hsir_amd/_lib.py
@@ -46,7 +46,7 @@
 
 class PgFwdArgs(_Args):
     _fields_ = _SZ + [(n, c_void_p) for n in ("mu", "Wprompt", "prompt_param", "Wq", "Wkv", "Wdown", "Wpproj", "bpproj", "Wup", "gate")] + \
-               [(n, c_int32) for n in ("nW", "C", "r")]
+               [(n, c_int32) for n in ("nW", "C", "r")] + [("state", c_void_p)]
 
 
 class GramArgs(_Args):
@@ -105,7 +105,8 @@
 
 class PgBwdArgs(_Args):
     _fields_ = _SZ + [(n, c_void_p) for n in ("mu", "dgate", "Wprompt", "prompt_param", "Wq", "Wkv", "Wdown", "Wpproj", "bpproj", "Wup",
-                                         "dmu", "L", "R")] + [(n, c_int32) for n in ("nW", "C", "r", "KL", "KR", "lr_bf16")]
+                                         "dmu", "L", "R")] + [(n, c_int32) for n in ("nW", "C", "r", "KL", "KR", "lr_bf16")] + \
+               [("state", c_void_p)]
 
 
 class SpectralBwdArgs(_Args):
@@ -155,7 +156,7 @@
 class ReduceSeg(ctypes.Structure):
     _fields_ = [("src", c_void_p), ("dst", c_void_p), ("n", c_int64), ("stride", c_int64), ("src_batch_stride", c_int64),
                 ("dst_batch_stride", c_int64), ("nsplit", c_int32), ("nbatch", c_int32), ("rows", c_int32),
-                ("dst_col_stride", c_int32), ("src_ld", c_int64), ("dst_ld", c_int64)]
+                ("dst_col_stride", c_int32), ("src_ld", c_int64), ("dst_ld", c_int64), ("mul", c_void_p), ("mul_stride", c_int64)]
 
 
 REDUCE_MAX_SEGS = 32
@@ -180,6 +181,7 @@
     "mphsir_win_attn_fwd": (c_int, [ctypes.POINTER(WinAttnArgs), c_int, c_void_p]),
     "mphsir_win_attn_hdp": (c_int, [c_int, c_int]),
     "mphsir_pg_gate_fwd": (c_int, [ctypes.POINTER(PgFwdArgs), c_void_p]),
+    "mphsir_pg_state_width": (c_int32, [c_int32]),
     "mphsir_dwconv_gram": (c_int, [ctypes.POINTER(GramArgs), c_int, c_void_p]),
     "mphsir_dwconv_gram_keeps_qk": (c_int, [c_int32, c_int32, c_int]),
     "mphsir_qkv_dwconv_gram": (c_int, [ctypes.POINTER(FusedGramArgs), c_int, c_void_p]),
diff --git a/mp-hsir_amd/autograd_ops.py b/mp-hsir_amd/autograd_ops.py
--- a/mp-hsir_amd/autograd_ops.py
+++ b/mp-hsir_amd/autograd_ops.py
@@ -175,7 +175,7 @@
     sa, mu, oattn = ops.win_attn_fwd(x, pk["ln1"][0], pk["ln1"][1], pk["wqkv"], pk["bqkv"], pk["rpb"], pk["wproj"],
                                      pk["bproj"], pk["pg"], heads, shift, save=True, gate=False)
     with ops.side_stream(sa, ops.SIDE_BRANCH) as br:
-        gate = ops.pg_gate_fwd(mu, pk["pg"])
+        gate, pgst = ops.pg_gate_fwd(mu, pk["pg"], keep_state=True)
     sa2 = sa.reshape(-1, Cc)
     if ops.FUSED_TRAIN and ops.qkv_dwconv_gram_fits(Cc, heads, H, W, dt):
         v, gp, spart, _, t, qk = ops.qkv_dwconv_gram(sa2, sp["wqkv"], w9, B, H, W, Cc, heads, keep=True)
@@ -185,7 +185,7 @@
                                               3 * Cc, B, H, W, Cc, heads, keep_qk=True)
     Mb, MbT, gp, spart = ops.spectral_fold(gp, spart, sp["temp"], sp["wo"], dt, transposed=True)
     br.join()
-    saved = (x, sa, gate, mu, oattn, t, v, gp, spart, Mb, MbT) + ((qk,) if qk is not None else ())
+    saved = (x, sa, gate, mu, oattn, t, v, gp, spart, Mb, MbT, pgst) + ((qk,) if qk is not None else ())
     if fuse:
         return None, saved
     y = ops.gemm_tok(v, Mb, epi=2, res=x.reshape(-1, Cc), sa=sa2, gate=gate, keep=k1, geom=(H, W, shift))
@@ -193,8 +193,8 @@
 
 
 def _pgsstb_attn_backward(blk, k1, saved, dy, extra=None):
-    x, sa, gate, mu, oattn, t, v, gp, spart, Mb, MbT = saved[:11]
-    qk = saved[11] if len(saved) > 11 else None
+    x, sa, gate, mu, oattn, t, v, gp, spart, Mb, MbT, pgst = saved[:12]
+    qk = saved[12] if len(saved) > 12 else None
     B, H, W, Cc = x.shape
     dt = x.dtype
     M = B * H * W
@@ -208,13 +208,13 @@
         if lean:
             with ops.side_stream(dy, ops.SIDE_BRANCH) as br:
                 _, d_sa, dgate = ops.combine_bwd(dy, sa, gate, k1, shift, want_dout=False)
-                dmu, gpg = ops.pg_gate_bwd(mu, dgate, pk["pg"], factor_dtype=torch.float32 if f32_factors else dt)
+                dmu, gpg = ops.pg_gate_bwd(mu, dgate, pk["pg"], factor_dtype=torch.float32 if f32_factors else dt, state=pgst)
             d_out, keep_s = dy, k1
         else:
             d_out, d_sa, dgate = ops.combine_bwd(dy, sa, gate, k1, shift)
             keep_s = None
             with ops.side_stream(dy, ops.SIDE_BRANCH) as br:
-                dmu, gpg = ops.pg_gate_bwd(mu, dgate, pk["pg"], factor_dtype=torch.float32 if f32_factors else dt)
+                dmu, gpg = ops.pg_gate_bwd(mu, dgate, pk["pg"], factor_dtype=torch.float32 if f32_factors else dt, state=pgst)
         t4 = t.reshape(B, H, W, 3 * Cc)
         w9 = sp["w9"]
         tq, tk, tv = t4[..., :Cc], t4[..., Cc:2 * Cc], t4[..., 2 * Cc:]
diff --git a/mp-hsir_amd/csrc/arena.hip b/mp-hsir_amd/csrc/arena.hip
--- a/mp-hsir_amd/csrc/arena.hip
+++ b/mp-hsir_amd/csrc/arena.hip
@@ -10,11 +10,13 @@
     long n, stride, sbs, dbs, t0, nitems;
     long src_ld, dst_ld;
     int nsplit, vec, lg, rows, dcs;
+    const float* mul; long mul_stride;
 };
 struct RedDev {
     RedSegDev s[MPHSIR_REDUCE_MAX_SEGS];
     int nseg; long threads;
 };
+static_assert(sizeof(RedDev) <= 4096, "reduce_parts: the by-value argument block must fit the 4 KB kernel-argument segment");
 
 __global__ __launch_bounds__(256) void reduce_parts_kernel(RedDev a) {
     const long t = (long)blockIdx.x * 256 + threadIdx.x;
@@ -33,7 +35,39 @@
     f32x4 acc = f32x4{0.f, 0.f, 0.f, 0.f};
     if (live) {
         int sp = g;
-        if (s.vec & 1) {
+        if (s.mul != nullptr) {
+            const float* mul = s.mul + r;
+            if (s.vec & 1) {
+                for (; sp + 7 * G < s.nsplit; sp += 8 * G) {
+                    f32x4 v[8];
+                    float m[8];
+#pragma unroll
+                    for (int u = 0; u < 8; ++u) {
+                        v[u] = *reinterpret_cast<const f32x4*>(src + (long)(sp + u * G) * s.stride);
+                        m[u] = mul[(long)(sp + u * G) * s.mul_stride];
+                    }
+#pragma unroll
+                    for (int u = 0; u < 8; ++u) acc += m[u] * v[u];
+                }
+                for (; sp < s.nsplit; sp += G) acc += mul[(long)sp * s.mul_stride] * *reinterpret_cast<const f32x4*>(src + (long)sp * s.stride);
+            } else {
+                for (; sp + 7 * G < s.nsplit; sp += 8 * G) {
+                    f32x4 v[8];
+                    float m[8];
+#pragma unroll
+                    for (int u = 0; u < 8; ++u) {
+                        for (int e = 0; e < 4; ++e) v[u][e] = e < ne ? src[(long)(sp + u * G) * s.stride + e] : 0.f;
+                        m[u] = mul[(long)(sp + u * G) * s.mul_stride];
+                    }
+#pragma unroll
+                    for (int u = 0; u < 8; ++u) acc += m[u] * v[u];
+                }
+                for (; sp < s.nsplit; sp += G) {
+                    const float m = mul[(long)sp * s.mul_stride];
+                    for (int e = 0; e < ne; ++e) acc[e] += m * src[(long)sp * s.stride + e];
+                }
+            }
+        } else if (s.vec & 1) {
             for (; sp + 7 * G < s.nsplit; sp += 8 * G) {
                 f32x4 v[8];
 #pragma unroll
@@ -161,8 +195,9 @@
     for (int k = 0; k < nseg; ++k) {
         const mphsir_reduce_seg& g = segs[k];
         MPHSIR_REQUIRE(g.src && g.dst && g.n > 0 && g.nsplit > 0 && g.nbatch > 0, "reduce_parts: bad segment %d", k);
+        MPHSIR_REQUIRE(g.mul == nullptr || (g.nbatch == 1 && g.mul_stride > 0), "reduce_parts: product segment %d needs nbatch 1 and a row pitch of mul", k);
         const int rows = g.rows > 1 ? g.rows : 1, dcs = g.dst_col_stride > 0 ? g.dst_col_stride : 1;
-        const long src_ld = rows > 1 ? (long)g.src_ld : 0, dst_ld = rows > 1 ? (long)g.dst_ld : 0;
+        const long src_ld = rows > 1 && !g.mul ? (long)g.src_ld : 0, dst_ld = rows > 1 ? (long)g.dst_ld : 0;
         const bool vload = aligned16(g.src) && g.n % 4 == 0 && g.stride % 4 == 0 && g.src_batch_stride % 4 == 0 && src_ld % 4 == 0;
         const bool vstore = vload && aligned16(g.dst) && dcs == 1 && g.dst_batch_stride % 4 == 0 && dst_ld % 4 == 0;
         const long nitems = (long)g.nbatch * rows * ((g.n + 3) / 4);
@@ -170,7 +205,7 @@
         while (lg < 6 && (g.nsplit >> lg) > 32) ++lg;
         while (lg < 6 && (nitems << lg) < 8192 && (g.nsplit >> lg) > 4) ++lg;
         d.s[k] = RedSegDev{g.src, g.dst, (long)g.n, (long)g.stride, (long)g.src_batch_stride, (long)g.dst_batch_stride, threads, nitems,
-                           src_ld, dst_ld, g.nsplit, (vload ? 1 : 0) | (vstore ? 2 : 0), lg, rows, dcs};
+                           src_ld, dst_ld, g.nsplit, (vload ? 1 : 0) | (vstore ? 2 : 0), lg, rows, dcs, g.mul, (long)g.mul_stride};
         threads += ((nitems << lg) + 63) / 64 * 64;
     }
     d.threads = threads;
diff --git a/mp-hsir_amd/csrc/pg_gate.hip b/mp-hsir_amd/csrc/pg_gate.hip
--- a/mp-hsir_amd/csrc/pg_gate.hip
+++ b/mp-hsir_amd/csrc/pg_gate.hip
@@ -13,7 +13,8 @@
     float* gate;
     float* dmu;
     void* L; void* R;
-    int nW, C, r, KL, KR, lr_bf16;
+    float* state;
+    int nW, C, r, KL, KR, lr_bf16, SW;
     int stage_wdn;
     int wpg;
     unsigned long long* dbg;
@@ -101,12 +102,13 @@
     s.At = s.sm + PG_NWIN * PG_SMW;
     return s;
 }
-static size_t pg_lds_bytes(int C, int r, bool bwd, bool wdn = false) {
+static size_t pg_lds_bytes(int C, int r, bool bwd, bool wdn = false, bool at = false) {
     const size_t rp = r + 1;
     const int pgw = r;
     size_t n = (size_t)PG_NWIN * (C + 8) * (bwd ? 2 : 1) + (size_t)PG_NWIN * 136 * (bwd ? 2 : 1) + 132 * rp + 3 + 4 * (size_t)r * rp +
                ((r + 3) & ~3) + (size_t)C * rp + 32 + 3 + (size_t)PG_NWIN * PG_SMW;
-    if (bwd) n += (size_t)PG_NWIN * (r * rp + 4) + (wdn ? (size_t)r * C : 0);
+    if (bwd || at) n += (size_t)PG_NWIN * (r * rp + 4);
+    if (bwd && wdn) n += (size_t)r * C;
     return n * sizeof(float);
 }
 
@@ -137,6 +139,32 @@
         pg_load_chunk<NT, COLS>(wf, W, ld, nrows, nk, row0, k0, K);
         pg_mma_chunk<NT>(acc, wf, B, ldb, k0, K);
     }
+}
+
+static int pg_state_width(int r) { return (128 + 7 * r + r * r + 3) & ~3; }
+
+template <bool BWD, int R>
+__device__ __forceinline__ void pg_stage(const PgDev& a, const PgLds& s, int win0) {
+    const int C = a.C, r = R > 0 ? R : a.r, tid = threadIdx.x, nwl = a.wpg;
+    const FastDiv byC(C), byR(r);
+#pragma unroll 4
+    for (int i = tid; i < nwl * C; i += 256) {
+        const int w = byC.div(i), c = i - w * C;
+        s.mu[w * s.LDC + c] = win0 + w < a.nW ? a.mu[(long)(win0 + w) * C + c] : 0.f;
+    }
+    const int RP = s.RP;
+#pragma unroll 4
+    for (int i = tid; i < 128 * r; i += 256) { const int q = byR.div(i); s.P[q * RP + i - q * r] = a.Pp[i]; }
+    for (int i = tid; i < r * r; i += 256) {
+        const int q = byR.div(i), o = q * RP + i - q * r;
+        s.Wq[o] = a.Wq[i]; s.Wpp[o] = a.Wpproj[i]; s.Wkv[o] = a.Wkv[i]; s.Wkv[r * RP + o] = a.Wkv[r * r + i];
+    }
+    if (tid < r) s.bpp[tid] = a.bpproj[tid];
+#pragma unroll 4
+    for (int i = tid; i < C * r; i += 256) { const int q = byR.div(i); s.Wup[q * RP + i - q * r] = a.Wup[i]; }
+    if (tid < 32) s.Wup[C * RP + tid] = 0.f;
+    if (BWD && a.stage_wdn)
+        for (int i = tid; i < r * C; i += 256) s.Wdn[i] = a.Wdown[i];
 }
 
 template <bool KEEP_AT, int R>
@@ -148,25 +176,9 @@
     f32x4 wfp[8][2], wfd[8][1];
     pg_load_chunk<2, false>(wfp, a.Wprompt, C, 128, 0, rows, 0, C);
     if (has_d) pg_load_chunk<1, false>(wfd, a.Wdown, C, r, 0, rowd, 0, C);
-    const FastDiv byC(C), byR(r);
-#pragma unroll 4
-    for (int i = tid; i < nwl * C; i += 256) {
-        const int w = byC.div(i), c = i - w * C;
-        s.mu[w * s.LDC + c] = win0 + w < a.nW ? a.mu[(long)(win0 + w) * C + c] : 0.f;
-    }
+    pg_stage<KEEP_AT, R>(a, s, win0);
+    const FastDiv byR(r);
     const int RP = s.RP;
-#pragma unroll 4
-    for (int i = tid; i < 128 * r; i += 256) { const int q = byR.div(i); s.P[q * RP + i - q * r] = a.Pp[i]; }
-    for (int i = tid; i < r * r; i += 256) {
-        const int q = byR.div(i), o = q * RP + i - q * r;
-        s.Wq[o] = a.Wq[i]; s.Wpp[o] = a.Wpproj[i]; s.Wkv[o] = a.Wkv[i]; s.Wkv[r * RP + o] = a.Wkv[r * r + i];
-    }
-    if (tid < r) s.bpp[tid] = a.bpproj[tid];
-#pragma unroll 4
-    for (int i = tid; i < C * r; i += 256) { const int q = byR.div(i); s.Wup[q * RP + i - q * r] = a.Wup[i]; }
-    if (tid < 32) s.Wup[C * RP + tid] = 0.f;
-    if (KEEP_AT && a.stage_wdn)
-        for (int i = tid; i < r * C; i += 256) s.Wdn[i] = a.Wdown[i];
     __syncthreads();
     PG_MARK(1);
     {
@@ -256,12 +268,31 @@
 }
 
 template <int R>
+__device__ __forceinline__ float* pg_state_slot(const PgLds& s, int r, int w, int e, const FastDiv& byR) {
+    const int pgw = r;
+    if (e < 128) return s.w + w * s.LDW + e;
+    if (e < 128 + 7 * r) return s.sm + w * PG_SMW + (e - 128);
+    const int k = e - 128 - 7 * r, m = byR.div(k);
+    return s.At + w * s.LDA + m * s.RP + (k - m * r);
+}
+
+template <int R, bool KEEP>
 __global__ __launch_bounds__(256) void pg_gate_fwd_kernel(PgDev a) {
     HIP_DYNAMIC_SHARED(f32x4, smem_v)
     const int C = a.C, r = R > 0 ? R : a.r, pgw = r, tid = threadIdx.x, nwl = a.wpg, win0 = blockIdx.x * nwl;
     const PgLds s = pg_lds(reinterpret_cast<float*>(smem_v), C, r, false);
-    pg_forward_chain<false, R>(a, s, win0);
+    pg_forward_chain<KEEP, R>(a, s, win0);
     PG_MARK(7);
+    if (KEEP) {
+        const int SW = a.SW, nst = 128 + 7 * r + r * r;
+        const FastDiv bySW(SW), byR(r);
+#pragma unroll 4
+        for (int i = tid; i < nwl * SW; i += 256) {
+            const int w = bySW.div(i), e = i - w * SW;
+            if (win0 + w >= a.nW) continue;
+            a.state[(long)(win0 + w) * SW + e] = e < nst ? *pg_state_slot<R>(s, r, w, e, byR) : 0.f;
+        }
+    }
     const FastDiv byC(C);
     if (R > 0 && R % 4 == 0 && 256 % C == 0) {
         constexpr int RR = R > 0 ? R : 4;
@@ -294,7 +325,7 @@
     PG_MARK(8);
 }
 
-template <int R>
+template <int R, bool STATE>
 __global__ __launch_bounds__(256) void pg_gate_bwd_kernel(PgDev a) {
     HIP_DYNAMIC_SHARED(f32x4, smem_v)
     const int C = a.C, r = R > 0 ? R : a.r, pgw = r, tid = threadIdx.x, lane = tid & 63, wv = wave_id_uniform(), nwl = a.wpg, win0 = blockIdx.x * nwl;
@@ -310,7 +341,21 @@
         const int w = byC.div(i), c = i - w * C;
         s.dg[w * s.LDC + c] = win0 + w < a.nW ? a.dgate[(long)(win0 + w) * C + c] : 0.f;
     }
-    pg_forward_chain<true, R>(a, s, win0);
+    if (STATE) {
+        PG_MARK(0);
+        pg_stage<true, R>(a, s, win0);
+        const int SW = a.SW, nst = 128 + 7 * r + r * r;
+        const FastDiv bySW(SW);
+#pragma unroll 4
+        for (int i = tid; i < nwl * SW; i += 256) {
+            const int w = bySW.div(i), e = i - w * SW;
+            if (e >= nst) continue;
+            *pg_state_slot<R>(s, r, w, e, byR) = win0 + w < a.nW ? a.state[(long)(win0 + w) * SW + e] : 0.f;
+        }
+        __syncthreads();
+    } else {
+        pg_forward_chain<true, R>(a, s, win0);
+    }
     PG_MARK(7);
     const float sc = rsqrtf((float)r);
     if (wv * 16 < r) {
@@ -452,6 +497,10 @@
 void pg_debug_buffer(unsigned long long* p) { g_pg_dbg = p; }
 }
 
+extern "C" int32_t mphsir_pg_state_width(int32_t r) {
+    return (r > 0 && r <= mphsir::PG_RMAX) ? mphsir::pg_state_width(r) : MPHSIR_EINVAL;
+}
+
 extern "C" int mphsir_pg_gate_fwd(const mphsir_pg_fwd_args* a, void* stream) {
     using namespace mphsir;
     clear_error();
@@ -459,17 +508,23 @@
     MPHSIR_REQUIRE(a && a->mu && a->Wprompt && a->prompt_param && a->Wq && a->Wkv && a->Wdown && a->Wpproj && a->bpproj && a->Wup && a->gate,
                    "pg_gate_fwd: null pointer");
     MPHSIR_REQUIRE(a->nW > 0 && a->C > 0 && a->C % 16 == 0 && a->r > 0 && a->r <= PG_RMAX, "pg_gate_fwd: need C %% 16 == 0 and 0 < r <= 32");
+    MPHSIR_REQUIRE(a->state == nullptr || aligned16(a->state), "pg_gate_fwd: state must be 16-byte aligned");
     PgDev d{a->mu, nullptr, a->Wprompt, a->prompt_param, a->Wq, a->Wkv, a->Wdown, a->Wpproj, a->bpproj, a->Wup, a->gate, nullptr, nullptr,
-            nullptr, a->nW, a->C, a->r, 0, 0, 0, 0, pg_windows_per_wg(a->nW), g_pg_dbg};
-    const size_t shmem = pg_lds_bytes(a->C, a->r, false);
+            nullptr, a->state, a->nW, a->C, a->r, 0, 0, 0, pg_state_width(a->r), 0, pg_windows_per_wg(a->nW), g_pg_dbg};
+    const size_t shmem = pg_lds_bytes(a->C, a->r, false, false, a->state != nullptr);
     MPHSIR_REQUIRE(shmem <= 160 * 1024, "pg_gate_fwd: (C=%d, r=%d) needs %d bytes of LDS", a->C, a->r, (int)shmem);
     const dim3 grid((a->nW + d.wpg - 1) / d.wpg);
     hipStream_t s = reinterpret_cast<hipStream_t>(stream);
-#define MPHSIR_PG_FWD(R_)                                                                        \
-    do {                                                                                         \
-        allow_big_lds(pg_gate_fwd_kernel<R_>, shmem);                                            \
-        MPHSIR_LAUNCH(MPHSIR_K_PG_GATE, pg_gate_fwd_kernel<R_>, grid, dim3(256), shmem, s, d);    \
-        return MPHSIR_OK;                                                                        \
+#define MPHSIR_PG_FWD(R_)                                                                                   \
+    do {                                                                                                    \
+        if (d.state) {                                                                                      \
+            allow_big_lds(pg_gate_fwd_kernel<R_, true>, shmem);                                             \
+            MPHSIR_LAUNCH(MPHSIR_K_PG_GATE, (pg_gate_fwd_kernel<R_, true>), grid, dim3(256), shmem, s, d);   \
+        } else {                                                                                            \
+            allow_big_lds(pg_gate_fwd_kernel<R_, false>, shmem);                                            \
+            MPHSIR_LAUNCH(MPHSIR_K_PG_GATE, (pg_gate_fwd_kernel<R_, false>), grid, dim3(256), shmem, s, d);  \
+        }                                                                                                   \
+        return MPHSIR_OK;                                                                                   \
     } while (0)
     if (a->r == 8) MPHSIR_PG_FWD(8);
     if (a->r == 12) MPHSIR_PG_FWD(12);
@@ -488,18 +543,24 @@
     MPHSIR_REQUIRE(a->nW > 0 && a->C > 0 && a->C % 16 == 0 && a->r > 0 && a->r <= PG_RMAX, "pg_gate_bwd: need C %% 16 == 0 and 0 < r <= 32");
     MPHSIR_REQUIRE(a->KL >= a->C + 5 * a->r + 256 && a->KR >= 5 * a->r + 1 + a->C, "pg_gate_bwd: factor widths too small");
     MPHSIR_REQUIRE(!a->lr_bf16 || (a->KL % 8 == 0 && a->KR % 8 == 0), "pg_gate_bwd: bf16 factor rows need KL, KR multiples of 8");
+    MPHSIR_REQUIRE(a->state == nullptr || aligned16(a->state), "pg_gate_bwd: state must be 16-byte aligned");
     PgDev d{a->mu, a->dgate, a->Wprompt, a->prompt_param, a->Wq, a->Wkv, a->Wdown, a->Wpproj, a->bpproj, a->Wup, nullptr, a->dmu, a->L, a->R,
-            a->nW, a->C, a->r, a->KL, a->KR, a->lr_bf16, 0, pg_windows_per_wg(a->nW), g_pg_dbg};
+            const_cast<float*>(a->state), a->nW, a->C, a->r, a->KL, a->KR, a->lr_bf16, pg_state_width(a->r), 0, pg_windows_per_wg(a->nW), g_pg_dbg};
     d.stage_wdn = pg_lds_bytes(a->C, a->r, true, true) <= 160 * 1024 ? 1 : 0;
     const size_t shmem = pg_lds_bytes(a->C, a->r, true, d.stage_wdn != 0);
     MPHSIR_REQUIRE(shmem <= 160 * 1024, "pg_gate_bwd: (C=%d, r=%d) needs %d bytes of LDS", a->C, a->r, (int)shmem);
     const dim3 grid((a->nW + d.wpg - 1) / d.wpg);
     hipStream_t s = reinterpret_cast<hipStream_t>(stream);
-#define MPHSIR_PG_BWD(R_)                                                                            \
-    do {                                                                                             \
-        allow_big_lds(pg_gate_bwd_kernel<R_>, shmem);                                                \
-        MPHSIR_LAUNCH(MPHSIR_K_PG_GATE_BWD, pg_gate_bwd_kernel<R_>, grid, dim3(256), shmem, s, d);    \
-        return MPHSIR_OK;                                                                            \
+#define MPHSIR_PG_BWD(R_)                                                                                       \
+    do {                                                                                                        \
+        if (d.state) {                                                                                          \
+            allow_big_lds(pg_gate_bwd_kernel<R_, true>, shmem);                                                 \
+            MPHSIR_LAUNCH(MPHSIR_K_PG_GATE_BWD, (pg_gate_bwd_kernel<R_, true>), grid, dim3(256), shmem, s, d);   \
+        } else {                                                                                                \
+            allow_big_lds(pg_gate_bwd_kernel<R_, false>, shmem);                                                \
+            MPHSIR_LAUNCH(MPHSIR_K_PG_GATE_BWD, (pg_gate_bwd_kernel<R_, false>), grid, dim3(256), shmem, s, d);  \
+        }                                                                                                       \
+        return MPHSIR_OK;                                                                                       \
     } while (0)
     if (a->r == 8) MPHSIR_PG_BWD(8);
     if (a->r == 12) MPHSIR_PG_BWD(12);
diff --git a/mp-hsir_amd/ops.py b/mp-hsir_amd/ops.py
--- a/mp-hsir_amd/ops.py
+++ b/mp-hsir_amd/ops.py
@@ -109,7 +109,7 @@
                 _flush_calls(self.calls)
                 _flush_gemms(self.gemms)
                 for g in self.segs:
-                    g["keep"] = (g["keep"][0], g["keep"][1].detach())
+                    g["keep"] = (g["keep"][0], g["keep"][1].detach()) + tuple(g["keep"][2:])
                 _poison(self.segs)
                 _DEFERRED.extend(self.segs)
             else:
@@ -147,7 +147,7 @@
         st = _DW_STREAM[dev] = torch.cuda.Stream(dev)
     main = torch.cuda.current_stream(dev)
     for g in scope.segs:
-        g["keep"] = (g["keep"][0], g["keep"][1].detach())
+        g["keep"] = (g["keep"][0], g["keep"][1].detach()) + tuple(g["keep"][2:])
     _poison(scope.segs)
     if DW_SIDE >= 2:
         nbytes = sum(g["M"] * (g["N1"] + g["N2"]) * 2 for g in scope.gemms)
@@ -304,6 +304,7 @@
             a.n, a.stride, a.src_batch_stride, a.dst_batch_stride = g["n"], g["stride"], g["sbs"], g["dbs"]
             a.nsplit, a.nbatch, a.rows, a.dst_col_stride = g["nsplit"], g["nbatch"], g["rows"], g["dcs"]
             a.src_ld, a.dst_ld = g["src_ld"], g["dst_ld"]
+            a.mul, a.mul_stride = g.get("mul"), g.get("mul_stride", 0)
             nbytes += 4.0 * g["nbatch"] * max(1, g["rows"]) * g["n"] * (g["nsplit"] + 1)
         _lib.check(lib.mphsir_reduce_parts(arr, len(chunk), _stream(chunk[0]["keep"][0])), "reduce_parts")
         _acct("reduce_parts", nbytes / 4.0, nbytes)
@@ -354,6 +355,17 @@
                  nbatch=1, rows=max(nr, 1), dcs=dcs, src_ld=Cc, dst_ld=dst_ld, keep=(part, out)), immediate)
     if nr == 1:
         pass
+    return out
+
+
+def reduce_product(L, R, r0, nr, c0, nc, out, immediate=False):
+    _check(L, R, out)
+    assert L.dtype == R.dtype == out.dtype == torch.float32 and L.dim() == 2 and R.dim() == 2 and L.shape[0] == R.shape[0]
+    assert L.stride(1) == 1 and R.stride(1) == 1 and 0 <= r0 and r0 + nr <= L.shape[1] and 0 <= c0 and c0 + nc <= R.shape[1]
+    assert tuple(out.shape) == (nr, nc) and out.stride(1) == 1
+    _submit(dict(src=R.data_ptr() + 4 * c0, dst=out.data_ptr(), n=nc, stride=R.stride(0), sbs=0, dbs=0, nsplit=L.shape[0], nbatch=1,
+                 rows=max(nr, 1), dcs=1, src_ld=0, dst_ld=out.stride(0), mul=L.data_ptr() + 4 * r0, mul_stride=L.stride(0),
+                 keep=(L, out, R)), immediate)
     return out
 
 
@@ -870,7 +882,7 @@
     return sa, gate
 
 
-def pg_gate_fwd(mu, pg):
+def pg_gate_fwd(mu, pg, keep_state=False):
     lib = _lib.load()
     _check(mu, *pg.values())
     nW, C = mu.shape
@@ -878,13 +890,19 @@
     gate = torch.empty_like(mu)
     a = _lib.PgFwdArgs()
     a.mu, a.gate = _p(mu), _p(gate)
+    state = None
+    if keep_state:
+        sw = lib.mphsir_pg_state_width(r)
+        assert sw > 0, "pg_gate_fwd: r = %d unsupported" % r
+        state = torch.empty((nW, sw), dtype=torch.float32, device=mu.device)
+        a.state = _p(state)
     a.Wprompt, a.prompt_param = _p(pg["linear_prompt.weight"]), _p(pg["prompt_param"])
     a.Wq, a.Wkv, a.Wdown = _p(pg["q.weight"]), _p(pg["kv.weight"]), _p(pg["linear_down.weight"])
     a.Wpproj, a.bpproj, a.Wup = _p(pg["proj.weight"]), _p(pg["proj.bias"]), _p(pg["linear_up.weight"])
     a.nW, a.C, a.r = nW, C, r
     _lib.check(lib.mphsir_pg_gate_fwd(ctypes.byref(a), _stream(mu)), "pg_gate_fwd")
-    _acct("pg_gate", 2.0 * nW * C * (128 + 2 * r), 4.0 * nW * 2 * C)
-    return gate
+    _acct("pg_gate", 2.0 * nW * C * (128 + 2 * r), 4.0 * nW * (2 * C + (state.shape[1] if keep_state else 0)))
+    return (gate, state) if keep_state else gate
 
 
 def pack_dw(w):
@@ -1642,9 +1660,28 @@
     return W2, reduce_parts(dWo), reduce_parts(dtemp)
 
 
-def pg_gate_bwd(mu, dgate, pg, factor_dtype=torch.float32):
+def pg_factor_blocks(C, r):
+    return {
+        "linear_up.weight": (0, C, 0, r),
+        "proj.weight": (C, r, r, r),
+        "proj.bias": (C, r, 2 * r, 1),
+        "kv.weight": (C + r, 2 * r, 2 * r + 1, r),
+        "q.weight": (C + 3 * r, r, 3 * r + 1, r),
+        "prompt_param": (C + 4 * r, 128, 4 * r + 1, r),
+        "linear_prompt.weight": (C + 4 * r + 128, 128, 5 * r + 1, C),
+        "linear_down.weight": (C + 4 * r + 256, r, 5 * r + 1, C),
+    }
+
+
+def pg_gate_bwd(mu, dgate, pg, factor_dtype=torch.float32, state=None, factor_gemm=None):
     lib = _lib.load()
     _check(mu, dgate, *pg.values())
+    if factor_gemm is None:
+        factor_gemm = factor_dtype != torch.float32
+    assert factor_gemm or factor_dtype == torch.float32, "product segments take fp32 factor rows"
+    if state is not None:
+        _check(state)
+        assert state.dtype == torch.float32 and state.is_contiguous() and tuple(state.shape) == (mu.shape[0], lib.mphsir_pg_state_width(pg["linear_down.weight"].shape[0]))
     nW, C = mu.shape
     r = pg["linear_down.weight"].shape[0]
     KL, KR = round_up(C + 5 * r + 256, 8), round_up(5 * r + 1 + C, 8)
@@ -1658,21 +1695,16 @@
     a.Wpproj, a.bpproj, a.Wup = _p(pg["proj.weight"]), _p(pg["proj.bias"]), _p(pg["linear_up.weight"])
     a.dmu, a.L, a.R = _p(dmu), _p(L), _p(R)
     a.nW, a.C, a.r, a.KL, a.KR, a.lr_bf16 = nW, C, r, KL, KR, _DT[factor_dtype]
+    if state is not None:
+        a.state = _p(state)
     _lib.check(lib.mphsir_pg_gate_bwd(ctypes.byref(a), _stream(mu)), "pg_gate_bwd")
     _acct("pg_gate_bwd", 4.0 * nW * C * (128 + 2 * r), 4.0 * nW * (2 * C + KL + KR))
-    part = gemm_tn(L, R, reduce=False)[0]
-    blocks = {
-        "linear_up.weight": (0, C, 0, r),
-        "proj.weight": (C, r, r, r),
-        "proj.bias": (C, r, 2 * r, 1),
-        "kv.weight": (C + r, 2 * r, 2 * r + 1, r),
-        "q.weight": (C + 3 * r, r, 3 * r + 1, r),
-        "prompt_param": (C + 4 * r, 128, 4 * r + 1, r),
-        "linear_prompt.weight": (C + 4 * r + 128, 128, 5 * r + 1, C),
-        "linear_down.weight": (C + 4 * r + 256, r, 5 * r + 1, C),
-    }
-    g = {k: reduce_block(part, r0, nr, c0, nc, torch.empty((nr, nc), dtype=torch.float32, device=mu.device))
-         for k, (r0, nr, c0, nc) in blocks.items()}
+    part = gemm_tn(L, R, reduce=False)[0] if factor_gemm else None
+    blocks = pg_factor_blocks(C, r)
+    g = {}
+    for k, (r0, nr, c0, nc) in blocks.items():
+        out = torch.empty((nr, nc), dtype=torch.float32, device=mu.device)
+        g[k] = reduce_block(part, r0, nr, c0, nc, out) if factor_gemm else reduce_product(L, R, r0, nr, c0, nc, out)
     g["proj.bias"] = g["proj.bias"].reshape(r)
     return dmu, g
 
```

Measured after the change: 1715 patches/s. No clear change (-0.6%).
